# Luckick/EAGCN

Hardware: AMD Instinct MI355X
Metric: molecules/sec fwd+bwd, 2-layer 5-view EAGCN, Tox21 batch (higher is better)
Workload: dtype f32 (bf16x3 split, fp32 accumulate): every fp32 operand leaves its producer as three bf16 planes, six v_mfma_f32_32x32x16_bf16 piece products per 16 k rebuild the fp32 product (csrc/gemm_bx3.hip); aggregation, BatchNorm, head, first layer fp32

## Files before the change

eagcn_amd/_lib.py:

```python
import ctypes as C
import os

_HERE = os.path.dirname(os.path.abspath(__file__))
LIB_PATH = os.path.join(_HERE, 'lib', 'libeagcn_hip.so')

MAX_VIEWS = 8
MAX_SEGS = 8
META_WORDS = 16
META_NLOG = 8
META_T, META_NMAX, META_NTILES, META_BAD_ADJ, META_BAD_REL, META_NEDGE, META_OVERFLOW, META_EDGE_OVERFLOW = range(8)
META_NBLK = 9
STRUCT_CONCATE, STRUCT_WEIGHTED = 0, 1

_fp = C.c_void_p


class Batch(C.Structure):
    _fields_ = [('B', C.c_int32), ('N', C.c_int32), ('K', C.c_int32), ('ldc', C.c_int32),
                ('T', C.c_int32), ('n_max', C.c_int32), ('n_tiles', C.c_int32),
                ('channels', C.c_int32 * MAX_VIEWS),
                ('code', _fp), ('deg_bn', _fp), ('nat', _fp), ('row0', _fp), ('tile0', _fp),
                ('meta', _fp), ('row_mol', _fp), ('row_loc', _fp), ('row_m', _fp), ('row_deg', _fp),
                ('tile_mol', _fp), ('row_info', _fp), ('tile_info', _fp),
                ('rel_vec', _fp * MAX_VIEWS), ('rel_c', C.c_int32 * MAX_VIEWS),
# ... 41 lines not shown
def bond_ptrs_len(T, B):
    return 4 * T + 4 * B + 8 * (B + 1) + 8


def set_bond_lists(c, small_ptr, ptrs, edges, E):
    c.E = int(E)
    c.ecnt, c.edge0 = small_ptr, small_ptr + 4 * c.B
    pb, T = ptrs.data_ptr(), c.T
    c.row_ptr, c.col_ptr, c.mol_info = pb, pb + 8 * T, pb + 16 * T
    blk = pb + 16 * T + 16 * c.B
    c.blk = blk + (-blk) % 16 if ptrs.numel() >= bond_ptrs_len(T, c.B) else None
    eb = edges.data_ptr()
    c.nbr, c.tnbr = eb, eb + 4 * E
    code = eb + 8 * E
    code += (-code) % 8
    c.ecode, c.tcode = code, code + 8 * E


def index_error(meta, row_cap=None, edge_cap=None, compact=False):
    if meta[META_BAD_ADJ] and compact:
        return '%d bonds are out of range or listed twice' % meta[META_BAD_ADJ]
    if meta[META_BAD_ADJ]:
        return ('adjs holds %d entries outside {0,1}: the hot path requires a 0/1 adjacency (reference neural_fp.py:85,109-110)'
                % meta[META_BAD_ADJ])
    if meta[META_BAD_REL]:
        return ('%d bonded (i,j,view) positions are not one-hot over the relation channels (reference neural_fp.py:111-120); '
                'build the model with relations=\'general\' for relation tensors with arbitrary channel values (layers.py:82)'
                % meta[META_BAD_REL])
    if row_cap is not None and meta[META_OVERFLOW]:
        return ('%d packed rows, more than row_cap=%d (the batch is indexed as an empty batch; no memory is overwritten)'
                % (meta[META_OVERFLOW], row_cap))
    if edge_cap is not None and meta[META_EDGE_OVERFLOW]:
        return ('%d directed bonds, more than edge_cap=%d (the batch is indexed as an empty batch; no memory is overwritten)'
                % (meta[META_EDGE_OVERFLOW], edge_cap))
    return None


def dropout_seeds(seed, n_layers=4):
    seed = int(seed)
    return [(seed + 7919 * (l + 1)) & (2 ** 63 - 1) for l in range(n_layers)], (seed + 0x51ED27) & (2 ** 63 - 1)


STRUCTURES = {'Concate': 0, 'Weighted_sum': 1}


def structure_code(name):
    return STRUCTURES.get(name, -1)


class GatParams(C.Structure):
    _fields_ = [('fin', C.c_int32), ('ld_in', C.c_int32), ('F', C.c_int32), ('training', C.c_int32),
                ('alpha', C.c_float), ('att_dropout', C.c_float), ('dropout', C.c_float), ('reserved_', C.c_float),
                ('seed', C.c_uint64), ('W', _fp), ('a', _fp), ('seed_dev', C.c_void_p)]


POOL_MAX = 8


class PoolAtt(C.Structure):
    _fields_ = [('K', C.c_int32), ('mode', C.c_int32), ('att_c', C.c_int32 * MAX_VIEWS), ('att_w', _fp * MAX_VIEWS),
                ('ave_a', _fp), ('self_r', _fp), ('datt_w', _fp * MAX_VIEWS), ('dave_a', _fp), ('dself_r', _fp)]


class Layout(C.Structure):
    _fields_ = [('nseg', C.c_int32), ('width', C.c_int32 * MAX_SEGS), ('pad', C.c_int32 * MAX_SEGS)]


class LayerParams(C.Structure):
    _fields_ = [('K', C.c_int32), ('structure', C.c_int32), ('training', C.c_int32),
                ('width', C.c_int32 * MAX_VIEWS), ('inp', Layout),
                ('dropout', C.c_float), ('bn_eps', C.c_float), ('bn_momentum', C.c_float),
                ('seed', C.c_uint64), ('seed_dev', _fp),
                ('att_w', _fp * MAX_VIEWS), ('self_r', _fp * MAX_VIEWS), ('W', _fp * MAX_VIEWS),
                ('bias', _fp * MAX_VIEWS), ('gamma', _fp * MAX_VIEWS), ('beta', _fp * MAX_VIEWS),
                ('run_mean', _fp * MAX_VIEWS), ('run_var', _fp * MAX_VIEWS), ('ave_w', _fp)]


class LayerBufs(C.Structure):
    _fields_ = [('x', _fp), ('P', _fp), ('Y', _fp), ('rscale', _fp), ('bn', _fp), ('xout', _fp),
                ('pad_row', _fp), ('scratch', _fp), ('scratch_bytes', C.c_size_t),
                ('aux_stream', _fp), ('packed', _fp), ('packed_bytes', C.c_size_t),
                ('stats_hook', _fp), ('stats_user', _fp), ('x_planes', _fp), ('xout_planes', _fp)]


class LayerGrads(C.Structure):
    _fields_ = [('dW', _fp * MAX_VIEWS), ('dbias', _fp * MAX_VIEWS), ('dgamma', _fp * MAX_VIEWS),
                ('dbeta', _fp * MAX_VIEWS), ('datt_w', _fp * MAX_VIEWS), ('dself_r', _fp * MAX_VIEWS),
                ('dave_w', _fp)]


class HeadParams(C.Structure):
    _fields_ = [('f_in', C.c_int32), ('n_den1', C.c_int32), ('n_den2', C.c_int32), ('nclass', C.c_int32),
                ('dropout', C.c_float), ('bn_eps', C.c_float), ('bn_momentum', C.c_float),
                ('den1_w', _fp), ('den2_w', _fp), ('den3_w', _fp),
                ('gbn_w', _fp), ('gbn_b', _fp), ('gbn_rm', _fp), ('gbn_rv', _fp),
                ('bn1_w', _fp), ('bn1_b', _fp), ('bn1_rm', _fp), ('bn1_rv', _fp),
                ('bn2_w', _fp), ('bn2_b', _fp), ('bn2_rm', _fp), ('bn2_rv', _fp)]


class HeadGrads(C.Structure):
    _fields_ = [(n, _fp) for n in ('d_den1_w', 'd_den2_w', 'd_den3_w', 'd_gbn_w', 'd_gbn_b', 'd_bn1_w', 'd_bn1_b',
                                   'd_bn2_w', 'd_bn2_b')]


class Model(C.Structure):
    _fields_ = [('n_layers', C.c_int32), ('molfp_mode', C.c_int32), ('training', C.c_int32),
                ('head_seed', C.c_uint64), ('head_seed_dev', _fp), ('input_packed', C.c_int32), ('aux_stream', _fp),
                ('layer', LayerParams * 4), ('head', HeadParams), ('stats_hook', _fp), ('stats_user', _fp),
                ('stats_world', C.c_int32), ('fuse_readout', C.c_int32), ('fwd_signal', _fp), ('wait_flag', _fp), ('start_signal', _fp)]


class StepLoss(C.Structure):
    _fields_ = [('kind', C.c_int32), ('labels', _fp), ('class_weight', _fp), ('loss', _fp), ('scale', _fp), ('dout', _fp)]


ALLREDUCE_FN = C.CFUNCTYPE(C.c_int, C.c_void_p, C.c_int, C.c_void_p, C.c_void_p)


SIGNATURES = {
    'eagcn_abi_version': (C.c_int, []),
    'eagcn_struct_size': (C.c_size_t, [C.c_int]),
    'eagcn_last_error': (C.c_char_p, []),
    'eagcn_pad16': (C.c_int, [C.c_int]),
    'eagcn_layer_out_ld': (C.c_int, [C.POINTER(LayerParams)]),
    'eagcn_layer_fp': (C.c_int, [C.POINTER(LayerParams)]),
    'eagcn_layer_packed_bytes': (C.c_size_t, [C.POINTER(Batch), C.POINTER(LayerParams)]),
    'eagcn_layer_fwd_scratch_bytes': (C.c_size_t, [C.POINTER(Batch), C.POINTER(LayerParams)]),
    'eagcn_layer_bwd_scratch_bytes': (C.c_size_t, [C.POINTER(Batch), C.POINTER(LayerParams)]),
    'eagcn_layer_route': (C.c_int, [C.POINTER(Batch), C.POINTER(LayerParams), C.POINTER(LayerBufs), C.c_int, C.c_int, C.c_int, C.c_int,
                                    C.POINTER(C.c_int32 * 16)]),
    'eagcn_index_build': (C.c_int, [_fp, C.POINTER(_fp), C.POINTER(Batch), _fp, _fp]),
    'eagcn_index_from_bonds': (C.c_int, [_fp, _fp, _fp, _fp, C.c_int64, C.POINTER(Batch), _fp, _fp]),
    'eagcn_index_rows': (C.c_int, [C.POINTER(Batch), _fp]),
    'eagcn_set_gemm_mode': (C.c_int, [C.c_int]),
    'eagcn_stream_wait_counter': (C.c_int, [_fp, C.c_uint32, _fp]),
    'eagcn_stream_signal_flag': (C.c_int, [_fp, _fp]),
    'eagcn_stream_wait_flag': (C.c_int, [_fp, C.c_double, _fp]),
    'eagcn_stream_wait_timeouts': (C.c_int, []),
    'eagcn_stream_wait_reset': (None, []),
    'eagcn_adam_step': (C.c_int, [_fp, _fp, _fp, _fp, C.c_int64, _fp, _fp, _fp, _fp]),
    'eagcn_grad_norm_workspace_bytes': (C.c_size_t, []),
    'eagcn_grad_norm': (C.c_int, [_fp, _fp, C.c_int64, _fp, C.c_int, _fp]),
    'eagcn_adam_step_clipped': (C.c_int, [_fp, _fp, _fp, _fp, C.c_int64, _fp, _fp, _fp, _fp, _fp, _fp, _fp]),
    'eagcn_agg_wants_bond_lists': (C.c_int, [C.c_int, C.c_int]),
    'eagcn_agg_wants_bond_lists_for': (C.c_int, [C.c_int, C.c_int, C.c_int]),
    'eagcn_bx3_used_splits': (C.c_int, [C.c_int, C.c_int, C.c_int, C.c_int]),
    'eagcn_set_bx3_wide': (C.c_int, [C.c_int]),
    'eagcn_set_top_bn_sums': (C.c_int, [C.c_int]),
    'eagcn_set_hidden_bn_sums': (C.c_int, [C.c_int]),
    'eagcn_hidden_bn_sums_taken': (C.c_long, [C.c_int]),
    'eagcn_set_first_layer_fused': (C.c_int, [C.c_int]),
    'eagcn_first_layer_fused_taken': (C.c_long, [C.c_int]),
    'eagcn_first_layer_fused_last': (None, [C.POINTER(C.c_int32)]),
    'eagcn_bx3_pair_used_splits': (C.c_int, [C.c_int] * 7),
    'eagcn_bx3_plane_elems': (C.c_size_t, [C.c_int, C.c_int]),
    'eagcn_bx3_split': (C.c_int, [_fp, C.c_int, C.c_int, _fp, C.c_size_t, C.c_int, C.c_int, _fp]),
    'eagcn_gemm_bx3': (C.c_int, [C.c_int, C.c_int, C.c_int, C.c_int, _fp, C.c_size_t, C.c_int, C.c_int, _fp, C.c_size_t, C.c_int, C.c_int,
                                 _fp, C.c_int, C.c_int, C.c_size_t, C.c_int, _fp]),
    'eagcn_gemm_bx3_pair': (C.c_int, [C.c_int, C.c_int, C.c_int, _fp, C.c_size_t, C.c_int, C.c_int, _fp, C.c_size_t, C.c_int, C.c_int, _fp, C.c_int,
                                      C.c_int, C.c_int, C.c_int, _fp, C.c_size_t, C.c_int, C.c_int, _fp, C.c_size_t, C.c_int, C.c_int, _fp, C.c_int,
                                      C.c_int, C.c_size_t, C.c_int, _fp]),
    'eagcn_pack_rows': (C.c_int, [C.POINTER(Batch), _fp, C.c_int, C.POINTER(Layout), _fp, _fp]),
    'eagcn_unpack_rows': (C.c_int, [C.POINTER(Batch), _fp, C.POINTER(Layout), _fp, _fp, C.c_int, _fp]),
    'eagcn_pad_rows': (C.c_int, [_fp, _fp, C.c_int, C.c_int, C.c_int, _fp, _fp]),
    'eagcn_gat_scratch_bytes': (C.c_size_t, [C.POINTER(Batch), C.c_int]),
    'eagcn_gat_forward': (C.c_int, [C.POINTER(Batch), C.POINTER(GatParams), _fp, _fp, _fp, _fp, _fp]),
    'eagcn_gat_backward': (C.c_int, [C.POINTER(Batch), C.POINTER(GatParams), _fp, _fp, _fp, _fp, _fp, _fp, _fp, _fp, _fp,
                                     C.c_size_t, _fp]),
    'eagcn_pool_scratch_bytes': (C.c_size_t, []),
    'eagcn_pool_attention_forward': (C.c_int, [C.POINTER(Batch), C.POINTER(PoolAtt), _fp, C.c_int, _fp, _fp, _fp]),
    'eagcn_pool_attention_backward': (C.c_int, [C.POINTER(Batch), C.POINTER(PoolAtt), _fp, C.c_int, _fp, _fp, _fp, C.c_size_t,
                                                _fp]),
    'eagcn_pool_mix_forward': (C.c_int, [C.POINTER(Batch), C.POINTER(Layout), _fp, C.c_int, _fp, _fp, _fp, _fp, C.c_int, _fp]),
    'eagcn_pool_mix_backward': (C.c_int, [C.POINTER(Batch), C.POINTER(Layout), _fp, C.c_int, _fp, _fp, _fp, _fp, C.c_int, _fp,
                                          _fp, _fp, _fp]),
    'eagcn_pool_reduce_forward': (C.c_int, [C.POINTER(Batch), _fp, C.c_int, C.c_int, C.c_int, _fp, _fp, _fp, _fp]),
    'eagcn_pool_reduce_backward': (C.c_int, [C.POINTER(Batch), _fp, C.c_int, C.c_int, C.c_int, _fp, _fp, _fp, _fp, _fp]),
    'eagcn_layer_forward': (C.c_int, [C.POINTER(Batch), C.POINTER(LayerParams), C.POINTER(LayerBufs), _fp]),
    'eagcn_layer_backward': (C.c_int, [C.POINTER(Batch), C.POINTER(LayerParams), C.POINTER(LayerBufs),
                                       _fp, _fp, _fp, C.POINTER(LayerGrads), _fp]),
    'eagcn_attention_dense': (C.c_int, [C.POINTER(Batch), C.POINTER(LayerParams), _fp, _fp]),
    'eagcn_readout_forward': (C.c_int, [C.POINTER(Batch), _fp, C.POINTER(Layout), _fp, _fp, C.c_int, _fp,
                                        C.c_int, _fp]),
    'eagcn_readout_backward': (C.c_int, [C.POINTER(Batch), _fp, C.POINTER(Layout), _fp, C.c_int, C.c_int,
                                         _fp, _fp, _fp]),
    'eagcn_gemm_f32': (C.c_int, [C.c_int, C.c_int, C.c_int, C.c_int, C.c_int, _fp, C.c_int, _fp, C.c_int,
                                 _fp, C.c_int, _fp]),
    'eagcn_gemm_f32_dev': (C.c_int, [C.c_int, C.c_int, C.c_int, C.c_int, C.c_int, _fp, C.c_int, _fp, C.c_int,
                                     _fp, C.c_int, _fp, C.c_int, _fp]),
    'eagcn_gemm_sk_workspace_bytes': (C.c_size_t, []),
    'eagcn_gemm_f32_sk': (C.c_int, [C.c_int, C.c_int, C.c_int, C.c_int, C.c_int, _fp, C.c_int, _fp, C.c_int,
                                    _fp, C.c_int, _fp, C.c_size_t, _fp]),
    'eagcn_gemm_pair_sk': (C.c_int, [C.c_int, C.c_int, C.c_int, _fp, C.c_int, _fp, C.c_int, _fp, C.c_int,
                                     C.c_int, C.c_int, C.c_int, _fp, C.c_int, _fp, C.c_int, _fp, C.c_int,
                                     _fp, C.c_size_t, _fp]),
    'eagcn_gemm_pair_sk_slabs': (C.c_int, [C.c_int, C.c_int, C.c_int, _fp, C.c_int, _fp, C.c_int, _fp, C.c_int,
                                           C.c_int, C.c_int, C.c_int, _fp, C.c_int, _fp, C.c_int, _fp, C.c_int,
                                           C.c_size_t, _fp, C.c_size_t, _fp]),
    'eagcn_gemm_sk_plan': (C.c_int, [C.c_int] * 7 + [C.POINTER(C.c_int), C.POINTER(C.c_int)]),
    'eagcn_gemm_sk_timeouts': (C.c_int, []),
    'eagcn_gemm_sk_failed': (C.c_int, []),
    'eagcn_gemm_sk_reset_failed': (None, []),
    'eagcn_gemm_sk_inject_failure': (None, []),
    'eagcn_model_saved_bytes': (C.c_size_t, [C.POINTER(Batch), C.POINTER(Model)]),
    'eagcn_model_scratch_bytes': (C.c_size_t, [C.POINTER(Batch), C.POINTER(Model)]),
    'eagcn_model_atom_rep': (C.c_int, [C.POINTER(Batch), C.POINTER(Model), C.POINTER(C.c_size_t),
                                       C.POINTER(C.c_size_t), C.POINTER(C.c_int)]),
    'eagcn_model_atom_rep_materialize': (C.c_int, [C.POINTER(Batch), C.POINTER(Model), _fp, C.c_size_t, _fp]),
    'eagcn_model_pack_input': (C.c_int, [C.POINTER(Batch), C.POINTER(Model), _fp, _fp, C.c_size_t, _fp]),
    'eagcn_model_forward': (C.c_int, [C.POINTER(Batch), C.POINTER(Model), _fp, _fp, _fp, C.c_size_t, _fp,
                                      C.c_size_t, _fp, _fp, _fp]),
    'eagcn_model_backward': (C.c_int, [C.POINTER(Batch), C.POINTER(Model), _fp, _fp, C.c_size_t, _fp, C.c_size_t,
                                       _fp, _fp, C.POINTER(LayerGrads), C.POINTER(HeadGrads), _fp]),
    'eagcn_model_backward_range': (C.c_int, [C.POINTER(Batch), C.POINTER(Model), _fp, _fp, C.c_size_t, _fp, C.c_size_t,
                                             _fp, _fp, C.POINTER(LayerGrads), C.POINTER(HeadGrads), C.c_int, C.c_int, C.c_int, _fp]),
    'eagcn_model_route': (C.c_int, [C.POINTER(Batch), C.POINTER(Model), _fp, C.c_size_t, _fp, C.c_size_t, C.c_int, C.c_int, C.c_int, C.c_int,
                                    C.c_int, C.POINTER(C.c_int32 * 16 * 4)]),
    'eagcn_model_input_scratch_bytes': (C.c_size_t, [C.POINTER(Batch), C.POINTER(Model)]),
    'eagcn_model_backward_input': (C.c_int, [C.POINTER(Batch), C.POINTER(Model), _fp, _fp, C.c_size_t, _fp, C.c_size_t,
                                             _fp, _fp, C.POINTER(LayerGrads), C.POINTER(HeadGrads), _fp, _fp]),
    'eagcn_attr_alpha': (C.c_float, [C.c_int, C.c_int]),
    'eagcn_attr_weight': (C.c_float, [C.c_int]),
    'eagcn_attr_acc_elems': (C.c_size_t, [C.POINTER(Batch), C.POINTER(Model)]),
    'eagcn_attr_pack_input': (C.c_int, [C.POINTER(Batch), C.POINTER(Model), _fp, _fp, C.c_float, _fp, C.c_size_t, _fp]),
    'eagcn_attr_step': (C.c_int, [C.POINTER(Batch), C.POINTER(Model), _fp, _fp, C.c_size_t, _fp, C.c_size_t, _fp, _fp, C.c_float,
                                  C.c_int, _fp, _fp]),
    'eagcn_attr_finalize': (C.c_int, [C.POINTER(Batch), C.POINTER(Model), _fp, _fp, _fp, _fp, _fp, _fp]),
    'eagcn_layer_bond_grad': (C.c_int, [C.POINTER(Batch), C.POINTER(LayerParams), C.POINTER(LayerBufs), _fp, C.c_int, C.c_float, C.c_int,
                                        _fp, _fp]),
    'eagcn_bond_attr_finalize': (C.c_int, [C.POINTER(Batch), _fp, C.c_int, _fp, _fp, _fp, _fp, _fp, _fp]),
    'eagcn_model_forward_step': (C.c_int, [C.POINTER(Batch), C.POINTER(Model), _fp, _fp, _fp, C.c_size_t, _fp, C.c_size_t, _fp, _fp,
                                           C.POINTER(StepLoss), _fp, C.POINTER(HeadGrads), _fp]),
    'eagcn_head_saved_bytes': (C.c_size_t, [C.POINTER(HeadParams), C.c_int]),
    'eagcn_head_scratch_bytes': (C.c_size_t, [C.POINTER(HeadParams), C.c_int]),
    'eagcn_head_forward': (C.c_int, [C.POINTER(HeadParams), C.c_int, C.c_int, C.c_uint64, _fp, _fp, _fp, C.c_size_t, _fp, C.c_size_t,
                                     _fp, _fp, _fp]),
    'eagcn_head_backward': (C.c_int, [C.POINTER(HeadParams), C.c_int, C.c_int, C.c_uint64, _fp, _fp, _fp, C.c_size_t, _fp, C.c_size_t,
                                      _fp, _fp, C.POINTER(HeadGrads), _fp, _fp]),
    'eagcn_bce_loss': (C.c_int, [_fp, _fp, _fp, C.c_int, C.c_int, _fp, _fp, _fp]),
    'eagcn_mse_loss': (C.c_int, [_fp, _fp, C.c_int, _fp, _fp, _fp]),
    'eagcn_eval_append': (C.c_int, [_fp, _fp, C.c_int, C.c_int, C.c_int, _fp, _fp, _fp, C.c_int64, _fp]),
    'eagcn_eval_metrics_workspace_bytes': (C.c_size_t, [C.c_int64, C.c_int]),
    'eagcn_eval_class_metrics': (C.c_int, [_fp, _fp, _fp, C.c_int64, C.c_int, _fp, C.c_size_t, _fp, _fp]),
    'eagcn_eval_reg_metrics': (C.c_int, [_fp, _fp, _fp, C.c_int64, C.c_int, _fp, C.c_size_t, _fp, _fp]),
    'eagcn_rep_gather': (C.c_int, [C.POINTER(Batch), _fp, C.POINTER(Layout), _fp, _fp, C.c_int, C.c_int, _fp, _fp, _fp, _fp, _fp, _fp,
                                   C.c_int64, _fp]),
    'eagcn_rep_gather_dense': (C.c_int, [_fp, C.c_int, C.c_int, C.c_int, _fp, C.c_int, C.c_int, C.c_int, _fp, _fp, _fp, _fp, _fp, _fp,
                                         C.c_int64, _fp]),
    'eagcn_kmeans_workspace_bytes': (C.c_size_t, [C.c_int64, C.c_int, C.c_int]),
    'eagcn_kmeans_begin': (C.c_int, [_fp, C.c_int64, C.c_int, C.c_int, C.c_int, _fp, C.c_double, _fp, C.c_size_t, _fp]),
    'eagcn_kmeans_iterate': (C.c_int, [_fp, C.c_int64, C.c_int, C.c_int, C.c_int, _fp, C.c_size_t, _fp]),
    'eagcn_kmeans_finish': (C.c_int, [_fp, C.c_int64, C.c_int, C.c_int, C.c_int, _fp, C.c_size_t, _fp]),
    'eagcn_kmeans_assign': (C.c_int, [_fp, C.c_int64, C.c_int, C.c_int, _fp, C.c_int, _fp, _fp, _fp, C.c_size_t, _fp]),
    'eagcn_sqdist': (C.c_int, [_fp, C.c_int64, C.c_int, C.c_int, _fp, _fp]),
    'eagcn_tsne_workspace_bytes': (C.c_size_t, [C.c_int64]),
    'eagcn_tsne_affinities': (C.c_int, [_fp, C.c_int64, C.c_double, _fp, C.c_int, _fp, _fp, _fp, C.c_size_t, _fp]),
    'eagcn_tsne_gradient': (C.c_int, [_fp, C.c_int, _fp, C.c_int64, C.c_float, C.c_int, _fp, _fp, _fp, C.c_size_t, _fp]),
    'eagcn_tsne_begin': (C.c_int, [_fp, C.c_int, C.c_int64, _fp, C.c_float, C.c_float, C.c_int, C.c_int, C.c_double, _fp, C.c_size_t,
                                   _fp]),
    'eagcn_tsne_iterate': (C.c_int, [_fp, C.c_int, C.c_int64, _fp, C.c_size_t, _fp]),
    'eagcn_tsne_finish': (C.c_int, [_fp, C.c_int, C.c_int64, _fp, C.c_size_t, _fp]),
    'eagcn_pca_workspace_bytes': (C.c_size_t, [C.c_int64, C.c_int]),
    'eagcn_pca_cov': (C.c_int, [_fp, C.c_int64, C.c_int, C.c_int, _fp, _fp, _fp, C.c_size_t, _fp]),
    'eagcn_pca_project': (C.c_int, [_fp, C.c_int64, C.c_int, C.c_int, _fp, _fp, C.c_int, _fp, _fp]),
    'eagcn_knn_workspace_bytes': (C.c_size_t, [C.c_int64, C.c_int64, C.c_int, C.c_int, C.c_int]),
    'eagcn_knn': (C.c_int, [_fp, C.c_int64, C.c_int, C.c_int, _fp, C.c_int64, C.c_int, C.c_int, C.c_int, C.c_int, _fp, _fp, _fp, C.c_size_t,
                            _fp]),
    'eagcn_knn_rank': (C.c_int, [_fp, C.c_int64, C.c_int, C.c_int, _fp, C.c_int, C.c_int, _fp, _fp, C.c_size_t, _fp]),
    'eagcn_prof_enable': (None, [C.c_int]),
    'eagcn_prof_reset': (None, []),
    'eagcn_prof_ntags': (C.c_int, []),
    'eagcn_prof_tag_name': (C.c_char_p, [C.c_int]),
    'eagcn_prof_read': (C.c_int, [C.c_int, C.POINTER(C.c_double), C.POINTER(C.c_double), C.POINTER(C.c_int64)]),
}

_lib = None


class EagcnHipError(RuntimeError):
    pass


ABI_VERSION = 8


def load():
    global _lib
    if _lib is not None:
        return _lib
    if not os.path.exists(LIB_PATH):
        raise EagcnHipError(
            'libeagcn_hip.so is not built (%s). Run `python -c "import __graft_entry__ as g; g.build()"` '
            'or `python -m eagcn_amd.build`; eagcn_amd has no CPU fallback.' % LIB_PATH)
    lib = C.CDLL(LIB_PATH)
    lib.eagcn_abi_version.restype = C.c_int
    if lib.eagcn_abi_version() != ABI_VERSION:
        raise EagcnHipError('libeagcn_hip.so speaks ABI version %d, this binding version %d: rebuild it '
                            '(`python -c "import __graft_entry__ as g; g.build()"`)' % (lib.eagcn_abi_version(), ABI_VERSION))
    for name, (res, args) in SIGNATURES.items():
        fn = getattr(lib, name)
        fn.restype = res
        fn.argtypes = args
    for which, cls in ((0, Batch), (1, Layout), (2, LayerParams), (3, LayerBufs), (4, LayerGrads), (5, HeadParams), (6, HeadGrads),
                       (7, Model), (10, StepLoss)):
        if lib.eagcn_struct_size(which) != C.sizeof(cls):
            raise EagcnHipError('ABI mismatch: %s is %d bytes here, %d in libeagcn_hip.so'
# ... 27 lines not shown
```

eagcn_amd/build.py:

```python
import os
import shutil
import subprocess
import sys
from concurrent.futures import ThreadPoolExecutor

HERE = os.path.dirname(os.path.abspath(__file__))
CSRC = os.path.join(HERE, 'csrc')
LIBDIR = os.path.join(HERE, 'lib')
LIB = os.path.join(LIBDIR, 'libeagcn_hip.so')
HIP_SOURCES = ['index.hip', 'gemm.hip', 'gemm3.hip', 'gemm_bx3.hip', 'gemm_bx3w.hip', 'agg.hip', 'lagg.hip', 'lagg_in.hip', 'lagg_top.hip', 'lagg_dw.hip', 'gat.hip', 'pool.hip', 'layer.hip', 'readout.hip', 'head.hip', 'head2.hip', 'loss.hip', 'clip.hip', 'attr.hip', 'battr.hip', 'metrics.hip', 'reps.hip', 'embed.hip', 'knn.hip']
CPP_SOURCES = ['api.cpp']
HEADERS = ['common.h', 'kernels.h', 'lagg_kernel.h', 'gemm_x6.h', 'bx3.h', 'bx3_epi.h', os.path.join('..', '..', 'include', 'eagcn_hip.h')]
ARCH = 'gfx950'


def _hipcc():
    for cand in (shutil.which('hipcc'), '/opt/rocm/bin/hipcc'):
        if cand and os.path.exists(cand):
            return cand
    raise RuntimeError('hipcc not found: the EAGCN HIP library cannot be built')


def _newest(paths):
    return max(os.path.getmtime(p) for p in paths)


def needs_build():
    srcs = [os.path.join(CSRC, s) for s in HIP_SOURCES + CPP_SOURCES + HEADERS if os.path.exists(os.path.join(CSRC, s))]
    return (not os.path.exists(LIB)) or os.path.getmtime(LIB) < _newest(srcs)


def build_library(force=False, verbose=False):
    if not force and not needs_build():
        return LIB
    hipcc = _hipcc()
    os.makedirs(LIBDIR, exist_ok=True)
    objdir = os.path.join(LIBDIR, 'obj')
    os.makedirs(objdir, exist_ok=True)
    flags = ['--offload-arch=' + ARCH, '-O3', '-std=c++17', '-fPIC', '-Wall', '-Wno-unused-function', '-munsafe-fp-atomics']

    hdr_time = _newest([os.path.join(CSRC, h) for h in HEADERS if os.path.exists(os.path.join(CSRC, h))])

    def compile_one(src):
        obj = os.path.join(objdir, os.path.splitext(src)[0] + '.o')
        if not force and os.path.exists(obj) and os.path.getmtime(obj) > max(hdr_time, os.path.getmtime(os.path.join(CSRC, src))):
            return obj
        cmd = [hipcc] + flags + ['-c', os.path.join(CSRC, src), '-o', obj]
        if src.endswith('.cpp'):
            cmd = [hipcc, '-O2', '-std=c++17', '-fPIC', '-c', os.path.join(CSRC, src), '-o', obj]
        r = subprocess.run(cmd, capture_output=True, text=True)
        if r.returncode != 0:
            raise RuntimeError('hipcc failed on %s:\n%s\n%s' % (src, r.stdout, r.stderr))
        if verbose and r.stderr.strip():
            print(r.stderr, file=sys.stderr)
        return obj

    sources = [s for s in HIP_SOURCES + CPP_SOURCES if os.path.exists(os.path.join(CSRC, s))]
    with ThreadPoolExecutor(max_workers=min(8, len(sources))) as ex:
        objs = list(ex.map(compile_one, sources))
    tmp = LIB + '.tmp'
    r = subprocess.run([hipcc, '--offload-arch=' + ARCH, '-shared', '-fPIC', '-o', tmp] + objs,
                       capture_output=True, text=True)
    if r.returncode != 0:
        raise RuntimeError('link failed:\n%s\n%s' % (r.stdout, r.stderr))
    os.replace(tmp, LIB)
    return LIB


if __name__ == '__main__':
    print(build_library(force='--force' in sys.argv, verbose=True))
```

eagcn_amd/csrc/head.hip:

```cpp
#include <stdlib.h>

#include <algorithm>

#include "common.h"
#include "kernels.h"

namespace eagcn {

__global__ void wait_counter_kernel(const uint32_t* __restrict__ word, uint32_t value, int* __restrict__ err,
                                    unsigned long long budget_ticks) {
    if (threadIdx.x == 0) {
        const unsigned long long t0 = wall_clock64();
        while ((int32_t)(__hip_atomic_load(word, __ATOMIC_ACQUIRE, __HIP_MEMORY_SCOPE_AGENT) - value) < 0) {
            __builtin_amdgcn_s_sleep(64);
            if (wall_clock64() - t0 > budget_ticks) {
                if (err) __hip_atomic_store(err, 1, __ATOMIC_RELAXED, __HIP_MEMORY_SCOPE_SYSTEM);
                break;
            }
        }
    }
}



// ... 129 lines not shown
    const eagcn_head_params* h = &m->head;
    const size_t B = (size_t)b->B, T = (size_t)b->T;
    s.n_hst = 2 * (h->f_in + h->n_den1 + h->n_den2) + 6;
    s.hst = c.take<double>((size_t)(HEAD_COPIES + 1) * s.n_hst + HEAD_WS);
    s.hsb = s.hst + (size_t)HEAD_COPIES * s.n_hst;
    s.hws = s.hsb + s.n_hst;
    s.da2 = c.take<float>(B * h->n_den2);
    s.da1 = c.take<float>(B * h->n_den1);
    s.dgn = c.take<float>(B * h->f_in);
    s.dg = c.take<float>(B * h->f_in);
    s.hdw_ks = head_dw_chunks(b->B);
    s.hdw = c.take<float>(s.hdw_ks > 1 ? (size_t)s.hdw_ks * ((size_t)h->f_in * h->n_den1 + (size_t)h->n_den1 * h->n_den2 +
                                                             (size_t)h->n_den2 * h->nclass) : 1);
    int ldmax = 0;
    size_t lbytes = 0;
    for (int l = 0; l < m->n_layers; ++l) {
        ldmax = std::max(ldmax, eagcn_layer_out_ld(&m->layer[l]));
        lbytes = std::max(lbytes, eagcn_layer_fwd_scratch_bytes(b, &m->layer[l]));
        lbytes = std::max(lbytes, eagcn_layer_bwd_scratch_bytes(b, &m->layer[l]));
    }
    s.dxa = c.take<float>(T * ldmax);
    s.dxb = c.take<float>(T * ldmax);
    s.dpad = c.take<float>((size_t)EAGCN_MAX_VIEWS * ldmax);
    s.layer_bytes = lbytes;
    s.layer = c.take<char>(lbytes);
    s.top_dge = c.take<float>(B * h->f_in);
    s.top_slab = c.take<double>((size_t)top_bn_slabs(b->B) * eagcn_layer_fp(&m->layer[m->n_layers - 1]) * 2);
    int fpmax = 0;
    for (int l = 0; l + 1 < m->n_layers; ++l) fpmax = std::max(fpmax, eagcn_layer_fp(&m->layer[l]));
    s.hid_slab = c.take<double>(fpmax ? (size_t)hidden_bn_slabs(b->T) * fpmax * 2 : 1);
    if (out) *out = s;
    return c.off;
}

static int check_model(const eagcn_batch* b, const eagcn_model* m, const char* who) {
    EAGCN_CHECK_ARG(b && m, "%s: null argument", who);
    if (int rc = check_reserved_null(m->aux_stream, who, "eagcn_model.aux_stream")) return rc;
    EAGCN_CHECK_ARG(m->n_layers >= 1 && m->n_layers <= 4, "%s: n_layers=%d", who, m->n_layers);
    const eagcn_head_params* h = &m->head;
    EAGCN_CHECK_ARG(h->f_in >= 1 && h->n_den1 >= 1 && h->n_den2 >= 1 && h->nclass >= 1, "%s: bad head sizes", who);
    EAGCN_CHECK_ARG(h->den1_w && h->den2_w && h->den3_w && h->gbn_w && h->gbn_b && h->gbn_rm && h->gbn_rv &&
                        h->bn1_w && h->bn1_b && h->bn1_rm && h->bn1_rv && h->bn2_w && h->bn2_b && h->bn2_rm &&
                        h->bn2_rv, "%s: null head parameter", who);
    const eagcn_layer_params* last = &m->layer[m->n_layers - 1];
    const int f_last = last->structure == EAGCN_STRUCT_CONCATE ? [&] { int s = 0; for (int k = 0; k < last->K; ++k) s += last->width[k]; return s; }()
                                                                 : last->width[0];
    EAGCN_CHECK_ARG(f_last == h->f_in, "%s: head expects %d features, last layer yields %d", who, h->f_in, f_last);
    EAGCN_CHECK_ARG(!m->training || b->B > 1, "%s: BatchNorm in training mode needs more than one molecule", who);
    return EAGCN_OK;
}

static eagcn_layout out_layout(const eagcn_layer_params* p) {
    eagcn_layout l;
    memset(&l, 0, sizeof(l));
    if (p->structure == EAGCN_STRUCT_CONCATE) {
        l.nseg = p->K;
        for (int k = 0; k < p->K; ++k) { l.width[k] = p->width[k]; l.pad[k] = pad16(p->width[k]); }
    } else {
        l.nseg = 1;
        l.width[0] = p->width[0];
        l.pad[0] = pad16(p->width[0]);
    }
    return l;
}

static bool fused_readout(const eagcn_model* m) {
    static const bool env = !env_flag("EAGCN_NO_FUSED_READOUT", false);
    return env && m->fuse_readout && m->layer[m->n_layers - 1].structure == EAGCN_STRUCT_CONCATE;
}

struct ModelAsk { int layer_hi = -1, layer_lo = 0; bool has_dx0 = false, input_only = false; };
struct LayerPlan {
    eagcn_layer_bufs w;
    LayerRoute fwd, bwd;
    bool planes_only = false;
    bool skip_apply = false;
    BxBnEpi below = {};
};
struct ModelPlan { LayerPlan L[4]; bool top_formed = false; };
static ModelPlan plan_model(const eagcn_batch* b, const eagcn_model* m, const ModelSaved& sv, const ModelScratch& sc, const ModelAsk& ask) {
    ModelPlan P{};
    const int top = m->n_layers - 1;
    PlanAsk full;
    full.has_dx = true;
    for (int l = 0; l <= top; ++l) {
        const LayerSaved& L = sv.L[l];
        LayerPlan& Q = P.L[l];
        eagcn_layer_bufs& w = Q.w;
        w.P = L.P; w.Y = L.Y; w.rscale = L.rscale; w.bn = L.bn; w.xout = L.xout; w.pad_row = L.pad_row;
        w.scratch = sc.layer; w.scratch_bytes = sc.layer_bytes; w.packed = L.packed; w.packed_bytes = L.packed_bytes;
        w.stats_hook = m->stats_hook; w.stats_user = m->stats_user;
        w.x_planes = l > 0 ? sv.L[l - 1].xout_planes : nullptr; w.xout_planes = L.xout_planes;
        const bool try_planes = w.x_planes && planes_only_enabled();
        w.x = l == 0 ? sv.x0 : try_planes ? nullptr : sv.L[l - 1].xout;
        Q.fwd = plan_layer(b, &m->layer[l], &w, PlanAsk{});
        if (try_planes) {
            P.L[l - 1].planes_only = Q.fwd.fwd_prod == FWD_PLANES && plan_layer(b, &m->layer[l], &w, full).bwd_prod == BWD_PLANES_PAIR;
            if (!P.L[l - 1].planes_only) { w.x = sv.L[l - 1].xout; Q.fwd = plan_layer(b, &m->layer[l], &w, PlanAsk{}); }
        }
    }
    P.L[top].skip_apply = fused_readout(m);
    const float* dge = top_bn_gather_enabled() ? sc.top_dge : nullptr;
    auto call_ask = [&](int l, const ModelAsk& k, bool top_sums) {
        PlanAsk a;
        a.has_dx = l > 0 || k.has_dx0; a.mol_grad = l == top; a.input_only = k.input_only; a.has_drain_out = l > k.layer_lo && !k.input_only;
        a.top_sums = l == top && top_sums && !k.input_only; a.top_gather = a.top_sums && top_gather_ok(&m->layer[top], dge, m->head.f_in);
        return a;
    };
    if (top_bn_sums_enabled() && P.L[top].skip_apply && m->training && m->layer[top].training && !m->stats_hook && (unsigned)m->molfp_mode <= 1u) {
        const LayerRoute r = plan_layer(b, &m->layer[top], &P.L[top].w, call_ask(top, ModelAsk{top}, true));
        P.top_formed = r.bn2 == BN2_STAGED_FROM_READOUT && r.bwd_agg == AGG_LAGG && r.edge == EDGE_WITH_LAGG;
    }
    for (int l = ask.layer_hi; l >= ask.layer_lo; --l) {
        LayerPlan& Q = P.L[l];
        PlanAsk a = call_ask(l, ask, P.top_formed);
        a.dh_given = l < ask.layer_hi && P.L[l + 1].bwd.carries_below;
        if (l > ask.layer_lo && !ask.input_only && m->training && !m->stats_hook && sv.L[l].ld_in == sv.L[l - 1].fp) {
            PlanAsk low = call_ask(l - 1, ask, false);
            low.dh_given = true;
            a.below = plan_layer(b, &m->layer[l - 1], &P.L[l - 1].w, low).dh_given;
        }
        Q.bwd = plan_layer(b, &m->layer[l], &Q.w, a);
        if (Q.bwd.carries_below) {
            const eagcn_layer_params* lo = &m->layer[l - 1];
            const DropArgs dr = drop_args(lo->dropout, lo->training != 0, lo->seed, lo->seed_dev);
            const LayerSaved& S = sv.L[l - 1];
            Q.below = BxBnEpi{S.Y, S.fp, S.bn, S.fp, b->row_m, dr.on, dr.thr, dr.inv_keep, dr.seed, dr.seed_dev, sc.hid_slab};
        }
    }
    return P;
}

}

using namespace eagcn;

#define RC(call) do { int rc_ = (call); if (rc_) return rc_; } while (0)

extern "C" size_t eagcn_model_saved_bytes(const eagcn_batch* b, const eagcn_model* m) {
    return carve_saved(nullptr, b, m, nullptr);
}
extern "C" size_t eagcn_model_scratch_bytes(const eagcn_batch* b, const eagcn_model* m) {
    return carve_scratch(nullptr, b, m, nullptr);
}
extern "C" int eagcn_model_atom_rep(const eagcn_batch* b, const eagcn_model* m, size_t* xout_offset,
                                    size_t* pad_row_offset, int* ld) {
    EAGCN_CHECK_ARG(b && m && xout_offset && pad_row_offset && ld, "eagcn_model_atom_rep: null argument");
    RC(check_reserved_null(m->aux_stream, "eagcn_model_atom_rep", "eagcn_model.aux_stream"));
    ModelSaved s;
    carve_saved(nullptr, b, m, &s);
    *xout_offset = s.xout_last_off;
    *pad_row_offset = s.pad_last_off;
    *ld = eagcn_layer_out_ld(&m->layer[m->n_layers - 1]);
    return EAGCN_OK;
}

extern "C" int eagcn_model_atom_rep_materialize(const eagcn_batch* b, const eagcn_model* m, void* saved, size_t saved_bytes,
                                                 void* stream) {
    EAGCN_CHECK_ARG(b && m && saved, "eagcn_model_atom_rep_materialize: null argument");
    RC(check_reserved_null(m->aux_stream, "eagcn_model_atom_rep_materialize", "eagcn_model.aux_stream"));
    if (!fused_readout(m)) return EAGCN_OK;
    ModelSaved sv;
    EAGCN_CHECK_ARG(carve_saved(saved, b, m, &sv) <= saved_bytes, "eagcn_model_atom_rep_materialize: saved block too small");
    const int l = m->n_layers - 1;
    LayerSaved& L = sv.L[l];
    eagcn_layer_bufs w;
    memset(&w, 0, sizeof(w));
    w.Y = L.Y; w.bn = L.bn; w.xout = L.xout; w.pad_row = L.pad_row; w.packed = L.packed; w.packed_bytes = L.packed_bytes;
    return layer_apply_impl(b, &m->layer[l], &w, stream);
}

extern "C" int eagcn_model_pack_input(const eagcn_batch* b, const eagcn_model* m, const float* afm, void* saved,
                                      size_t saved_bytes, void* stream) {
    EAGCN_CHECK_ARG(b && m && afm && saved, "eagcn_model_pack_input: null argument");
    RC(check_reserved_null(m->aux_stream, "eagcn_model_pack_input", "eagcn_model.aux_stream"));
    ModelSaved sv;
    EAGCN_CHECK_ARG(carve_saved(saved, b, m, &sv) <= saved_bytes, "eagcn_model_pack_input: saved block too small");
    return eagcn_pack_rows(b, afm, layout_width(&m->layer[0].in), &m->layer[0].in, sv.x0, stream);
}

struct HeadPlan {
    HeadFwd f1, f2, f3;
    HeadBwd b3, b2, b1;
    HeadGbn bg;
    double *st_g, *st_1, *st_2, *sb_g, *sb_1, *sb_2;
    bool sync;
    const int64_t* size;
};
static HeadPlan head_plan(const eagcn_batch* b, const eagcn_model* m, const ModelSaved& sv, const ModelScratch& sc, float* out,
                          float* graph_rep, const float* dout, const float* dgraph_rep, const eagcn_head_grads* hg,
                          const int64_t* size = nullptr, bool top_formed = false) {
    HeadPlan P;
    P.size = size;
    const eagcn_head_params* h = &m->head;
    const int B = b->B, F = h->f_in, n1 = h->n_den1, n2 = h->n_den2, nc = h->nclass;
    P.st_g = sc.hst; P.st_1 = sc.hst + 2 * F + 2; P.st_2 = sc.hst + 2 * (F + n1) + 4;
    P.sb_g = sc.hsb; P.sb_1 = sc.hsb + 2 * F + 2; P.sb_2 = sc.hsb + 2 * (F + n1) + 4;
    P.sync = m->stats_hook && m->training;
    const int copies = P.sync ? 1 : HEAD_COPIES;
    const HeadDrop nodrop{0, 0u, 1.0f, 0, nullptr}, drop1 = drop_args(h->dropout, m->training != 0, m->head_seed, m->head_seed_dev);
    P.f1 = HeadFwd{B, F, n1, sv.g, P.st_g, h->gbn_w, h->gbn_b, h->gbn_rm, h->gbn_rv, sv.bn_g, h->den1_w, sv.h1, nullptr, P.st_1,
                   m->training, 0, h->bn_eps, h->bn_momentum, nodrop};
    P.f2 = HeadFwd{B, n1, n2, sv.h1, P.st_1, h->bn1_w, h->bn1_b, h->bn1_rm, h->bn1_rv, sv.bn_1, h->den2_w, sv.h2, graph_rep, P.st_2,
                   m->training, 1, h->bn_eps, h->bn_momentum, drop1};
    P.f3 = HeadFwd{B, n2, nc, sv.h2, P.st_2, h->bn2_w, h->bn2_b, h->bn2_rm, h->bn2_rv, sv.bn_2, h->den3_w, out, nullptr, nullptr,
                   m->training, 1, h->bn_eps, h->bn_momentum, nodrop};
    if (P.sync) { P.f1.cnt_in = P.st_g + 2 * F; P.f2.cnt_in = P.st_1 + 2 * n1; P.f3.cnt_in = P.st_2 + 2 * n2; }
    P.f3.nw = 8;
    P.f1.signal = m->fwd_signal;
    P.f1.st_copies = P.f2.st_copies = P.f3.st_copies = copies;
    P.f1.st_stride = P.f2.st_stride = P.f3.st_stride = sc.n_hst;
    if (!hg) return P;
    const double *cn_g = sc.hst + 2 * F, *cn_1 = sc.hst + 2 * F + 2 + 2 * n1, *cn_2 = sc.hst + 2 * (F + n1) + 4 + 2 * n2;
    const float gscale = P.sync && m->stats_world > 1 ? 1.0f / (float)m->stats_world : 1.0f;
    P.b3 = HeadBwd{B, n2, nc, sv.h2, sv.bn_2, 1, nodrop, h->den3_w, dout, nullptr, nullptr, nullptr, nullptr, nullptr, nullptr,
                   sc.da2, P.sb_2, hg->d_den3_w, m->training};
    P.b2 = HeadBwd{B, n1, n2, sv.h1, sv.bn_1, 1, drop1, h->den2_w, sc.da2, sv.h2, sv.bn_2, P.sb_2, dgraph_rep, hg->d_bn2_w, hg->d_bn2_b,
                   sc.da1, P.sb_1, hg->d_den2_w, m->training};
    P.b1 = HeadBwd{B, F, n1, sv.g, sv.bn_g, 0, nodrop, h->den1_w, sc.da1, sv.h1, sv.bn_1, P.sb_1, nullptr, hg->d_bn1_w, hg->d_bn1_b,
                   sc.dgn, P.sb_g, hg->d_den1_w, m->training};
    if (P.sync) { P.b2.cnt_y = cn_2; P.b2.gscale = gscale; P.b1.cnt_y = cn_1; P.b1.gscale = gscale; }
    P.b3.nw = 8;
    const int ks = sc.hdw_ks;
    float* part3 = sc.hdw;
    float* part2 = part3 + (size_t)ks * n2 * nc;
    float* part1 = part2 + (size_t)ks * n1 * n2;
    if (ks > 1) {
        P.b3.ks = ks; P.b3.dW_part = part3;
        P.b2.ks = ks; P.b2.dW_part = part2;
        P.b1.ks = ks; P.b1.dW_part = part1;
    }
    P.bg = HeadGbn{B, F, sc.dgn, sv.g, sv.bn_g, P.sb_g, sc.dg, hg->d_gbn_w, hg->d_gbn_b, m->training};
    if (P.sync) { P.bg.cnt = cn_g; P.bg.gscale = gscale; }
    if (top_formed) {
        const eagcn_layer_params* last = &m->layer[m->n_layers - 1];
        const eagcn_layout lay = out_layout(last);
        P.bg.top = HeadTopSums{sv.top_a1, sv.top_a2, sc.top_slab, top_bn_slabs(B), eagcn_layer_fp(last), make_colmap(&lay), P.size, m->molfp_mode,
                               top_bn_gather_enabled() ? sc.top_dge : nullptr};
    }
    if (ks > 1) {
        P.bg.sum[0] = HeadDwSum{hg->d_den3_w, part3, n2 * nc, ks};
        P.bg.sum[1] = HeadDwSum{hg->d_den2_w, part2, n1 * n2, ks};
        P.bg.sum[2] = HeadDwSum{hg->d_den1_w, part1, F * n1, ks};
        P.bg.nsum = 3;
    }
    return P;
}

static int model_forward_trunk(const eagcn_batch* b, const eagcn_model* m, const float* afm, const int64_t* size, void* saved,
                               size_t saved_bytes, void* scratch, size_t scratch_bytes, ModelSaved& sv, ModelScratch& sc,
                               ModelPlan& P, void* stream, const char* who) {
    hipStream_t s = (hipStream_t)stream;
    RC(check_model(b, m, who));
    EAGCN_CHECK_GEMM3(who);
    EAGCN_CHECK_ARG((afm || m->input_packed) && saved && scratch, "%s: null buffer", who);
    EAGCN_CHECK_ARG(m->molfp_mode == 0 || size, "%s: 'ave' read-out needs size", who);
    EAGCN_CHECK_ARG(carve_saved(saved, b, m, &sv) <= saved_bytes, "%s: saved block too small", who);
    EAGCN_CHECK_ARG(carve_scratch(scratch, b, m, &sc) <= scratch_bytes, "%s: scratch too small", who);
    const eagcn_head_params* h = &m->head;
    HandOff ho{m->start_signal, m->wait_flag, wait_err_word(), 200000000ull};
    if (!m->input_packed && (m->wait_flag || m->start_signal)) {
        handoff_kernel<<<1, 64, 0, s>>>(ho);
        EAGCN_LAUNCH_CHECK();
        ho.start = nullptr; ho.flag = nullptr;
    }
    ZeroJob zj;
    RC(gemm3_zero_job(sc.layer, sc.layer_bytes, sc.hst, (HEAD_COPIES + 1) * sc.n_hst + HEAD_WS, &zj));
    if (!m->input_packed)
        RC(eagcn_pack_rows(b, afm, layout_width(&m->layer[0].in), &m->layer[0].in, sv.x0, stream));
    {
        const eagcn_layer_params* ps[4];
        void* pk[4];
        size_t pkb[4];
        for (int l = 0; l < m->n_layers; ++l) { ps[l] = &m->layer[l]; pk[l] = sv.L[l].packed; pkb[l] = sv.L[l].packed_bytes; }
        RC(pack_params_all(b, ps, pk, pkb, m->n_layers, stream, &zj, &ho));
    }
    P = plan_model(b, m, sv, sc, ModelAsk{});
    for (int l = 0; l < m->n_layers; ++l)
        RC(layer_forward_impl(b, &m->layer[l], &P.L[l].w, stream, P.L[l].fwd, true, P.L[l].skip_apply, P.L[l].planes_only));
    const eagcn_layer_params* last = &m->layer[m->n_layers - 1];
    const LayerSaved& LL = sv.L[m->n_layers - 1];
    const eagcn_layout lay = out_layout(last);
    const int B = b->B, F = h->f_in, n1 = h->n_den1, n2 = h->n_den2;
    double *st_g = sc.hst, *st_1 = sc.hst + 2 * F + 2, *st_2 = sc.hst + 2 * (F + n1) + 4;
    const int copies = (m->stats_hook && m->training) ? 1 : HEAD_COPIES;
    if (fused_readout(m)) {
        ReadoutBn rb;
        rb.Y = LL.Y; rb.ldy = LL.fp; rb.bn = LL.bn; rb.fp = LL.fp;
        const DropArgs ld = drop_args(last->dropout, last->training != 0, last->seed, last->seed_dev);
        rb.do_drop = ld.on; rb.thr = ld.thr; rb.inv_keep = ld.inv_keep; rb.seed = ld.seed; rb.seed_dev = ld.seed_dev;
        rb.size = size; rb.mode = m->molfp_mode; rb.g = sv.g; rb.F = F; rb.st = st_g;
        rb.cnt0 = st_g + 2 * F; rb.cnt1 = st_1 + 2 * n1; rb.cnt2 = st_2 + 2 * n2;
        rb.st_copies = copies; rb.st_stride = sc.n_hst;
        if (P.top_formed) { rb.A1 = sv.top_a1; rb.A2 = sv.top_a2; }
        RC(readout_bn_forward(b, &lay, rb, stream));
    } else if (pad_sampled(m))
        RC(readout_forward_sampled(b, LL.xout, &lay, last, LL.bn + (size_t)LL.fp , size,
                                   m->molfp_mode, sv.g, F, sv.pad_cnt, sv.padc, sv.pad_tab, stream));
    else
        RC(eagcn_readout_forward(b, LL.xout, &lay, last->structure == EAGCN_STRUCT_WEIGHTED ? LL.pad_row : nullptr,
                                 size, m->molfp_mode, sv.g, F, stream));
    if (!fused_readout(m)) RC(head_colstats(sv.g, B, F, st_g, s, st_g + 2 * F, st_1 + 2 * n1, st_2 + 2 * n2));
    return EAGCN_OK;
}

static int stats_hook_call(const eagcn_model* m, bool sync, double* buf, int n, void* stream) {
    if (!sync) return EAGCN_OK;
    if (m->stats_hook(buf, n, stream, m->stats_user)) {
        set_error("eagcn_model: the sync-BatchNorm all-reduce hook failed");
        return EAGCN_ERR_HIP;
    }
    return EAGCN_OK;
}

static int head_forward_launches(const eagcn_model* m, const HeadPlan& P, void* stream) {
    hipStream_t s = (hipStream_t)stream;
    const eagcn_head_params* h = &m->head;
    RC(stats_hook_call(m, P.sync, P.st_g, 2 * h->f_in + 1, stream));
    RC(head_fwd(P.f1, s));
    RC(stats_hook_call(m, P.sync, P.st_1, 2 * h->n_den1 + 1, stream));
    RC(head_fwd(P.f2, s));
    RC(stats_hook_call(m, P.sync, P.st_2, 2 * h->n_den2 + 1, stream));
    RC(head_fwd(P.f3, s));
    return EAGCN_OK;
}
static int head_backward_launches(const eagcn_model* m, const HeadPlan& P, void* stream) {
    hipStream_t s = (hipStream_t)stream;
    const eagcn_head_params* h = &m->head;
    RC(head_bwd(P.b3, s));
    RC(stats_hook_call(m, P.sync, P.sb_2, 2 * h->n_den2, stream));
    RC(head_bwd(P.b2, s));
    RC(stats_hook_call(m, P.sync, P.sb_1, 2 * h->n_den1, stream));
    RC(head_bwd(P.b1, s));
    RC(stats_hook_call(m, P.sync, P.sb_g, 2 * h->f_in, stream));
    RC(head_gbn_bwd(P.bg, s));
    return EAGCN_OK;
}
static int readout_pad_backward(const eagcn_batch* b, const eagcn_model* m, const int64_t* size, const ModelSaved& sv,
                                const ModelScratch& sc, void* stream) {
    const eagcn_layer_params* last = &m->layer[m->n_layers - 1];
    const eagcn_layout lay = out_layout(last);
    const int F = m->head.f_in;
    if (pad_sampled(m)) return readout_backward_pad_views(b, sc.dg, &lay, size, m->molfp_mode, F, last->K, sv.pad_cnt, last->dropout, sc.dpad, stream);
    if (last->structure == EAGCN_STRUCT_WEIGHTED) return readout_backward_pad(b, sc.dg, &lay, size, m->molfp_mode, F, sc.dpad, stream);
    return EAGCN_OK;
}

extern "C" int eagcn_model_forward(const eagcn_batch* b, const eagcn_model* m, const float* afm,
                                   const int64_t* size, void* saved, size_t saved_bytes, void* scratch,
                                   size_t scratch_bytes, float* out, float* graph_rep, void* stream) {
    EAGCN_CHECK_ARG(out && graph_rep, "eagcn_model_forward: null buffer");
    ModelSaved sv;
    ModelScratch sc;
    ModelPlan mp;
    RC(model_forward_trunk(b, m, afm, size, saved, saved_bytes, scratch, scratch_bytes, sv, sc, mp, stream, "eagcn_model_forward"));
    const HeadPlan P = head_plan(b, m, sv, sc, out, graph_rep, nullptr, nullptr, nullptr);
    return head_forward_launches(m, P, stream);
}

namespace eagcn {
static int check_head(const eagcn_head_params* h, int B, int training, const char* who) {
    EAGCN_CHECK_ARG(h, "%s: null argument", who);
    EAGCN_CHECK_ARG(B >= 1 && h->f_in >= 1 && h->n_den1 >= 1 && h->n_den2 >= 1 && h->nclass >= 1, "%s: bad head sizes", who);
    EAGCN_CHECK_ARG(h->den1_w && h->den2_w && h->den3_w && h->gbn_w && h->gbn_b && h->gbn_rm && h->gbn_rv && h->bn1_w && h->bn1_b &&
                        h->bn1_rm && h->bn1_rv && h->bn2_w && h->bn2_b && h->bn2_rm && h->bn2_rv, "%s: null head parameter", who);
    EAGCN_CHECK_ARG(!training || B > 1, "%s: BatchNorm in training mode needs more than one molecule", who);
    return EAGCN_OK;
}
static size_t carve_head_saved(void* base, const eagcn_head_params* h, int B, ModelSaved* out) {
    Carver2 c(base);
    ModelSaved s;
    memset(&s, 0, sizeof(s));
    s.h1 = c.take<float>((size_t)B * h->n_den1);
    s.h2 = c.take<float>((size_t)B * h->n_den2);
    s.bn_g = c.take<float>((size_t)4 * h->f_in);
    s.bn_1 = c.take<float>((size_t)4 * h->n_den1);
    s.bn_2 = c.take<float>((size_t)4 * h->n_den2);
    if (out) *out = s;
    return c.off;
}
static size_t carve_head_scratch(void* base, const eagcn_head_params* h, int B, ModelScratch* out) {
    Carver2 c(base);
    ModelScratch s;
    memset(&s, 0, sizeof(s));
    s.n_hst = 2 * (h->f_in + h->n_den1 + h->n_den2) + 6;
    s.hst = c.take<double>((size_t)(HEAD_COPIES + 1) * s.n_hst + HEAD_WS);
    s.hsb = s.hst + (size_t)HEAD_COPIES * s.n_hst;
    s.hws = s.hsb + s.n_hst;
    s.da2 = c.take<float>((size_t)B * h->n_den2);
    s.da1 = c.take<float>((size_t)B * h->n_den1);
    s.dgn = c.take<float>((size_t)B * h->f_in);
    s.hdw_ks = head_dw_chunks(B);
    s.hdw = c.take<float>(s.hdw_ks > 1 ? (size_t)s.hdw_ks * ((size_t)h->f_in * h->n_den1 + (size_t)h->n_den1 * h->n_den2 +
                                                             (size_t)h->n_den2 * h->nclass) : 1);
    if (out) *out = s;
    return c.off;
}
__global__ __launch_bounds__(256) void head_zero_kernel(double* __restrict__ p, int n) {
    for (int i = blockIdx.x * blockDim.x + threadIdx.x; i < n; i += gridDim.x * blockDim.x) p[i] = 0.0;
}
static int head_zero(double* p, size_t n, hipStream_t s) {
    head_zero_kernel<<<(unsigned)std::max<size_t>(1, std::min<size_t>((n + 255) / 256, 64)), 256, 0, s>>>(p, (int)n);
    EAGCN_LAUNCH_CHECK();
    return EAGCN_OK;
}
static void head_alone_model(const eagcn_head_params* h, int B, int training, uint64_t seed, const uint64_t* seed_dev,
                             eagcn_batch* b, eagcn_model* m) {
    memset(b, 0, sizeof(*b));
    memset(m, 0, sizeof(*m));
    b->B = B;
    m->head = *h; m->training = training ? 1 : 0; m->head_seed = seed; m->head_seed_dev = seed_dev;
}
}

extern "C" size_t eagcn_head_saved_bytes(const eagcn_head_params* h, int B) { return h ? carve_head_saved(nullptr, h, B, nullptr) : 0; }
extern "C" size_t eagcn_head_scratch_bytes(const eagcn_head_params* h, int B) { return h ? carve_head_scratch(nullptr, h, B, nullptr) : 0; }

extern "C" int eagcn_head_forward(const eagcn_head_params* h, int B, int training, uint64_t seed, const uint64_t* seed_dev,
                                  const float* g, void* saved, size_t saved_bytes, void* scratch, size_t scratch_bytes, float* out,
                                  float* graph_rep, void* stream) {
    hipStream_t s = (hipStream_t)stream;
    RC(check_head(h, B, training, "eagcn_head_forward"));
    EAGCN_CHECK_GEMM3("eagcn_head_forward");
    EAGCN_CHECK_ARG(g && saved && scratch && out && graph_rep, "eagcn_head_forward: null buffer");
    ModelSaved sv;
    ModelScratch sc;
    EAGCN_CHECK_ARG(carve_head_saved(saved, h, B, &sv) <= saved_bytes, "eagcn_head_forward: saved block too small");
    EAGCN_CHECK_ARG(carve_head_scratch(scratch, h, B, &sc) <= scratch_bytes, "eagcn_head_forward: scratch too small");
    eagcn_batch b;
    eagcn_model m;
    head_alone_model(h, B, training, seed, seed_dev, &b, &m);
    sv.g = const_cast<float*>(g);
    const int F = h->f_in, n1 = h->n_den1, n2 = h->n_den2;
    RC(head_zero(sc.hst, (size_t)(HEAD_COPIES + 1) * sc.n_hst + HEAD_WS, s));
    double *st_g = sc.hst, *st_1 = sc.hst + 2 * F + 2, *st_2 = sc.hst + 2 * (F + n1) + 4;
    RC(head_colstats(g, B, F, st_g, s, st_g + 2 * F, st_1 + 2 * n1, st_2 + 2 * n2));
    const HeadPlan P = head_plan(&b, &m, sv, sc, out, graph_rep, nullptr, nullptr, nullptr);
    return head_forward_launches(&m, P, stream);
}

extern "C" int eagcn_head_backward(const eagcn_head_params* h, int B, int training, uint64_t seed, const uint64_t* seed_dev,
                                   const float* g, void* saved, size_t saved_bytes, void* scratch, size_t scratch_bytes,
                                   const float* dout, const float* dgraph_rep, const eagcn_head_grads* hg, float* dg, void* stream) {
    hipStream_t s = (hipStream_t)stream;
    RC(check_head(h, B, training, "eagcn_head_backward"));
    EAGCN_CHECK_GEMM3("eagcn_head_backward");
    EAGCN_CHECK_ARG(g && saved && scratch && dout && hg && dg, "eagcn_head_backward: null buffer");
// ... 279 lines not shown
```

eagcn_amd/csrc/kernels.h:

```cpp
#pragma once
#include "bx3.h"
#include "common.h"

namespace eagcn {

struct AggArgs {
    eagcn_batch bt;
    ViewCols vc;
    const float* src; int lds;
    float* dst; int ldd;
    const float* sig;
    const float* rsig;
    float* rscale;
    double* stats;
    int nchunk;
    int cpw = 1;
    int xcd = 0;
    bool w_rowm = false;
    bool w_gather = false;
    BxOut planes = {nullptr, 0, 0, 0};
    const float* bn_tab = nullptr; const float* bn_cc = nullptr; int bn_fp = 0;
    const float* w_aw = nullptr;
    int w_drop = 0; uint32_t w_thr = 0; float w_inv_keep = 1.0f; uint64_t w_seed = 0; const uint64_t* w_seed_dev = nullptr;
    const float* fx = nullptr; int fx_ld = 0; float* dw = nullptr; size_t dw_slab = 0; int dw_ny = 0;
// ... 114 lines not shown
                               "co-resident with its owner): that launch's results are NaN-poisoned; call "           \
                               "eagcn_gemm_sk_reset_failed() after fixing the cause (EAGCN_GEMM3_WGS, concurrent work)", who); \
            return EAGCN_ERR_HIP;                                                                                      \
        }                                                                                                              \
    } while (0)
int gemm_mode();
inline int gemm_planes() { const int m = gemm_mode(); return m == 3 ? 3 : m == 4 ? 1 : 0; }
struct ZeroJob { unsigned* u; int nu; double* d; int nd; };
struct HandOff { uint32_t* start; uint32_t* flag; int* err; unsigned long long budget; };
__device__ __forceinline__ void handoff_body(const HandOff& h) {
    if (h.start) __hip_atomic_fetch_add(h.start, 1u, __ATOMIC_RELEASE, __HIP_MEMORY_SCOPE_AGENT);
    if (h.flag) {
        const unsigned long long t0 = wall_clock64();
        while (__hip_atomic_load(h.flag, __ATOMIC_ACQUIRE, __HIP_MEMORY_SCOPE_AGENT) == 0u) {
            __builtin_amdgcn_s_sleep(8);
            if (wall_clock64() - t0 > h.budget) {
                if (h.err) __hip_atomic_store(h.err, 1, __ATOMIC_RELAXED, __HIP_MEMORY_SCOPE_SYSTEM);
                break;
            }
        }
        __hip_atomic_store(h.flag, 0u, __ATOMIC_RELAXED, __HIP_MEMORY_SCOPE_AGENT);
    }
}
int gemm3_zero_job(void* workspace, size_t bytes, double* zero, int nzero, ZeroJob* out);
int zero_fill(void* p, size_t bytes, hipStream_t s);
bool gemm3_ok(const GemmDesc& g);
int launch_gemm3(const GemmDesc& g, const DwScatter* sc, void* workspace, size_t bytes, hipStream_t s);
int launch_gemm3_pair(const GemmDesc& dx, const GemmDesc& dw, const DwScatter* sc, void* workspace, size_t bytes, hipStream_t s,
                      size_t xk_slab = 0);

constexpr int HEAD_COPIES = 8;
using HeadDrop = DropArgs;
struct HeadFwd {
    int B, K, N;
    const float* x; const double* st_in; const float *gamma, *beta; float *run_mean, *run_var; float* bn;
    const float* W; float* y; float* y2; double* st_out;
    int training, relu; float eps, momentum; HeadDrop drop;
    const double* cnt_in = nullptr;
    int st_copies = 1, st_stride = 0;
    const float* lab = nullptr; int nlab = 0; unsigned* lab_cnt = nullptr;
    int nw = 0;
    uint32_t* signal = nullptr;
};
struct HeadBwd {
    int B, K, N;
    const float* x; const float* bnp; int relu_p; HeadDrop drop; const float* W;
    const float* dy; const float* y; const float* bny; const double* sb_y; const float* extra;
    float *dgamma_y, *dbeta_y; float* dyp; double* sb_p; float* dW; int training;
    const double* cnt_y = nullptr;
    float gscale = 1.0f;
    int ks = 1; float* dW_part = nullptr;
    int nw = 0;
};
inline int head_dw_chunks(int B) { return B > 256 ? (B + 255) / 256 < 16 ? (B + 255) / 256 : 16 : 1; }
struct HeadDwSum { float* dst; const float* part; int n, ks; };
struct HeadTopSums { const float *A1, *A2; double* slab; int nslab, fp; ColMapD map; const int64_t* size; int mode; float* dge; };
struct HeadGbn { int B, F; const float *dgn, *g, *bn; const double* sb; float *dg, *dgamma, *dbeta; int training;
                 const double* cnt = nullptr; float gscale = 1.0f;
                 HeadDwSum sum[3] = {}; int nsum = 0;
                 HeadTopSums top = {}; };
inline int top_bn_slabs(int B) { return B > 256 ? 64 : 16; }
struct HeadLoss { int kind;
                  const float* labels; const float* weight; float* loss; const float* scale; float* dout; };
struct HeadMid { HeadFwd f3; HeadBwd b3; HeadLoss L;
                 double* ws; };
constexpr int HEAD_WS = 4;
struct HeadLossFin { float* loss; const double* ws; const float* scale; int kind, n; };
bool head_mid_ok(int n_den2, int nclass);
int head_mid(const HeadMid& a, hipStream_t s);
int head_bwd_pair(const HeadBwd& a, const HeadBwd& e, const HeadLossFin& lf, hipStream_t s);
int head_colstats(const float* g, int B, int F, double* st, hipStream_t s, double* cnt0 = nullptr, double* cnt1 = nullptr,
                  double* cnt2 = nullptr);
int head_fwd(const HeadFwd& a, hipStream_t s);
int head_bwd(const HeadBwd& a, hipStream_t s);
int head_gbn_bwd(const HeadGbn& a, hipStream_t s);

struct EdgeDrain {
    double* eacc; int K;
    float* datt_w[EAGCN_MAX_VIEWS]; float* dself_r[EAGCN_MAX_VIEWS]; int channels[EAGCN_MAX_VIEWS];
    const float* rsig;
};
struct LayerBwdOpts {
    const ReadoutGrad* rg = nullptr;
    bool dpad_views = false;
    const ZeroJob* zero_after = nullptr;
    const EdgeDrain* drain_in = nullptr;
    EdgeDrain* drain_out = nullptr;
    bool input_only = false;
    const double* top_sums = nullptr; int top_nslab = 0;
    const float* top_dge = nullptr;
    const BxBnEpi* below = nullptr;
    const double* dh_sums = nullptr; int dh_nslab = 0;
};
inline int hidden_bn_slabs(int T) { return (T > 0 ? T + BX_EPI_ROWS - 1 : BX_EPI_ROWS) / BX_EPI_ROWS; }
bool top_bn_sums_enabled();
bool top_bn_gather_enabled();
bool planes_only_enabled();
bool top_gather_ok(const eagcn_layer_params* p, const float* dge, int F);

enum FwdProd { FWD_NONE = 0, FWD_PLANES, FWD_BALANCED, FWD_TILED, FWD_REFUSED };
enum AggPath { AGG_DENSE = 0, AGG_LAGG };
enum Bn2 {
    BN2_NONE = 0,
    BN2_ELEMENTWISE,
    BN2_REDUCE_APPLY,
    BN2_STAGED_FROM_DH,
    BN2_STAGED_FROM_UPSTREAM,
    BN2_STAGED_ROWMASK,
    BN2_STAGED_FROM_READOUT
};
enum EdgePath { EDGE_NONE = 0, EDGE_WITH_LAGG, EDGE_COLAUNCH };
enum BwdProd {
    BWD_NONE = 0, BWD_PLANES_PAIR, BWD_PLANES_DW, BWD_PLANES_DX,
    BWD_G3_XK, BWD_G3_SCATTER,
    BWD_TILED_PAIR, BWD_TILED_SEPARATE, BWD_TILED_DX,
    BWD_REFUSED
};
struct PlanAsk {
    bool has_dx = false;
    bool mol_grad = false;
    bool input_only = false;
    bool has_drain_out = false;
    bool top_sums = false;
    bool top_gather = false;
    bool dh_given = false;
    bool below = false;
};
struct LayerRoute {
    FwdProd fwd_prod = FWD_NONE; bool fwd_split_x = false;
    AggPath fwd_agg = AGG_DENSE, bwd_agg = AGG_DENSE;
    Bn2 bn2 = BN2_NONE;
    bool rows_first = false, rows_late = false;
    bool store_dh = false;
    EdgePath edge = EDGE_NONE; bool edge_atomic = false;
    BwdProd bwd_prod = BWD_NONE; bool bwd_split_x = false;
    bool bx_wide = false;
    bool carries_below = false;
    bool defer_drain = false;
    bool dh_given = false;
    bool dw_fused = false; int dw_ny = 0; bool dw_in_dp = false;
    bool bn2_staged() const { return bn2 >= BN2_STAGED_FROM_DH; }
    bool bwd_planes() const { return bwd_prod >= BWD_PLANES_PAIR && bwd_prod <= BWD_PLANES_DX; }
};
LayerRoute plan_layer(const eagcn_batch* b, const eagcn_layer_params* p, const eagcn_layer_bufs* w, const PlanAsk& ask);
int layer_backward_impl(const eagcn_batch* b, const eagcn_layer_params* p, const eagcn_layer_bufs* w, const float* dxout,
                        const float* dpad_row, float* dx, const eagcn_layer_grads* g, void* stream, const LayerRoute& r,
                        const LayerBwdOpts& o = LayerBwdOpts{});
int model_backward_input_packed(const eagcn_batch* b, const eagcn_model* m, const int64_t* size, void* saved, size_t saved_bytes,
                                void* scratch, size_t scratch_bytes, const float* dout, const float* dgraph_rep,
                                const eagcn_layer_grads* lg, const eagcn_head_grads* hg, float** dx0, void* stream, const char* who);
int launch_attr_dense(const eagcn_batch* b, const eagcn_layout* in, const float* acc, const float* x, const float* base, float* attr,
                      float* score, hipStream_t s);
int model_input_slot(const eagcn_batch* b, const eagcn_model* m, void* saved, size_t saved_bytes, float** x0, const char* who);
int layer_forward_impl(const eagcn_batch* b, const eagcn_layer_params* p, const eagcn_layer_bufs* w, void* stream, const LayerRoute& r,
                       bool prepacked, bool skip_apply = false, bool planes_only = false);
inline int check_reserved_null(const void* value, const char* who, const char* field) {
    EAGCN_CHECK_ARG(!value, "%s: %s is reserved and must be null", who, field);
    return EAGCN_OK;
}
int layer_apply_impl(const eagcn_batch* b, const eagcn_layer_params* p, const eagcn_layer_bufs* w, void* stream);
int pack_params_all(const eagcn_batch* b, const eagcn_layer_params* const* ps, void* const* packed,
                    const size_t* packed_bytes, int n, void* stream, const ZeroJob* zj = nullptr, const HandOff* ho = nullptr);
struct ReadoutBn {
    const float* Y; int ldy;
    const float* bn; int fp;
    int do_drop; uint32_t thr; float inv_keep; uint64_t seed; const uint64_t* seed_dev;
    const int64_t* size; int mode;
    float* g; int F;
    double* st;
    int st_copies = 1, st_stride = 0;
    bool pair = false;
    double *cnt0, *cnt1, *cnt2;
    float* A1 = nullptr; float* A2 = nullptr;
};
int readout_bn_forward(const eagcn_batch* b, const eagcn_layout* lay, const ReadoutBn& a, void* stream);
int readout_forward_sampled(const eagcn_batch* b, const float* x, const eagcn_layout* lay, const eagcn_layer_params* p,
                            const float* bn_sh, const int64_t* size, int mode, float* g, int F, uint16_t* cnt, float* padc,
                            uint32_t* tab, void* stream);
int readout_backward_pad_views(const eagcn_batch* b, const float* dg, const eagcn_layout* lay, const int64_t* size, int mode,
                               int F, int K, const uint16_t* cnt, float dropout, float* dpad, void* stream);
int readout_backward_pad(const eagcn_batch* b, const float* dg, const eagcn_layout* lay, const int64_t* size,
                         int mode, int F, float* dpad_row, void* stream);

}
```

eagcn_amd/csrc/layer.hip:

```cpp
#include <algorithm>

#include <stdlib.h>

#include "common.h"
#include "kernels.h"

namespace eagcn {

struct ParamPtrs {
    const float* att_w[EAGCN_MAX_VIEWS];
    const float* self_r[EAGCN_MAX_VIEWS];
    const float* W[EAGCN_MAX_VIEWS];
    const float* bias[EAGCN_MAX_VIEWS];
    const float* gamma[EAGCN_MAX_VIEWS];
    const float* beta[EAGCN_MAX_VIEWS];
    float* run_mean[EAGCN_MAX_VIEWS];
    float* run_var[EAGCN_MAX_VIEWS];
    const float* ave_w;
    int channels[EAGCN_MAX_VIEWS];
    const float* rel_vec[EAGCN_MAX_VIEWS];
    int rel_c[EAGCN_MAX_VIEWS];
};
__device__ __forceinline__ float att_logit(const ParamPtrs& pp, int k, int c) {
    if (!pp.rel_vec[k]) return pp.att_w[k][c - 1];
    const float* v = pp.rel_vec[k] + (size_t)(c - 1) * pp.rel_c[k];
    float s = 0.0f;
    for (int ch = 0; ch < pp.rel_c[k]; ++ch) s = fmaf(pp.att_w[k][ch], v[ch], s);
    return s;
}
struct GradPtrs {
    float* dW[EAGCN_MAX_VIEWS];
    float* dbias[EAGCN_MAX_VIEWS];
    float* dgamma[EAGCN_MAX_VIEWS];
    float* dbeta[EAGCN_MAX_VIEWS];
    float* datt_w[EAGCN_MAX_VIEWS];
    float* dself_r[EAGCN_MAX_VIEWS];
    float* dave_w;
};

enum { CP_GAMMA = 0, CP_BETA, CP_BIAS, CP_RMEAN, CP_RVAR, CP_AVEW, CP_ROWS = 8 };

__device__ __forceinline__ int col_view(const ViewCols& vc, int cp) {
    int k = 0;
#pragma unroll
    for (int v = 1; v < EAGCN_MAX_VIEWS; ++v) k += (v < vc.K && cp >= vc.off[v]) ? 1 : 0;
    return k;
}
__device__ __forceinline__ int packed_to_exact(const ColMapD& m, int cp) {
    int eo = 0, po = 0;
    for (int s = 0; s < m.nseg; ++s) {
        if (cp < po + m.p[s]) return (cp - po < m.w[s]) ? eo + (cp - po) : -1;
        eo += m.w[s];
        po += m.p[s];
    }
    return -1;
}

__device__ __forceinline__ void pack_params_body(const ParamPtrs& pp, const ViewCols& vc, const ColMapD& in, int ld_in,
                                                 int fp, float* __restrict__ Wcat, float* __restrict__ WcatT,
                                                 float* __restrict__ colp, float* __restrict__ sig, float* __restrict__ rsig,
                                                 const BxOut wp = BxOut{nullptr, 0, 0, 0}, const BxOut wtp = BxOut{nullptr, 0, 0, 0}) {
    __shared__ float tile[32][33];
    const int tx = threadIdx.x & 31, ty = threadIdx.x >> 5;
    const int ntx = (fp + 31) >> 5, nty = (ld_in + 31) >> 5;
    for (int t = blockIdx.x; t < ntx * nty; t += gridDim.x) {
        const int ip0 = (t / ntx) << 5, cp0 = (t % ntx) << 5;
        {
            const int cp = cp0 + tx;
            const int k = cp < fp ? col_view(vc, cp) : 0;
            const int f = cp - vc.off[k];
#pragma unroll
            for (int j = 0; j < 4; ++j) {
                const int ip = ip0 + ty + 8 * j;
                float v = 0.0f;
                if (ip < ld_in && cp < fp) {
                    const int fi = packed_to_exact(in, ip);
                    if (fi >= 0 && f < vc.width[k]) v = pp.W[k][(size_t)fi * vc.width[k] + f];
                    Wcat[(size_t)ip * fp + cp] = v;
                }
                tile[ty + 8 * j][tx] = v;
            }
        }
        __syncthreads();
#pragma unroll
        for (int j = 0; j < 4; ++j) {
            const int cp = cp0 + ty + 8 * j, ip = ip0 + tx;
            if (cp < fp && ip < ld_in) WcatT[(size_t)cp * ld_in + ip] = tile[tx][ty + 8 * j];
        }
        if (wp.p) {
            const int r = threadIdx.x >> 3, c4 = (threadIdx.x & 7) << 2;
            if (ip0 + r < ld_in && cp0 + c4 < fp)
                bx_store4(wp, ip0 + r, cp0 + c4, make_float4(tile[r][c4], tile[r][c4 + 1], tile[r][c4 + 2], tile[r][c4 + 3]));
            if (cp0 + r < fp && ip0 + c4 < ld_in)
                bx_store4(wtp, cp0 + r, ip0 + c4, make_float4(tile[c4][r], tile[c4 + 1][r], tile[c4 + 2][r], tile[c4 + 3][r]));
        }
        __syncthreads();
    }
    for (int cp = blockIdx.x * blockDim.x + threadIdx.x; cp < fp; cp += gridDim.x * blockDim.x) {
        const int k = col_view(vc, cp), f = cp - vc.off[k];
        const bool ok = f < vc.width[k];
        colp[CP_GAMMA * fp + cp] = ok ? pp.gamma[k][f] : 0.0f;
        colp[CP_BETA * fp + cp] = ok ? pp.beta[k][f] : 0.0f;
        colp[CP_BIAS * fp + cp] = ok ? pp.bias[k][f] : 0.0f;
        colp[CP_RMEAN * fp + cp] = ok ? pp.run_mean[k][f] : 0.0f;
        colp[CP_RVAR * fp + cp] = ok ? pp.run_var[k][f] : 1.0f;
        colp[CP_AVEW * fp + cp] = pp.ave_w ? pp.ave_w[k] : 1.0f;
    }
    for (int e = blockIdx.x * blockDim.x + threadIdx.x; e < vc.K * 256; e += gridDim.x * blockDim.x) {
        const int k = e >> 8, c = e & 255;
        sig[e] = (c >= 1 && c <= pp.channels[k]) ? sigmoidf_(att_logit(pp, k, c)) : 0.0f;
    }
    if (blockIdx.x == 0 && threadIdx.x < vc.K) rsig[threadIdx.x] = sigmoidf_(pp.self_r[threadIdx.x][0]);
}
__global__ __launch_bounds__(256) void pack_params_kernel(ParamPtrs pp, ViewCols vc, ColMapD in, int ld_in, int fp,
                                                           float* __restrict__ Wcat, float* __restrict__ WcatT,
                                                           float* __restrict__ colp, float* __restrict__ sig,
                                                           float* __restrict__ rsig, BxOut wp, BxOut wtp) {
    pack_params_body(pp, vc, in, ld_in, fp, Wcat, WcatT, colp, sig, rsig, wp, wtp);
}
struct PackJob {
    ParamPtrs pp; ViewCols vc; ColMapD in; int ld_in, fp;
    float *Wcat, *WcatT, *colp, *sig, *rsig;
    BxOut wp, wtp;
};
struct PackJobs { PackJob j0, j1, j2, j3; };
__global__ __launch_bounds__(256) void pack_params_multi_kernel(PackJobs jobs, ZeroJob zj, HandOff ho) {
    if (blockIdx.y == 0) {
        for (int i = blockIdx.x * blockDim.x + threadIdx.x; i < max(zj.nu, zj.nd); i += gridDim.x * blockDim.x) {
            if (i < zj.nu) zj.u[i] = 0u;
            if (i < zj.nd) zj.d[i] = 0.0;
        }
    }
    if (blockIdx.y == 0) pack_params_body(jobs.j0.pp, jobs.j0.vc, jobs.j0.in, jobs.j0.ld_in, jobs.j0.fp, jobs.j0.Wcat, jobs.j0.WcatT, jobs.j0.colp, jobs.j0.sig, jobs.j0.rsig, jobs.j0.wp, jobs.j0.wtp);
    else if (blockIdx.y == 1) pack_params_body(jobs.j1.pp, jobs.j1.vc, jobs.j1.in, jobs.j1.ld_in, jobs.j1.fp, jobs.j1.Wcat, jobs.j1.WcatT, jobs.j1.colp, jobs.j1.sig, jobs.j1.rsig, jobs.j1.wp, jobs.j1.wtp);
    else if (blockIdx.y == 2) pack_params_body(jobs.j2.pp, jobs.j2.vc, jobs.j2.in, jobs.j2.ld_in, jobs.j2.fp, jobs.j2.Wcat, jobs.j2.WcatT, jobs.j2.colp, jobs.j2.sig, jobs.j2.rsig, jobs.j2.wp, jobs.j2.wtp);
    else pack_params_body(jobs.j3.pp, jobs.j3.vc, jobs.j3.in, jobs.j3.ld_in, jobs.j3.fp, jobs.j3.Wcat, jobs.j3.WcatT, jobs.j3.colp, jobs.j3.sig, jobs.j3.rsig, jobs.j3.wp, jobs.j3.wtp);
    if (blockIdx.x == 0 && blockIdx.y == 0 && threadIdx.x == 0) handoff_body(ho);
}

template <int L>
__device__ __forceinline__ void slab_sum(const double* __restrict__ slab, int nslab, int fp, int cp, int sl,
                                           double& s1, double& s2) {
    s1 = 0.0;
    s2 = 0.0;
    for (int s0 = sl; s0 < nslab; s0 += L * 8) {
        double2 v[8];
#pragma unroll
        for (int u = 0; u < 8; ++u) {
            const int s = s0 + L * u;
            v[u] = s < nslab ? *reinterpret_cast<const double2*>(slab + ((size_t)s * fp + cp) * 2) : make_double2(0.0, 0.0);
        }
#pragma unroll
        for (int u = 0; u < 8; ++u) { s1 += v[u].x; s2 += v[u].y; }
    }
#pragma unroll
    for (int o = L / 2; o > 0; o >>= 1) {
        s1 += __shfl_xor(s1, o);
        s2 += __shfl_xor(s2, o);
    }
}

constexpr int BWD_ROWS = 7;
template <int L>
__global__ __launch_bounds__(256) void bn_stats_sum_kernel(const double* __restrict__ slab, int nslab, int fp, double M,
                                                            double* __restrict__ out, const int32_t* __restrict__ meta,
                                                            int mode, int tiles_per_wg, int nvirt, int batch_B) {
    if (meta[EAGCN_META_NLOG] > 0) M = (double)batch_B * (double)meta[EAGCN_META_NLOG];
    if (mode == 1 && tiles_per_wg > 0) nslab = min(nslab, (meta[EAGCN_META_NTILES] + tiles_per_wg - 1) / tiles_per_wg);
    if (mode == 1 && tiles_per_wg < 0) nslab = min(nslab, meta[EAGCN_META_NBLK]);
    if (mode == 2) nslab = max(1, min(nslab, (meta[EAGCN_META_T] + nvirt + BWD_ROWS - 1) / BWD_ROWS));
    const int cpr = blockIdx.x * (256 / L) + threadIdx.x / L, sl = threadIdx.x % L;
    const int cp = min(cpr, fp - 1);
    double s1, s2;
    slab_sum<L>(slab, nslab, fp, cp, sl, s1, s2);
    if (cpr < fp && sl == 0) { out[2 * cp] = s1; out[2 * cp + 1] = s2; }
    if (blockIdx.x == 0 && threadIdx.x == 0) out[2 * fp] = M;
}

template <int L>
__global__ __launch_bounds__(256) void bn_finalize_kernel(const double* __restrict__ slab, int nslab, int fp,
                                                           double M, int training, float eps, float momentum,
                                                           const float* __restrict__ colp, ParamPtrs pp,
                                                           ViewCols vc, float* __restrict__ bn,
                                                           const int32_t* __restrict__ meta, int tiles_per_wg, int batch_B,
                                                           const double* __restrict__ M_dev) {
    if (meta[EAGCN_META_NLOG] > 0) M = (double)batch_B * (double)meta[EAGCN_META_NLOG];
    if (M_dev) M = *M_dev;
    if (tiles_per_wg > 0) nslab = min(nslab, (meta[EAGCN_META_NTILES] + tiles_per_wg - 1) / tiles_per_wg);
    if (tiles_per_wg < 0) nslab = min(nslab, meta[EAGCN_META_NBLK]);
    const int cpr = blockIdx.x * (256 / L) + threadIdx.x / L, sl = threadIdx.x % L;
    const int cp = min(cpr, fp - 1);
    double s1 = 0.0, s2 = 0.0;
    if (training) slab_sum<L>(slab, nslab, fp, cp, sl, s1, s2);
    if (cpr >= fp || sl != 0) return;
    const int k = col_view(vc, cp), f = cp - vc.off[k];
    const float gamma = colp[CP_GAMMA * fp + cp], beta = colp[CP_BETA * fp + cp];
    const float bias = colp[CP_BIAS * fp + cp];
    float mu, inv;
    if (training) {
        const double mean = s1 / M;
        double var = s2 / M - mean * mean;
        var = var > 0.0 ? var : 0.0;
        mu = (float)mean;
        inv = (float)(1.0 / sqrt(var + (double)eps));
        if (f < vc.width[k]) {
            const double unbiased = var * (M / (M - 1.0));
            pp.run_mean[k][f] = (float)((1.0 - momentum) * (double)colp[CP_RMEAN * fp + cp] + momentum * (mean + (double)bias));
            pp.run_var[k][f] = (float)((1.0 - momentum) * (double)colp[CP_RVAR * fp + cp] + momentum * unbiased);
        }
    } else {
        mu = colp[CP_RMEAN * fp + cp] - bias;
        inv = 1.0f / sqrtf(colp[CP_RVAR * fp + cp] + eps);
    }
    const float sc = gamma * inv;
    bn[BN_SC * fp + cp] = sc;
    bn[BN_SH * fp + cp] = beta - mu * sc;
    bn[BN_MU * fp + cp] = mu;
    bn[BN_INV * fp + cp] = inv;
}

struct ApplyArgs {
    eagcn_batch bt;
    ViewCols vc;
    int structure, fp;
    const float* Y; int ldy;
    const float* bn;
    const float* colp;
    float* out; int ldo;
    float* pad_row;
    int do_drop; uint32_t thr; float inv_keep; uint64_t seed; const uint64_t* seed_dev;
    BxOut planes;
    int tile_map;
};

__global__ __launch_bounds__(256) void bn_apply_kernel(ApplyArgs a) {
    const int fp = a.fp;
    const uint64_t seed = a.seed_dev ? *a.seed_dev : a.seed;
    if (blockIdx.x == 0) {
        for (int c = threadIdx.x; c < a.ldo; c += blockDim.x) {
            float v = 0.0f;
            if (a.structure == EAGCN_STRUCT_WEIGHTED)
                for (int k = 0; k < a.vc.K; ++k) {
                    const int cp = a.vc.off[k] + c;
                    v += a.colp[CP_AVEW * fp + cp] * fmaxf(a.bn[BN_SH * fp + cp], 0.0f);
                }
            a.pad_row[c] = v;
        }
    }
    const int T = dev_rows(a.bt);
    if (a.structure == EAGCN_STRUCT_CONCATE) {
        const uint32_t g4 = a.tile_map ? ((uint32_t)(fp + 31) >> 5) : fp / 4;
        const uint32_t total = a.tile_map ? (((uint32_t)T + 7) >> 3) * g4 * 64u : (uint32_t)T * g4;
        for (uint32_t e = blockIdx.x * blockDim.x + threadIdx.x; e < total; e += gridDim.x * blockDim.x) {
            int r, c;
            if (a.tile_map) {
                const uint32_t it = e >> 6, rg = it / g4;
                r = (int)(rg * 8u + ((e >> 3) & 7u)); c = (int)((it - rg * g4) * 32u + (e & 7u) * 4u);
                if (r >= T || c >= fp) continue;
            } else {
                r = (int)(e / g4); c = (int)(e - (uint32_t)r * g4) * 4;
            }
            const float4 y = *reinterpret_cast<const float4*>(a.Y + (size_t)r * a.ldy + c);
            const float4 sc = *reinterpret_cast<const float4*>(a.bn + BN_SC * fp + c);
            const float4 sh = *reinterpret_cast<const float4*>(a.bn + BN_SH * fp + c);
            const float m = a.bt.row_m[r];
            float4 o;
            o.x = fmaxf(y.x * sc.x + sh.x, 0.0f) * m;
            o.y = fmaxf(y.y * sc.y + sh.y, 0.0f) * m;
            o.z = fmaxf(y.z * sc.z + sh.z, 0.0f) * m;
            o.w = fmaxf(y.w * sc.w + sh.w, 0.0f) * m;
            if (a.do_drop) {
                float ds[4];
                drop_scale4(seed, (uint64_t)r * fp + c, a.thr, a.inv_keep, ds);
                o.x *= ds[0]; o.y *= ds[1]; o.z *= ds[2]; o.w *= ds[3];
            }
            if (a.out) *reinterpret_cast<float4*>(a.out + (size_t)r * a.ldo + c) = o;
            if (a.planes.p) bx_store4(a.planes, r, c, o);
        }
    } else {
        const uint32_t g4 = a.tile_map ? ((uint32_t)(a.ldo + 31) >> 5) : a.ldo / 4;
        const uint32_t total = a.tile_map ? (((uint32_t)T + 7) >> 3) * g4 * 64u : (uint32_t)T * g4;
        for (uint32_t e = blockIdx.x * blockDim.x + threadIdx.x; e < total; e += gridDim.x * blockDim.x) {
            int r, f;
            if (a.tile_map) {
                const uint32_t it = e >> 6, rg = it / g4;
                r = (int)(rg * 8u + ((e >> 3) & 7u)); f = (int)((it - rg * g4) * 32u + (e & 7u) * 4u);
                if (r >= T || f >= a.ldo) continue;
            } else {
                r = (int)(e / g4); f = (int)(e - (uint32_t)r * g4) * 4;
            }
            float4 y[EAGCN_MAX_VIEWS];
#pragma unroll
            for (int k = 0; k < EAGCN_MAX_VIEWS; ++k)
                if (k < a.vc.K) y[k] = *reinterpret_cast<const float4*>(a.Y + (size_t)r * a.ldy + a.vc.off[k] + f);
            float4 acc = {0.0f, 0.0f, 0.0f, 0.0f};
#pragma unroll
            for (int k = 0; k < EAGCN_MAX_VIEWS; ++k)
                if (k < a.vc.K) {
                    const int cp = a.vc.off[k] + f;
                    const float4 sc = *reinterpret_cast<const float4*>(a.bn + BN_SC * fp + cp);
                    const float4 sh = *reinterpret_cast<const float4*>(a.bn + BN_SH * fp + cp);
                    const float4 w = *reinterpret_cast<const float4*>(a.colp + CP_AVEW * fp + cp);
                    float4 p;
                    p.x = fmaxf(y[k].x * sc.x + sh.x, 0.0f);
                    p.y = fmaxf(y[k].y * sc.y + sh.y, 0.0f);
                    p.z = fmaxf(y[k].z * sc.z + sh.z, 0.0f);
                    p.w = fmaxf(y[k].w * sc.w + sh.w, 0.0f);
                    if (a.do_drop) {
                        float ds[4];
                        drop_scale4(seed, (uint64_t)r * fp + cp, a.thr, a.inv_keep, ds);
                        p.x *= ds[0]; p.y *= ds[1]; p.z *= ds[2]; p.w *= ds[3];
                    }
                    acc.x += w.x * p.x; acc.y += w.y * p.y; acc.z += w.z * p.z; acc.w += w.w * p.w;
                }
            if (a.out) *reinterpret_cast<float4*>(a.out + (size_t)r * a.ldo + f) = acc;
            if (a.planes.p) bx_store4(a.planes, r, f, acc);
        }
    }
}

struct BwdArgs {
    const int32_t* meta; int Tcap;
    const int32_t* row_mol;
    const float* row_m;
    ViewCols vc;
    int structure, fp, nvirt;
    const float* dxout; int ldo;
    ReadoutGrad rg;
    const float* dpad;
    int dpad_views;
    const float* Y; int ldy;
    const float* bn;
    const float* colp;
    float* dH;
    double* slab;
    double* slab_da;
    int do_drop; uint32_t thr; float inv_keep; uint64_t seed; const uint64_t* seed_dev;
    double* zero; int nzero;
    EdgeDrain drain;
    const float* cc;
    int store_dh;
};

template <bool WEIGHTED, bool DG, bool DROP, bool APPLY>
__global__ __launch_bounds__(256) void bn_bwd_reduce_kernel(BwdArgs a) {
    __shared__ double da_s[EAGCN_MAX_VIEWS];
    const uint64_t seed = DROP ? (a.seed_dev ? *a.seed_dev : a.seed) : 0ull;
    const int fp = a.fp, T = min(a.meta[EAGCN_META_T], a.Tcap);
    const int rows = T + (APPLY ? 0 : a.nvirt);
    const int nwg = max(1, min((int)gridDim.x, (rows + BWD_ROWS - 1) / BWD_ROWS));
    if (!APPLY && a.drain.eacc && blockIdx.x == 0 && blockIdx.y == 0) {
        const int K = a.drain.K;
        for (int e = threadIdx.x; e < K * EDGE_SLAB; e += blockDim.x) {
            const int k = e / EDGE_SLAB, c = e - k * EDGE_SLAB;
            if (c > 256) continue;
            double v[EDGE_COPIES];
#pragma unroll
            for (int z = 0; z < EDGE_COPIES; ++z) v[z] = a.drain.eacc[((size_t)z * K + k) * EDGE_SLAB + c];
            double t = 0.0;
#pragma unroll
            for (int z = 0; z < EDGE_COPIES; ++z) { t += v[z]; a.drain.eacc[((size_t)z * K + k) * EDGE_SLAB + c] = 0.0; }
            float* dw = nullptr;
            float* dr = nullptr;
            int ch = 0;
#pragma unroll
            for (int q = 0; q < EAGCN_MAX_VIEWS; ++q)
                if (q == k) { dw = a.drain.datt_w[q]; dr = a.drain.dself_r[q]; ch = a.drain.channels[q]; }
            if (c == 256) {
                const double r = (double)a.drain.rsig[k];
                dr[0] = (float)(t * r * (1.0 - r));
            } else if (c >= 1 && c <= ch) {
                dw[c - 1] = (float)t;
            }
        }
    }
    if ((int)blockIdx.x >= nwg || (APPLY && T == 0)) return;
    if constexpr (!APPLY) {
        if (threadIdx.x < EAGCN_MAX_VIEWS) da_s[threadIdx.x] = 0.0;
        __syncthreads();
    }
    constexpr bool weighted = WEIGHTED;
    double da[EAGCN_MAX_VIEWS];
#pragma unroll
    for (int k = 0; k < EAGCN_MAX_VIEWS; ++k) da[k] = 0.0;
    const int c_lo = blockIdx.y * (int)blockDim.x * 4;
    for (int cp = c_lo + threadIdx.x * 4; cp < min(fp, c_lo + (int)blockDim.x * 4); cp += blockDim.x * 4) {
        const int k = col_view(a.vc, cp), f = cp - a.vc.off[k];
        const float4 sc = *reinterpret_cast<const float4*>(a.bn + BN_SC * fp + cp);
        const float4 sh = *reinterpret_cast<const float4*>(a.bn + BN_SH * fp + cp);
        const float4 mu = *reinterpret_cast<const float4*>(a.bn + BN_MU * fp + cp);
// ... 433 lines not shown
    ParamPtrs pp;
    memset(&pp, 0, sizeof(pp));
    for (int k = 0; k < p->K; ++k) {
        pp.att_w[k] = p->att_w[k]; pp.self_r[k] = p->self_r[k]; pp.W[k] = p->W[k]; pp.bias[k] = p->bias[k];
        pp.gamma[k] = p->gamma[k]; pp.beta[k] = p->beta[k]; pp.run_mean[k] = p->run_mean[k];
        pp.run_var[k] = p->run_var[k]; pp.channels[k] = b->channels[k];
        pp.rel_vec[k] = b->rel_vec[k]; pp.rel_c[k] = b->rel_c[k];
    }
    pp.ave_w = p->structure == EAGCN_STRUCT_WEIGHTED ? p->ave_w : nullptr;
    return pp;
}

static inline int ew_grid(size_t n) { return (int)std::max<size_t>(1, std::min<size_t>((n + 255) / 256, 2048)); }

static void launch_pack_params(const ParamPtrs& pp, const LayerDims& d, const ColMapD& in, const Packed& pk, hipStream_t s) {
    ProfScope ps(PROF_PACK, s);
    pack_params_kernel<<<ew_grid(d.wslab), 256, 0, s>>>(pp, d.vc, in, d.ld_in, d.fp, pk.Wcat, pk.WcatT, pk.colp, pk.sig, pk.rsig,
                                                        BxOut{d.np ? pk.Wp : nullptr, d.wpslab, d.np, d.ld_in},
                                                        BxOut{d.np ? pk.WTp : nullptr, d.wtpslab, d.np, d.fp});
}
static double layer_gemm_work(const eagcn_batch* b, const eagcn_layer_params* p, const LayerDims& d) {
    double fsum = 0.0;
    for (int k = 0; k < p->K; ++k) fsum += p->width[k];
    return 2.0 * (double)b->T * (double)d.fin * fsum;
}

struct LayerOperands {
    const float* x; const uint16_t* xp;
    float* P; Packed pk;
    float* dP; uint16_t* dPp; float* dx; float* dWcat;
};
static LayerOperands layer_operands(const eagcn_layer_bufs* w, const LayerScratch& sc, float* dx) {
    return LayerOperands{w->x, w->x_planes ? w->x_planes : sc.xp, w->P, sc.pk, sc.dP, sc.dPp, dx, sc.dWcat};
}
struct PlaneProducts { BxProb bp, bx, bw; };
static PlaneProducts layer_plane_products(const eagcn_batch* b, const LayerDims& d, const LayerOperands& o) {
    const size_t xstride = bx_plane_elems(b->T, d.ld_in), pstride = bx_plane_elems(b->T, d.fp);
    const int* T_dev = b->meta + EAGCN_META_T;
    PlaneProducts q;
    memset(&q, 0, sizeof(q));
    q.bp.A = BxPlanes{o.xp, xstride, d.ld_in, b->T}; q.bp.B = BxPlanes{o.pk.WTp, d.wtpslab, d.ld_in, d.fp}; q.bp.C = o.P; q.bp.ldc = d.fp;
    q.bp.M = b->T; q.bp.N = d.fp; q.bp.K = d.ld_in; q.bp.M_dev = T_dev; q.bp.tn = 0; q.bp.splits = 1;
    q.bx.A = BxPlanes{o.dPp, pstride, d.fp, b->T}; q.bx.B = BxPlanes{o.pk.Wp, d.wpslab, d.fp, d.ld_in}; q.bx.C = o.dx; q.bx.ldc = d.ld_in;
    q.bx.M = b->T; q.bx.N = d.ld_in; q.bx.K = d.fp; q.bx.M_dev = T_dev; q.bx.tn = 0; q.bx.splits = 1;
    q.bw.A = BxPlanes{o.xp, xstride, d.ld_in, b->T}; q.bw.B = BxPlanes{o.dPp, pstride, d.fp, b->T};
    q.bw.C = o.dWcat; q.bw.ldc = d.fp; q.bw.M = d.ld_in; q.bw.N = d.fp; q.bw.K = b->T; q.bw.K_dev = T_dev; q.bw.tn = 1;
    q.bw.splits = d.bx_splits; q.bw.slab = d.wslab;
    return q;
}
struct Fp32Products { GemmDesc gp, gt, gx, gw; };
static Fp32Products layer_fp32_products(const eagcn_batch* b, const LayerDims& d, const LayerOperands& o, double work) {
    const int* T_dev = b->meta + EAGCN_META_T;
    Fp32Products q{GemmDesc{0, 1, b->T, d.fp, d.ld_in, o.x, d.ld_in, o.pk.WcatT, d.ld_in, o.P, d.fp, 1, 0, work},
                   GemmDesc{0, 0, b->T, d.fp, d.ld_in, o.x, d.ld_in, o.pk.Wcat, d.fp, o.P, d.fp, 1, 0, work},
                   GemmDesc{0, 1, b->T, d.ld_in, d.fp, o.dP, d.fp, o.pk.Wcat, d.fp, o.dx, d.ld_in, 1, 0, work},
                   GemmDesc{1, 0, d.ld_in, d.fp, b->T, o.x, d.ld_in, o.dP, d.fp, o.dWcat, d.fp, d.nsplit, d.wslab, work}};
    q.gp.M_dev = T_dev; q.gt.M_dev = T_dev; q.gx.M_dev = T_dev; q.gw.K_dev = T_dev;
    return q;
}

static bool sw_gemm3() { static const bool on = !env_flag("EAGCN_NO_GEMM3", false); return on; }
bool planes_only_enabled() { static const bool on = env_flag("EAGCN_PLANES_ONLY", true); return on; }
static bool bn_bwd_two_pass(bool weighted) {
    static const int force = getenv("EAGCN_BWD_STORE_DH") ? (env_flag("EAGCN_BWD_STORE_DH", false) ? 1 : 0) : -1;
    return force < 0 ? weighted : force == 0;
}
static bool gemm3_layer(int ld_in) {
    return sw_gemm3() && ld_in >= 128 && gemm_mode() != 2;
}
static int g_first_layer_fused = env_flag("EAGCN_FIRST_LAYER_FUSED", true) ? 1 : 0;
static long g_first_layer_fused_taken = 0;
static int32_t g_first_layer_fused_last[3] = {0, 0, 0};
static bool first_layer_fused_enabled() { return g_first_layer_fused != 0; }
static int g_hidden_bn_sums = env_flag("EAGCN_HIDDEN_BN_SUMS", true) ? 1 : 0;
static long g_hidden_bn_taken = 0;

static LayerRoute plan_layer(const eagcn_batch* b, const eagcn_layer_params* p, const eagcn_layer_bufs* w, const LayerDims& d,
                             const PlanAsk& ask) {
    LayerRoute r;
    const bool wt = p->structure == EAGCN_STRUCT_WEIGHTED;
    bool general = false;
    for (int k = 0; k < p->K; ++k) general = general || b->rel_vec[k] != nullptr;
    r.edge_atomic = !general;
    r.store_dh = !bn_bwd_two_pass(wt);
    if (b->T <= 0) return r;
    r.fwd_agg = fwd_agg_lagg(b, d.vc) ? AGG_LAGG : AGG_DENSE;
    float* const some_dx = reinterpret_cast<float*>(static_cast<uintptr_t>(4096));
    LayerScratch sc;
    carve_layer(w->scratch, b, d, true, &sc);
    if (w->packed) carve_packed(w->packed, d, &sc.pk);
    const LayerOperands o = layer_operands(w, sc, ask.has_dx ? some_dx : nullptr);
    const PlaneProducts bq = layer_plane_products(b, d, o);
    const Fp32Products gq = layer_fp32_products(b, d, o, 0.0);

    r.fwd_split_x = d.np && !w->x_planes;
    if (d.np && bx3_ok(bq.bp)) r.fwd_prod = FWD_PLANES;
    else if (!w->x) r.fwd_prod = FWD_REFUSED;
    else r.fwd_prod = (gemm3_layer(d.ld_in) && gemm3_ok(gq.gp)) ? FWD_BALANCED : FWD_TILED;

    const bool fuse_w = bn_bwd_two_pass(wt) && wt && lagg_wfuse();
    const bool absorbs = !bn_bwd_two_pass(wt) || (wt && lagg_wfuse());
    const bool lagg = ask.input_only ? lagg_use(b, 1, true) : (r.edge_atomic && lagg_use(b, 1, absorbs));
    r.bwd_agg = lagg ? AGG_LAGG : AGG_DENSE;
    if (ask.input_only && !p->training) {
        r.bn2 = !lagg ? BN2_REDUCE_APPLY : wt ? BN2_STAGED_FROM_UPSTREAM : BN2_STAGED_ROWMASK;
        r.rows_first = lagg && ask.mol_grad;
    } else if (lagg && fuse_w) {
        r.bn2 = BN2_STAGED_FROM_UPSTREAM;
        r.rows_first = ask.mol_grad;
    } else if (bn_bwd_two_pass(wt)) r.bn2 = BN2_REDUCE_APPLY;
    else r.bn2 = lagg ? BN2_STAGED_FROM_DH : BN2_ELEMENTWISE;
    if (ask.top_sums && r.bn2 == BN2_STAGED_FROM_DH && ask.mol_grad && !wt) {
        r.bn2 = BN2_STAGED_FROM_READOUT;
        r.rows_late = !ask.top_gather;
        r.store_dh = false;
    }

    r.dh_given = ask.dh_given && g_hidden_bn_sums && r.bn2 == BN2_STAGED_FROM_DH && r.store_dh && !wt && p->training && !ask.mol_grad &&
                 !ask.input_only && hidden_bn_slabs(b->T) <= d.gxb;
    const bool planes = d.np && bx3_ok(bq.bw) && (!ask.has_dx || bx3_ok(bq.bx));
    r.bwd_split_x = planes && !w->x_planes && !ask.input_only;
    if (ask.input_only) r.bwd_prod = planes ? BWD_PLANES_DX : BWD_TILED_DX;
    else if (!planes && !w->x) r.bwd_prod = BWD_REFUSED;
    if (r.bwd_prod != BWD_NONE) return r;
    r.edge = (lagg && r.edge_atomic) ? EDGE_WITH_LAGG : EDGE_COLAUNCH;
    if (planes) {
        r.bwd_prod = ask.has_dx ? BWD_PLANES_PAIR : BWD_PLANES_DW;
        r.bx_wide = (ask.has_dx ? bx3_pick_wide(bq.bx, &bq.bw, b->t_hint) : bx3_pick_wide(bq.bw, nullptr, b->t_hint)) != 0;
        r.carries_below = ask.below && ask.has_dx && !r.bx_wide;
    } else if (ask.has_dx && gemm3_layer(d.ld_in) && gemm3_ok(gq.gw) && gemm3_ok(gq.gx))
        r.bwd_prod = gemm3_xk_enabled() ? BWD_G3_XK : BWD_G3_SCATTER;
    else r.bwd_prod = ask.has_dx ? BWD_TILED_PAIR : BWD_TILED_SEPARATE;
    r.defer_drain = ask.has_drain_out && r.edge_atomic && r.bwd_prod == BWD_G3_SCATTER;
    const bool plain_staging = r.bn2 != BN2_STAGED_FROM_UPSTREAM && r.bn2 != BN2_STAGED_ROWMASK && r.bn2 != BN2_STAGED_FROM_READOUT;
    if (first_layer_fused_enabled() && r.bwd_prod == BWD_TILED_SEPARATE && r.edge == EDGE_WITH_LAGG && r.bwd_agg == AGG_LAGG &&
        plain_staging && d.ld_in <= 32 && gemm_mode() != 1 && gemm_mode() != 2 && w->x) {
        const long cap_w = std::max(std::max(d.nsplit, G3_XSEG), d.np ? d.bx_splits : 1);
        const long cap_p = (long)(((size_t)std::max(b->T, 1) * d.fp) / d.wslab);
        r.dw_fused = true;
        r.dw_ny = (int)std::max<long>(1, std::min<long>(lagg_bwd_grid_y(b, d.vc), std::max(cap_w, cap_p)));
        r.dw_in_dp = r.dw_ny > cap_w;
    }
    return r;
}
LayerRoute plan_layer(const eagcn_batch* b, const eagcn_layer_params* p, const eagcn_layer_bufs* w, const PlanAsk& ask) {
    return plan_layer(b, p, w, layer_dims(b, p), ask);
}
bool top_gather_ok(const eagcn_layer_params* p, const float* dge, int F) {
    bool ok = dge && (reinterpret_cast<uintptr_t>(dge) & 15) == 0 && (F & 3) == 0;
    for (int k = 0; k < p->K; ++k) ok = ok && (p->width[k] & 3) == 0;
    return ok;
}

static int apply_launch(const eagcn_batch* b, const eagcn_layer_params* p, const eagcn_layer_bufs* w, const LayerDims& d,
                        const float* colp, hipStream_t s, bool planes_only = false) {
    ProfScope psbn(PROF_BN, s);
    ApplyArgs aa;
    aa.bt = *b; aa.vc = d.vc; aa.structure = p->structure; aa.fp = d.fp; aa.Y = w->Y; aa.ldy = d.fp;
    aa.bn = w->bn; aa.colp = colp; aa.out = w->xout; aa.ldo = d.ldo; aa.pad_row = w->pad_row;
    const DropArgs dr = drop_args(p->dropout, p->training != 0, p->seed, p->seed_dev);
    aa.do_drop = dr.on; aa.thr = dr.thr; aa.inv_keep = dr.inv_keep; aa.seed = dr.seed; aa.seed_dev = dr.seed_dev;
    aa.planes = BxOut{gemm_planes() ? w->xout_planes : nullptr, bx_plane_elems(b->T, d.ldo), gemm_planes(), b->T};
    if (planes_only && aa.planes.p) aa.out = nullptr;
    aa.tile_map = aa.planes.p ? 1 : 0;
    const size_t nthr = aa.tile_map ? (size_t)cdiv(std::max(b->T, 1), 8) * cdiv(d.ldo, 32) * 64 : (size_t)std::max(b->T, 1) * d.ldo / 4;
    bn_apply_kernel<<<ew_grid(nthr), 256, 0, s>>>(aa);
    EAGCN_LAUNCH_CHECK();
    return EAGCN_OK;
}

}

using namespace eagcn;

extern "C" int eagcn_pad16(int w) { return pad16(w); }
extern "C" int eagcn_layer_fp(const eagcn_layer_params* p) { return view_cols(p).off[p->K]; }
extern "C" int eagcn_layer_out_ld(const eagcn_layer_params* p) {
    return p->structure == EAGCN_STRUCT_CONCATE ? eagcn_layer_fp(p) : pad16(p->width[0]);
}
extern "C" size_t eagcn_layer_packed_bytes(const eagcn_batch* b, const eagcn_layer_params* p) {
    return carve_packed(nullptr, layer_dims(b, p), nullptr);
}
extern "C" size_t eagcn_layer_fwd_scratch_bytes(const eagcn_batch* b, const eagcn_layer_params* p) {
    return carve_layer(nullptr, b, layer_dims(b, p), false, nullptr);
}
extern "C" size_t eagcn_layer_bwd_scratch_bytes(const eagcn_batch* b, const eagcn_layer_params* p) {
    return carve_layer(nullptr, b, layer_dims(b, p), true, nullptr);
}

static bool layer_reads_planes_only(const eagcn_batch* b, const eagcn_layer_params* p) {
    void* const some = reinterpret_cast<void*>(static_cast<uintptr_t>(4096));
    eagcn_layer_bufs w{};
    w.x_planes = static_cast<const uint16_t*>(some); w.P = static_cast<float*>(some); w.scratch = some;
    PlanAsk ask;
    ask.has_dx = true;
    const LayerRoute r = plan_layer(b, p, &w, ask);
    return planes_only_enabled() && r.fwd_prod == FWD_PLANES && r.bwd_prod == BWD_PLANES_PAIR;
}

extern "C" int eagcn_layer_route(const eagcn_batch* b, const eagcn_layer_params* p, const eagcn_layer_bufs* w, int has_dx,
                                 int mol_grad, int input_only, int has_drain_out, int32_t out[16]) {
    int rc = check_layer(b, p, "eagcn_layer_route");
    if (rc) return rc;
    EAGCN_CHECK_ARG(w && out, "eagcn_layer_route: null argument");
    rc = check_reserved_null(w->aux_stream, "eagcn_layer_route", "eagcn_layer_bufs.aux_stream");
    if (rc) return rc;
    PlanAsk ask;
    ask.has_dx = has_dx != 0; ask.mol_grad = mol_grad != 0; ask.input_only = input_only != 0; ask.has_drain_out = has_drain_out != 0;
    const LayerRoute r = plan_layer(b, p, w, ask);
    const int32_t v[16] = {(int32_t)r.fwd_prod, r.fwd_split_x, (int32_t)r.fwd_agg, (int32_t)r.bwd_agg, (int32_t)r.bn2, r.rows_first, r.rows_late, r.store_dh, (int32_t)r.edge,
                           r.edge_atomic, (int32_t)r.bwd_prod, r.bwd_split_x, r.defer_drain,
                           layer_reads_planes_only(b, p), 0, 0};
    memcpy(out, v, sizeof(v));
    return EAGCN_OK;
}

static int clear_handoff_flags(const eagcn_layer_bufs* w, void* stream) {
    if (!(w && w->scratch && w->scratch_bytes >= gemm3_workspace_bytes())) return EAGCN_OK;
    return gemm3_clear_flags(w->scratch, w->scratch_bytes, (hipStream_t)stream);
}
static int plan_checked(const eagcn_batch* b, const eagcn_layer_params* p, const eagcn_layer_bufs* w, const PlanAsk& ask, const char* who,
                        LayerRoute* r) {
    const int rc = check_layer(b, p, who);
    if (rc) return rc;
    EAGCN_CHECK_ARG(w, "%s: null buffer", who);
    *r = plan_layer(b, p, w, ask);
    return EAGCN_OK;
}
extern "C" int eagcn_layer_forward(const eagcn_batch* b, const eagcn_layer_params* p, const eagcn_layer_bufs* w,
                                   void* stream) {
    EAGCN_CHECK_GEMM3("eagcn_layer_forward");
    LayerRoute r;
    int rc = check_reserved_null(w ? w->aux_stream : nullptr, "eagcn_layer_forward", "eagcn_layer_bufs.aux_stream");
    if (!rc) rc = plan_checked(b, p, w, PlanAsk{}, "eagcn_layer_forward", &r);
    if (!rc) rc = clear_handoff_flags(w, stream);
    return rc ? rc : layer_forward_impl(b, p, w, stream, r, false);
}

int eagcn::pack_params_all(const eagcn_batch* b, const eagcn_layer_params* const* ps, void* const* packed,
                           const size_t* packed_bytes, int n, void* stream, const ZeroJob* zj, const HandOff* ho) {
    hipStream_t s = (hipStream_t)stream;
    EAGCN_CHECK_ARG(n >= 1 && n <= 4, "pack_params_all: 1..4 layers");
    PackJob jobs[4];
    size_t wmax = 0;
    for (int l = 0; l < 4; ++l) {
        const int ll = l < n ? l : n - 1;
        int rc = check_layer(b, ps[ll], "eagcn_model_forward");
        if (rc) return rc;
        const LayerDims d = layer_dims(b, ps[ll]);
        Packed pk;
        const size_t pneed = carve_packed(packed[ll], d, &pk);
        if (pneed > packed_bytes[ll]) {
            set_error("pack_params_all: packed buffer of layer %d too small (%zu < %zu)", ll, packed_bytes[ll], pneed);
            return EAGCN_ERR_SCRATCH;
        }
        jobs[l].pp = param_ptrs(b, ps[ll]); jobs[l].vc = d.vc; jobs[l].in = make_colmap(&ps[ll]->in);
        jobs[l].ld_in = d.ld_in; jobs[l].fp = d.fp;
        jobs[l].Wcat = pk.Wcat; jobs[l].WcatT = pk.WcatT; jobs[l].colp = pk.colp; jobs[l].sig = pk.sig; jobs[l].rsig = pk.rsig;
        jobs[l].wp = BxOut{d.np ? pk.Wp : nullptr, d.wpslab, d.np, d.ld_in};
        jobs[l].wtp = BxOut{d.np ? pk.WTp : nullptr, d.wtpslab, d.np, d.fp};
        if (l < n) wmax = std::max(wmax, d.wslab);
    }
    PackJobs pj{jobs[0], jobs[1], jobs[2], jobs[3]};
    ProfScope ps_(PROF_PACK, s);
    const ZeroJob none{nullptr, 0, nullptr, 0};
    const HandOff noho{nullptr, nullptr, nullptr, 0};
    pack_params_multi_kernel<<<dim3(ew_grid(wmax), n), 256, 0, s>>>(pj, zj ? *zj : none, ho ? *ho : noho);
    EAGCN_LAUNCH_CHECK();
    return EAGCN_OK;
}

#define EAGCN_BY_SLABS(n, kernel, ...) do { if ((n) > 64) kernel<64><<<cdiv(d.fp, 4), 256, 0, s>>>(__VA_ARGS__); \
                                            else kernel<16><<<cdiv(d.fp, 16), 256, 0, s>>>(__VA_ARGS__); } while (0)

int eagcn::layer_forward_impl(const eagcn_batch* b, const eagcn_layer_params* p, const eagcn_layer_bufs* w,
                              void* stream, const LayerRoute& r, bool prepacked, bool skip_apply, bool planes_only) {
    hipStream_t s = (hipStream_t)stream;
    int rc = check_layer(b, p, "eagcn_layer_forward");
    if (rc) return rc;
    EAGCN_CHECK_ARG(w && w->bn && w->xout && w->pad_row && w->scratch, "eagcn_layer_forward: null buffer");
    EAGCN_CHECK_ARG(b->T == 0 || ((w->x || w->x_planes) && w->P && w->Y && w->rscale), "eagcn_layer_forward: null activation buffer");
    EAGCN_CHECK_ARG(!planes_only || (w->xout_planes && gemm_planes()), "eagcn_layer_forward: planes-only output without plane images");
    const LayerDims d = layer_dims(b, p);
    LayerScratch sc;
    rc = carve_checked(b, w, d, false, &sc, "eagcn_layer_forward");
    if (rc) return rc;
    const ParamPtrs pp = param_ptrs(b, p);
    EAGCN_CHECK_ARG(!prepacked || w->packed, "eagcn_layer_forward: prepacked parameters need the packed block");
    if (!prepacked) launch_pack_params(pp, d, make_colmap(&p->in), sc.pk, s);
    EAGCN_LAUNCH_CHECK();
    int nslab = 0, tiles_per_wg = agg_ksplit(b) ? 1 : 4;
    if (b->T > 0) {
        const double gemm_work = layer_gemm_work(b, p, d);
        const LayerOperands o = layer_operands(w, sc, nullptr);
        const Fp32Products gq = layer_fp32_products(b, d, o, gemm_work);
        if (r.fwd_prod == FWD_REFUSED) {
            set_error("eagcn_layer_forward: the input exists as plane images only and the plane product does not apply");
            return EAGCN_ERR_ARG;
        }
        if (r.fwd_split_x) {
            rc = launch_bx3_split(w->x, b->T, b->meta + EAGCN_META_T, d.ld_in, sc.xp, bx_plane_elems(b->T, d.ld_in), b->T, d.np, s);
            if (rc) return rc;
        }
        switch (r.fwd_prod) {
        case FWD_PLANES: {
            const BxProb bp = layer_plane_products(b, d, o).bp;
            rc = launch_bx3(bp, nullptr, d.np, s, gemm_work, PROF_GEMM, bx3_pick_wide(bp, nullptr, b->t_hint));
            break;
        }
        case FWD_BALANCED: rc = launch_gemm3(gq.gp, nullptr, sc.gws, gemm3_workspace_bytes(), s); break;
        default: rc = launch_gemm(gq.gt, s); break;
        }
        if (rc) return rc;
        AggArgs a;
        a.bt = *b; a.vc = d.vc; a.src = w->P; a.lds = d.fp; a.dst = w->Y; a.ldd = d.fp;
        a.sig = sc.pk.sig; a.rsig = sc.pk.rsig; a.rscale = w->rscale; a.stats = sc.stats; a.nchunk = 1;
        if (r.fwd_agg == AGG_LAGG) {
            rc = launch_lagg_fwd(a, s);
            nslab = lagg_slabs(b);
            tiles_per_wg = -1;
        } else {
            rc = launch_agg(a, false, s);
            nslab = d.gx;
        }
        if (rc) return rc;
    }
    const double M = (double)b->B * (double)b->N;
    {
        ProfScope psbn(PROF_BN, s);
        const bool sync = w->stats_hook && p->training;
        if (sync) {
            EAGCN_BY_SLABS(nslab, bn_stats_sum_kernel, sc.stats, nslab, d.fp, M, sc.gsum, b->meta, 1, tiles_per_wg, 0, b->B);
            EAGCN_LAUNCH_CHECK();
            if (w->stats_hook(sc.gsum, 2 * d.fp + 1, stream, w->stats_user)) {
                set_error("eagcn_layer_forward: the sync-BatchNorm all-reduce hook failed");
                return EAGCN_ERR_HIP;
            }
            nslab = 1;
        }
        EAGCN_BY_SLABS(nslab, bn_finalize_kernel, sync ? sc.gsum : sc.stats, nslab, d.fp, M, p->training, p->bn_eps, p->bn_momentum, sc.pk.colp,
                       pp, d.vc, w->bn, b->meta, sync ? 0 : tiles_per_wg, b->B, sync ? sc.gsum + 2 * d.fp : nullptr);
        EAGCN_LAUNCH_CHECK();
    }
    if (skip_apply) return EAGCN_OK;
    return apply_launch(b, p, w, d, sc.pk.colp, s, planes_only);
}

static int g_top_bn_sums = !env_flag("EAGCN_TOP_BN_SUMS", true) ? 0 : env_int("EAGCN_TOP_BN_SUMS", 1) == 2 ? 2 : 1;
bool eagcn::top_bn_sums_enabled() { return g_top_bn_sums != 0; }
bool eagcn::top_bn_gather_enabled() { return g_top_bn_sums == 1; }
extern "C" int eagcn_set_top_bn_sums(int on) {
    const int old = g_top_bn_sums;
    g_top_bn_sums = on == 2 ? 2 : on ? 1 : 0;
    return old;
}
extern "C" long eagcn_hidden_bn_sums_taken(int reset) {
    const long n = g_hidden_bn_taken;
    if (reset) g_hidden_bn_taken = 0;
    return n;
}
extern "C" int eagcn_set_hidden_bn_sums(int on) {
    const int old = g_hidden_bn_sums;
    g_hidden_bn_sums = on ? 1 : 0;
    return old;
}
extern "C" long eagcn_first_layer_fused_taken(int reset) {
    const long n = g_first_layer_fused_taken;
    if (reset) g_first_layer_fused_taken = 0;
    return n;
}
extern "C" void eagcn_first_layer_fused_last(int32_t out[3]) { memcpy(out, g_first_layer_fused_last, sizeof(g_first_layer_fused_last)); }
extern "C" int eagcn_set_first_layer_fused(int on) {
    const int old = g_first_layer_fused;
    g_first_layer_fused = on ? 1 : 0;
    return old;
}
int eagcn::layer_apply_impl(const eagcn_batch* b, const eagcn_layer_params* p, const eagcn_layer_bufs* w, void* stream) {
    EAGCN_CHECK_ARG(b && p && w && w->bn && w->xout && w->pad_row && w->packed, "layer_apply: null buffer");
    const LayerDims d = layer_dims(b, p);
    Packed pk;
    EAGCN_CHECK_ARG(carve_packed(w->packed, d, &pk) <= w->packed_bytes, "layer_apply: packed buffer too small");
    return apply_launch(b, p, w, d, pk.colp, (hipStream_t)stream);
}

static void launch_bn_bwd_pass(bool apply, bool wt, bool dg, bool dr, dim3 grid, const BwdArgs& ba, hipStream_t s) {
#define EAGCN_BWD(W, G, D) do { if (apply) bn_bwd_reduce_kernel<W, G, D, true><<<grid, 256, 0, s>>>(ba); \
                                else bn_bwd_reduce_kernel<W, G, D, false><<<grid, 256, 0, s>>>(ba); } while (0)
    if (wt) { if (dg) { if (dr) EAGCN_BWD(true, true, true); else EAGCN_BWD(true, true, false); }
              else    { if (dr) EAGCN_BWD(true, false, true); else EAGCN_BWD(true, false, false); } }
    else    { if (dg) { if (dr) EAGCN_BWD(false, true, true); else EAGCN_BWD(false, true, false); }
              else    { if (dr) EAGCN_BWD(false, false, true); else EAGCN_BWD(false, false, false); } }
#undef EAGCN_BWD
}

extern "C" int eagcn_layer_backward(const eagcn_batch* b, const eagcn_layer_params* p, const eagcn_layer_bufs* w,
                                    const float* dxout, const float* dpad_row, float* dx,
                                    const eagcn_layer_grads* g, void* stream) {
    EAGCN_CHECK_GEMM3("eagcn_layer_backward");
    LayerRoute r;
    int rc = check_reserved_null(w ? w->aux_stream : nullptr, "eagcn_layer_backward", "eagcn_layer_bufs.aux_stream");
    PlanAsk ask;
    ask.has_dx = dx != nullptr;
    if (!rc) rc = plan_checked(b, p, w, ask, "eagcn_layer_backward", &r);
    if (!rc) rc = clear_handoff_flags(w, stream);
    return rc ? rc : layer_backward_impl(b, p, w, dxout, dpad_row, dx, g, stream, r);
}

namespace {
struct LayerBwd {
    const eagcn_batch* b; const eagcn_layer_params* p; const eagcn_layer_bufs* w;
    const float* dxout; const float* dpad_row; LayerBwdOpts o;
    LayerDims d; LayerScratch sc; LayerRoute r; ParamPtrs pp; GradPtrs gp; ColMapD in;
    hipStream_t s;
    bool wt, dg; DropArgs drop; double gemm_work;
    int nsplit = 0, xk_G = 0;
    bool bx_slabs = false;
    int bx_per = 0;
};
}

static GradPtrs grad_ptrs(const eagcn_layer_params* p, const eagcn_layer_grads* g, const LayerDims& d, float* discard) {
    GradPtrs gp;
    memset(&gp, 0, sizeof(gp));
    for (int k = 0; k < p->K; ++k) {
        if (discard) {
            gp.dgamma[k] = discard + d.vc.off[k];
            gp.dbeta[k] = discard + d.fp + d.vc.off[k];
            gp.dbias[k] = discard + 2 * d.fp + d.vc.off[k];
        } else {
            gp.dW[k] = g->dW[k]; gp.dbias[k] = g->dbias[k]; gp.dgamma[k] = g->dgamma[k]; gp.dbeta[k] = g->dbeta[k];
            gp.datt_w[k] = g->datt_w[k]; gp.dself_r[k] = g->dself_r[k];
        }
    }
    gp.dave_w = p->structure != EAGCN_STRUCT_WEIGHTED ? nullptr : discard ? discard + 3 * d.fp : g->dave_w;
    return gp;
}

static int bwd_batchnorm(LayerBwd& c) {
    const eagcn_batch* b = c.b; const eagcn_layer_params* p = c.p; const eagcn_layer_bufs* w = c.w;
    const LayerDims& d = c.d; const LayerScratch& sc = c.sc; const LayerRoute& r = c.r; hipStream_t s = c.s;
    BwdArgs ba;
    ba.meta = b->meta; ba.Tcap = b->T; ba.row_mol = b->row_mol; ba.row_m = b->row_m;
    ba.vc = d.vc; ba.structure = p->structure; ba.fp = d.fp;
    ba.nvirt = (c.dpad_row && c.wt) ? 1 : 0;
    ba.dxout = c.dxout; ba.ldo = d.ldo; ba.dpad = c.dpad_row; ba.dpad_views = c.o.dpad_views ? 1 : 0;
    if (c.o.rg) ba.rg = *c.o.rg; else memset(&ba.rg, 0, sizeof(ba.rg)); ba.Y = w->Y; ba.ldy = d.fp; ba.bn = w->bn;
    ba.colp = sc.pk.colp; ba.dH = sc.dY; ba.slab = sc.slab; ba.slab_da = sc.slab_da;
    ba.do_drop = c.drop.on; ba.thr = c.drop.thr; ba.inv_keep = c.drop.inv_keep; ba.seed = c.drop.seed; ba.seed_dev = c.drop.seed_dev;
    const ZeroJob* za = c.o.zero_after;
    ba.zero = za ? za->d : nullptr;
    ba.nzero = za ? za->nd : 0;
    if (c.o.drain_in && c.o.drain_in->eacc) ba.drain = *c.o.drain_in; else memset(&ba.drain, 0, sizeof(ba.drain));
    ba.cc = sc.cc; ba.store_dh = r.store_dh ? 1 : 0;
    const int ny = cdiv(d.fp, 1024);
    const dim3 grid2(std::max(1, std::min(b->T, d.gxb)), ny);
    const bool dr = ba.do_drop != 0;
    int rc;
    if (c.o.input_only && !p->training) {
        if (r.rows_first) { rc = launch_readout_bwd_rows(b, ba.rg, d.ldo, sc.dY, s); if (rc) return rc; }
        if (r.bn2 == BN2_REDUCE_APPLY) {
            rc = zero_fill(sc.cc, (size_t)2 * d.fp * sizeof(float), s);
            if (rc) return rc;
            launch_bn_bwd_pass(true, c.wt, c.dg, false, grid2, ba, s);
            EAGCN_LAUNCH_CHECK();
        }
        return (za && za->nd) ? zero_fill(za->d, (size_t)za->nd * sizeof(double), s) : EAGCN_OK;
    }
    ProfScope ps(PROF_BN, s);
    const double M = (double)b->B * (double)b->N;
    if (r.bn2 == BN2_STAGED_FROM_READOUT) {
        const int ns = c.o.top_nslab;
        EAGCN_BY_SLABS(ns, bn_bwd_finalize_kernel, c.o.top_sums, sc.slab_da, ns, d.fp, M, p->training, w->bn, d.vc, c.gp, sc.cc, b->meta, 0,
                       b->B, ny, ns, nullptr, ba.zero, ba.nzero, 1);
        EAGCN_LAUNCH_CHECK();
        return r.rows_late ? launch_readout_bwd_rows(b, ba.rg, d.ldo, sc.dY, s) : EAGCN_OK;
    }
    if (r.dh_given) {
        ++g_hidden_bn_taken;
        const int ns = c.o.dh_nslab;
        EAGCN_BY_SLABS(ns, bn_bwd_finalize_kernel, c.o.dh_sums, sc.slab_da, ns, d.fp, M, p->training, w->bn, d.vc, c.gp, sc.cc, b->meta, 0,
                       b->B, ny, ns, nullptr, ba.zero, ba.nzero, 2);
        EAGCN_LAUNCH_CHECK();
        return EAGCN_OK;
    }
    const int gxb = std::max(1, std::min(b->T + ba.nvirt, d.gxb));
    bool dg = c.dg;
    if (r.rows_first) {
        rc = launch_readout_bwd_rows(b, ba.rg, d.ldo, sc.dY, s);
        if (rc) return rc;
        ba.dxout = sc.dY;
        dg = false;
    }
    launch_bn_bwd_pass(false, c.wt, dg, dr, dim3(gxb, ny), ba, s);
    EAGCN_LAUNCH_CHECK();
    const double* gsum = nullptr;
    if (w->stats_hook && p->training) {
        EAGCN_BY_SLABS(gxb, bn_stats_sum_kernel, sc.slab, gxb, d.fp, M, sc.gsum, b->meta, 2, 0, ba.nvirt, b->B);
        EAGCN_LAUNCH_CHECK();
// ... 214 lines not shown
```

eagcn_amd/csrc/readout.hip:

```cpp
#include <algorithm>

#include "common.h"
#include "kernels.h"

namespace eagcn {

__device__ __forceinline__ int exact_to_packed(const ColMapD& m, int ce) {
    int eo = 0, po = 0;
    for (int s = 0; s < m.nseg; ++s) {
        if (ce < eo + m.w[s]) return po + (ce - eo);
        eo += m.w[s];
        po += m.p[s];
    }
    return -1;
}

struct PadSample {
    int K, ld, fp;
    int off[EAGCN_MAX_VIEWS];
    const float* bn_sh;
    const float* ave_w;
    uint64_t seed; const uint64_t* seed_dev;
    uint32_t thr16; float inv_keep;
    uint16_t* cnt;
    float* padc;
    const uint32_t* tab;
    int tab_ld;
};
__global__ __launch_bounds__(1024) void pad_binomial_table_kernel(eagcn_batch bt, uint32_t thr16, uint32_t* __restrict__ tab, int tab_ld) {
    __shared__ double x_s[2][1024];
    const int m = blockIdx.x, k = threadIdx.x;
    if (m > dev_n(bt) || m >= tab_ld) return;
    const double q = __dsub_rn(1.0, __ddiv_rn((double)thr16, 65536.0));
    const double r = __ddiv_rn(q, __dsub_rn(1.0, q));
    int mode = (int)floor(__dmul_rn((double)(m + 1), q));
    mode = mode < 0 ? 0 : (mode > m ? m : mode);
    const bool in = k <= m;
    auto scan = [&](double v, bool down, bool mul) -> double {
        int cur = 0;
        x_s[0][k] = v;
        __syncthreads();
        for (int d = 1; d <= m; d <<= 1) {
            const int o = down ? k + d : k - d;
            double y = x_s[cur][k];
            if (in && o >= 0 && o <= m) y = mul ? __dmul_rn(y, x_s[cur][o]) : __dadd_rn(y, x_s[cur][o]);
            x_s[cur ^ 1][k] = y;
            __syncthreads();
            cur ^= 1;
        }
        const double res = x_s[cur][k];
        __syncthreads();
        return res;
    };
    double up = 1.0, dn = 1.0;
    if (in && k > mode) up = __ddiv_rn(__dmul_rn((double)(m - k + 1), r), (double)k);
    if (in && k < mode) dn = __ddiv_rn((double)(k + 1), __dmul_rn((double)(m - k), r));
    const double pu = scan(up, false, true), pd = scan(dn, true, true);
    const double w = k >= mode ? pu : pd;
    const double c = scan(in ? w : 0.0, false, false);
    __shared__ double S_s;
    if (k == m) S_s = c;
    __syncthreads();
    if (in) {
        const double y = __dmul_rn(__ddiv_rn(c, S_s), 4294967296.0);
        tab[(size_t)m * tab_ld + k] = y >= 4294967295.0 ? 0xFFFFFFFFu : (uint32_t)y;
    }
}
__global__ __launch_bounds__(256) void readout_pad_sample_kernel(eagcn_batch bt, PadSample a) {
    __shared__ uint32_t t_s[1025];
    const int b = blockIdx.y;
    const int c = blockIdx.x * blockDim.x + threadIdx.x;
    const uint64_t seed = a.seed_dev ? *a.seed_dev : a.seed;
    const int m = max(dev_n(bt) - bt.nat[b], 0);
    for (int j = threadIdx.x; j < m; j += blockDim.x) t_s[j] = a.tab[(size_t)m * a.tab_ld + j];
    __syncthreads();
    if (c >= a.ld) return;
    float acc = 0.0f;
    for (int k = 0; k < a.K; ++k) {
        const int cp = a.off[k] + c;
        const uint32_t u = (uint32_t)(rng_u64(seed, (PAD_STREAM_BASE + (uint64_t)b) * (uint64_t)a.fp + (uint64_t)cp) >> 32);
        int lo = 0, hi = m;
        while (lo < hi) {
            const int mid = (lo + hi) >> 1;
            if (t_s[mid] <= u) lo = mid + 1; else hi = mid;
        }
        a.cnt[((size_t)b * a.K + k) * a.ld + c] = (uint16_t)lo;
        acc += a.ave_w[k] * fmaxf(a.bn_sh[cp], 0.0f) * ((float)lo * a.inv_keep);
    }
    a.padc[(size_t)b * a.ld + c] = acc;
}
__global__ __launch_bounds__(1024) void readout_bwd_pad_views_kernel(eagcn_batch bt, const float* __restrict__ dg, ColMapD m,
                                                                      int ld, const int64_t* __restrict__ size, int mode, int F,
                                                                      int K, const uint16_t* __restrict__ cnt, float inv_keep,
                                                                      float* __restrict__ dpad) {
    __shared__ double part[16][64];
    const int lane = threadIdx.x & 63, wave = threadIdx.x >> 6;
    const int cp = blockIdx.x * 64 + lane, k = blockIdx.y;
    int eo = 0, po = 0, ce = -1;
    if (cp < ld)
        for (int s = 0; s < m.nseg; ++s) {
            if (cp < po + m.p[s]) { ce = (cp - po < m.w[s]) ? eo + (cp - po) : -1; break; }
            eo += m.w[s];
            po += m.p[s];
        }
    double acc = 0.0;
    if (ce >= 0) {
        const int per = (bt.B + 15) >> 4;
        const int b0 = wave * per, b1 = min(bt.B, b0 + per);
        for (int b = b0; b < b1; b += 8) {
            float v[8];
#pragma unroll
            for (int u = 0; u < 8; ++u) {
                const int bb = min(b + u, b1 - 1);
                const float inv = mode == 1 ? 1.0f / (float)size[bb] : 1.0f;
                const float t = (float)cnt[((size_t)bb * K + k) * ld + cp] * inv_keep * dg[(size_t)bb * F + ce] * inv;
                v[u] = b + u < b1 ? t : 0.0f;
            }
#pragma unroll
            for (int u = 0; u < 8; ++u) acc += (double)v[u];
        }
    }
    part[wave][lane] = acc;
    __syncthreads();
    if (wave == 0 && cp < ld) {
        double t = 0.0;
#pragma unroll
        for (int w = 0; w < 16; ++w) t += part[w][lane];
        dpad[(size_t)k * ld + cp] = (float)t;
    }
}

__global__ __launch_bounds__(256) void readout_fwd_kernel(eagcn_batch bt, const float* __restrict__ x, ColMapD m,
                                                           int ld, const float* __restrict__ pad_row,
                                                           const float* __restrict__ padc,
                                                           const int64_t* __restrict__ size, int mode,
                                                           float* __restrict__ g, int F) {
    __shared__ float part[4][64];
    const int b = blockIdx.x;
    const int lane = threadIdx.x & 63, wave = threadIdx.x >> 6;
    const int f = blockIdx.y * 64 + lane;
    const int n = bt.nat[b], r0 = bt.row0[b];
    const int cp = f < F ? exact_to_packed(m, f) : 0;
    float s = 0.0f;
    if (f < F)
        for (int i0 = wave; i0 < n; i0 += 16) {
            float v[4];
#pragma unroll
            for (int u = 0; u < 4; ++u) {
                const int i = i0 + 4 * u;
                v[u] = i < n ? x[(size_t)(r0 + i) * ld + cp] : 0.0f;
            }
            s += (v[0] + v[1]) + (v[2] + v[3]);
        }
    part[wave][lane] = s;
    __syncthreads();
    if (wave == 0 && f < F) {
        s = (part[0][lane] + part[1][lane]) + (part[2][lane] + part[3][lane]);
        if (padc) s += padc[(size_t)b * ld + cp];
        else if (pad_row) s += (float)(dev_n(bt) - n) * pad_row[cp];
        const float inv = mode == 1 ? 1.0f / (float)size[b] : 1.0f;
        g[(size_t)b * F + f] = s * inv;
    }
}

template <bool SUMS>
__global__ __launch_bounds__(256) void readout_bn_fwd_kernel(eagcn_batch bt, ColMapD m, ReadoutBn a) {
    __shared__ float part[4][4][64];
    __shared__ float part_a[SUMS ? 2 : 1][SUMS ? 4 : 1][SUMS ? 4 : 1][SUMS ? 64 : 1];
    const int lane = threadIdx.x & 63, wave = threadIdx.x >> 6;
    const int b0 = blockIdx.x * 4;
    const int f = blockIdx.y * 64 + lane;
    if (blockIdx.x == 0 && blockIdx.y == 0 && threadIdx.x == 0) {
        if (a.cnt0) *a.cnt0 = (double)bt.B;
        if (a.cnt1) *a.cnt1 = (double)bt.B;
        if (a.cnt2) *a.cnt2 = (double)bt.B;
    }
    const int nb = min(4, bt.B - b0);
    const bool okf = f < a.F;
    const int cp = okf ? exact_to_packed(m, f) : 0;
    float s[4] = {0.0f, 0.0f, 0.0f, 0.0f};
    float a1[SUMS ? 4 : 1] = {0.0f}, a2[SUMS ? 4 : 1] = {0.0f};
    if constexpr (SUMS) {
#pragma unroll
        for (int j = 1; j < 4; ++j) { a1[j] = 0.0f; a2[j] = 0.0f; }
    }
    const int rbeg = bt.row0[b0], rend = bt.row0[b0 + nb];
    int bnd[4];
#pragma unroll
    for (int j = 0; j < 4; ++j) bnd[j] = bt.row0[min(b0 + j + 1, b0 + nb)];
    if (okf) {
        const uint64_t seed = a.do_drop ? (a.seed_dev ? *a.seed_dev : a.seed) : 0ull;
        const float sc = a.bn[BN_SC * a.fp + cp], sh = a.bn[BN_SH * a.fp + cp];
        const float mu = SUMS ? a.bn[BN_MU * a.fp + cp] : 0.0f, iv = SUMS ? a.bn[BN_INV * a.fp + cp] : 0.0f;
        for (int r0 = rbeg + wave; r0 < rend; r0 += 32) {
            float y[8], mk[8];
#pragma unroll
            for (int u = 0; u < 8; ++u) {
                const int r = min(r0 + 4 * u, rend - 1);
                y[u] = a.Y[(size_t)r * a.ldy + cp];
                mk[u] = bt.row_m[r];
            }
            float ds[8];
            if (a.do_drop && a.pair) {
#pragma unroll
                for (int h = 0; h < 2; ++h) {
                    const int rs = r0 + 4 * (4 * h + (lane & 3));
                    const uint64_t zo = rng_u64(seed, ((uint64_t)rs * a.fp + cp) >> 2);
                    const int lo = (int)(uint32_t)zo, hi = (int)(uint32_t)(zo >> 32);
                    uint32_t w[4];
                    {
                        const uint32_t l0 = (uint32_t)__builtin_amdgcn_mov_dpp(lo, 0x00, 0xF, 0xF, true);
                        const uint32_t h0 = (uint32_t)__builtin_amdgcn_mov_dpp(hi, 0x00, 0xF, 0xF, true);
                        const uint32_t l1 = (uint32_t)__builtin_amdgcn_mov_dpp(lo, 0x55, 0xF, 0xF, true);
                        const uint32_t h1 = (uint32_t)__builtin_amdgcn_mov_dpp(hi, 0x55, 0xF, 0xF, true);
                        const uint32_t l2 = (uint32_t)__builtin_amdgcn_mov_dpp(lo, 0xAA, 0xF, 0xF, true);
                        const uint32_t h2 = (uint32_t)__builtin_amdgcn_mov_dpp(hi, 0xAA, 0xF, 0xF, true);
                        const uint32_t l3 = (uint32_t)__builtin_amdgcn_mov_dpp(lo, 0xFF, 0xF, 0xF, true);
                        const uint32_t h3 = (uint32_t)__builtin_amdgcn_mov_dpp(hi, 0xFF, 0xF, 0xF, true);
                        const bool up = (lane & 2) != 0;
                        w[0] = up ? h0 : l0; w[1] = up ? h1 : l1; w[2] = up ? h2 : l2; w[3] = up ? h3 : l3;
                    }
                    const int sh = 16 * (lane & 1);
#pragma unroll
                    for (int j = 0; j < 4; ++j) ds[4 * h + j] = ((w[j] >> sh) & 0xFFFFu) >= (a.thr >> 16) ? a.inv_keep : 0.0f;
                }
            } else {
#pragma unroll
                for (int u = 0; u < 8; ++u)
                    ds[u] = a.do_drop ? drop_scale_el(seed, (uint64_t)(r0 + 4 * u) * a.fp + cp, a.thr, a.inv_keep) : 1.0f;
            }
#pragma unroll
            for (int u = 0; u < 8; ++u) {
                const int r = r0 + 4 * u;
                if (r < rend) {
                    float v = fmaxf(y[u] * sc + sh, 0.0f) * mk[u];
                    if (a.do_drop) v *= ds[u];
                    const int mi = (r >= bnd[0] ? 1 : 0) + (r >= bnd[1] ? 1 : 0) + (r >= bnd[2] ? 1 : 0);
#pragma unroll
                    for (int j = 0; j < 4; ++j) s[j] += mi == j ? v : 0.0f;
                    if constexpr (SUMS) {
                        const float h = y[u] * sc + sh;
                        const float q = h > 0.0f ? mk[u] * (a.do_drop ? ds[u] : 1.0f) : 0.0f;
                        const float qx = q * ((y[u] - mu) * iv);
#pragma unroll
                        for (int j = 0; j < 4; ++j) { a1[j] += mi == j ? q : 0.0f; a2[j] += mi == j ? qx : 0.0f; }
                    }
                }
            }
        }
    }
#pragma unroll
    for (int j = 0; j < 4; ++j) part[wave][j][lane] = s[j];
    if constexpr (SUMS) {
#pragma unroll
        for (int j = 0; j < 4; ++j) { part_a[0][wave][j][lane] = a1[j]; part_a[1][wave][j][lane] = a2[j]; }
    }
    __syncthreads();
    if (wave == 0 && okf) {
        double s1 = 0.0, s2 = 0.0;
#pragma unroll
        for (int j = 0; j < 4; ++j)
            if (j < nb) {
                float v = (part[0][j][lane] + part[1][j][lane]) + (part[2][j][lane] + part[3][j][lane]);
                if (a.mode == 1) v *= 1.0f / (float)a.size[b0 + j];
                a.g[(size_t)(b0 + j) * a.F + f] = v;
                if constexpr (SUMS) {
                    a.A1[(size_t)(b0 + j) * a.F + f] = (part_a[0][0][j][lane] + part_a[0][1][j][lane]) + (part_a[0][2][j][lane] + part_a[0][3][j][lane]);
                    a.A2[(size_t)(b0 + j) * a.F + f] = (part_a[1][0][j][lane] + part_a[1][1][j][lane]) + (part_a[1][2][j][lane] + part_a[1][3][j][lane]);
                }
                s1 += (double)v;
                s2 += (double)v * (double)v;
            }
        double* st = a.st + (size_t)(blockIdx.x % a.st_copies) * a.st_stride;
        atomicAdd(&st[2 * f], s1);
        atomicAdd(&st[2 * f + 1], s2);
    }
}

int readout_bn_forward(const eagcn_batch* b, const eagcn_layout* lay, const ReadoutBn& a, void* stream) {
    hipStream_t s = (hipStream_t)stream;
    ProfScope ps(PROF_READOUT, s);
    ReadoutBn aa = a;
    aa.pair = (a.fp & 3) == 0 && (a.F & 3) == 0;
    for (int sg = 0; sg < lay->nseg; ++sg) aa.pair = aa.pair && (lay->width[sg] & 3) == 0 && (lay->pad[sg] & 3) == 0;
    EAGCN_CHECK_ARG((a.A1 == nullptr) == (a.A2 == nullptr), "readout_bn_forward: A1 and A2 come together");
    const dim3 grid(cdiv(b->B, 4), cdiv(a.F, 64));
    if (a.A1) readout_bn_fwd_kernel<true><<<grid, 256, 0, s>>>(*b, make_colmap(lay), aa);
    else readout_bn_fwd_kernel<false><<<grid, 256, 0, s>>>(*b, make_colmap(lay), aa);
    EAGCN_LAUNCH_CHECK();
    return EAGCN_OK;
}

__global__ __launch_bounds__(256) void readout_bwd_kernel(eagcn_batch bt, const float* __restrict__ dg, ColMapD m,
                                                           int ld, const int64_t* __restrict__ size, int mode,
                                                           int F, float* __restrict__ dx) {
    const size_t total = (size_t)dev_rows(bt) * ld;
    for (size_t e = (size_t)blockIdx.x * blockDim.x + threadIdx.x; e < total; e += (size_t)gridDim.x * blockDim.x) {
        const int r = (int)(e / ld), cp = (int)(e % ld);
        int eo = 0, po = 0, ce = -1;
        for (int s = 0; s < m.nseg; ++s) {
            if (cp < po + m.p[s]) { ce = (cp - po < m.w[s]) ? eo + (cp - po) : -1; break; }
            eo += m.w[s];
            po += m.p[s];
        }
        const int b = bt.row_mol[r];
        const float inv = mode == 1 ? 1.0f / (float)size[b] : 1.0f;
        dx[e] = ce >= 0 ? dg[(size_t)b * F + ce] * inv : 0.0f;
    }
}

__global__ __launch_bounds__(1024) void readout_bwd_pad_kernel(eagcn_batch bt, const float* __restrict__ dg, ColMapD m,
                                                                int ld, const int64_t* __restrict__ size, int mode,
                                                                int F, float* __restrict__ dpad) {
    __shared__ double part[16][64];
    const int lane = threadIdx.x & 63, wave = threadIdx.x >> 6;
    const int cp = blockIdx.x * 64 + lane;
    int eo = 0, po = 0, ce = -1;
    if (cp < ld)
        for (int s = 0; s < m.nseg; ++s) {
            if (cp < po + m.p[s]) { ce = (cp - po < m.w[s]) ? eo + (cp - po) : -1; break; }
            eo += m.w[s];
            po += m.p[s];
        }
    double acc = 0.0;
    if (ce >= 0) {
        const int per = (bt.B + 15) >> 4, n = dev_n(bt);
        const int b0 = wave * per, b1 = min(bt.B, b0 + per);
        for (int b = b0; b < b1; b += 8) {
            float v[8];
#pragma unroll
            for (int u = 0; u < 8; ++u) {
                const int bb = min(b + u, b1 - 1);
                const float inv = mode == 1 ? 1.0f / (float)size[bb] : 1.0f;
                const float t = (float)(n - bt.nat[bb]) * dg[(size_t)bb * F + ce] * inv;
                v[u] = b + u < b1 ? t : 0.0f;
            }
#pragma unroll
            for (int u = 0; u < 8; ++u) acc += (double)v[u];
        }
    }
    part[wave][lane] = acc;
    __syncthreads();
    if (wave == 0 && cp < ld) {
        double t = 0.0;
#pragma unroll
        for (int w = 0; w < 16; ++w) t += part[w][lane];
        dpad[cp] = (float)t;
    }
}

int readout_forward_sampled(const eagcn_batch* b, const float* x, const eagcn_layout* lay, const eagcn_layer_params* p,
                            const float* bn_sh, const int64_t* size, int mode, float* g, int F, uint16_t* cnt, float* padc,
                            uint32_t* tab, void* stream) {
    hipStream_t s = (hipStream_t)stream;
    const int ld = layout_ld(lay);
    EAGCN_CHECK_ARG(b->N <= 1023, "read-out of a Weighted_sum layer under dropout: N=%d exceeds the 1023 atom slots its kept-row table is built for", b->N);
    PadSample a;
    a.K = p->K; a.ld = ld; a.fp = p->K * ld;
    for (int k = 0; k < EAGCN_MAX_VIEWS; ++k) a.off[k] = k * ld;
    a.bn_sh = bn_sh; a.ave_w = p->ave_w; a.seed = p->seed; a.seed_dev = p->seed_dev;
    a.thr16 = (uint32_t)std::min(65535.0, (double)p->dropout * 65536.0);
    a.inv_keep = 1.0f / (1.0f - p->dropout);
    a.cnt = cnt; a.padc = padc;
    a.tab = tab; a.tab_ld = b->N + 1;
    ProfScope ps(PROF_READOUT, s);
    pad_binomial_table_kernel<<<b->N + 1, 1024, 0, s>>>(*b, a.thr16, tab, a.tab_ld);
    EAGCN_LAUNCH_CHECK();
    readout_pad_sample_kernel<<<dim3(cdiv(ld, 256), b->B), 256, 0, s>>>(*b, a);
    EAGCN_LAUNCH_CHECK();
    readout_fwd_kernel<<<dim3(b->B, cdiv(F, 64)), 256, 0, s>>>(*b, x, make_colmap(lay), ld, nullptr, padc, size, mode, g, F);
    EAGCN_LAUNCH_CHECK();
    return EAGCN_OK;
}
int readout_backward_pad_views(const eagcn_batch* b, const float* dg, const eagcn_layout* lay, const int64_t* size, int mode,
                               int F, int K, const uint16_t* cnt, float dropout, float* dpad, void* stream) {
    hipStream_t s = (hipStream_t)stream;
    ProfScope ps(PROF_READOUT, s);
    readout_bwd_pad_views_kernel<<<dim3(cdiv(layout_ld(lay), 64), K), 1024, 0, s>>>(*b, dg, make_colmap(lay), layout_ld(lay), size,
                                                                                mode, F, K, cnt, 1.0f / (1.0f - dropout), dpad);
    EAGCN_LAUNCH_CHECK();
    return EAGCN_OK;
}

int readout_backward_pad(const eagcn_batch* b, const float* dg, const eagcn_layout* lay, const int64_t* size,
                         int mode, int F, float* dpad_row, void* stream) {
    hipStream_t s = (hipStream_t)stream;
    ProfScope ps(PROF_READOUT, s);
    readout_bwd_pad_kernel<<<cdiv(layout_ld(lay), 64), 1024, 0, s>>>(*b, dg, make_colmap(lay), layout_ld(lay), size,
                                                                   mode, F, dpad_row);
    EAGCN_LAUNCH_CHECK();
    return EAGCN_OK;
}

}

using namespace eagcn;

extern "C" int eagcn_readout_forward(const eagcn_batch* b, const float* x, const eagcn_layout* lay,
                                     const float* pad_row, const int64_t* size, int mode, float* g, int F,
                                     void* stream) {
    hipStream_t s = (hipStream_t)stream;
    EAGCN_CHECK_ARG(b && lay && g, "eagcn_readout_forward: null argument");
    EAGCN_CHECK_ARG(b->T == 0 || x, "eagcn_readout_forward: null activations");
    EAGCN_CHECK_ARG(layout_width(lay) == F, "eagcn_readout_forward: layout width %d != F %d", layout_width(lay), F);
    EAGCN_CHECK_ARG(mode == 0 || (mode == 1 && size), "eagcn_readout_forward: mode 1 ('ave') needs size");
    ProfScope ps(PROF_READOUT, s);
    readout_fwd_kernel<<<dim3(b->B, cdiv(F, 64)), 256, 0, s>>>(*b, x, make_colmap(lay), layout_ld(lay), pad_row, nullptr, size, mode, g, F);
    EAGCN_LAUNCH_CHECK();
    return EAGCN_OK;
}

__global__ __launch_bounds__(256) void readout_bwd_rows_kernel(eagcn_batch bt, const float* __restrict__ dg, ColMapD m, int ld,
                                                                const int64_t* __restrict__ size, int mode, int F, float* __restrict__ dx) {
    const int cp = blockIdx.x * 256 + threadIdx.x;
    if (cp >= ld) return;
    int eo = 0, po = 0, ce = -1;
    for (int s = 0; s < m.nseg; ++s) {
        if (cp < po + m.p[s]) { ce = (cp - po < m.w[s]) ? eo + (cp - po) : -1; break; }
        eo += m.w[s];
        po += m.p[s];
    }
    const int T = dev_rows(bt);
    for (int r0 = blockIdx.y * 8; r0 < T; r0 += gridDim.y * 8) {
        float v[8];
#pragma unroll
        for (int u = 0; u < 8; ++u) {
            const int r = min(r0 + u, T - 1);
            const int b = bt.row_mol[r];
            const float inv = mode == 1 ? 1.0f / (float)size[b] : 1.0f;
            v[u] = ce >= 0 ? dg[(size_t)b * F + ce] * inv : 0.0f;
        }
#pragma unroll
        for (int u = 0; u < 8; ++u)
            if (r0 + u < T) dx[(size_t)(r0 + u) * ld + cp] = v[u];
    }
}
int eagcn::launch_readout_bwd_rows(const eagcn_batch* b, const ReadoutGrad& rg, int ld, float* dx, hipStream_t s) {
    const int gx = cdiv(ld, 256);
    const int gy = std::max(1, std::min(cdiv(std::max(b->T, 1), 8), std::max(1, 4096 / gx)));
    readout_bwd_rows_kernel<<<dim3(gx, gy), 256, 0, s>>>(*b, rg.dg, rg.map, ld, rg.size, rg.mode, rg.F, dx);
// ... 27 lines not shown
```

include/eagcn_hip.h:

```cpp
#ifndef EAGCN_HIP_H
#define EAGCN_HIP_H

#include <stddef.h>
#include <stdint.h>

#ifdef __cplusplus
extern "C" {
#endif

#define EAGCN_MAX_VIEWS 8
#define EAGCN_MAX_SEGS 8
#define EAGCN_MAX_CHANNELS 255
#define EAGCN_STRUCT_CONCATE 0
#define EAGCN_STRUCT_WEIGHTED 1

#define EAGCN_OK 0
#define EAGCN_ERR_ARG (-1)
#define EAGCN_ERR_HIP (-2)
#define EAGCN_ERR_SCRATCH (-3)

#define EAGCN_META_T 0
#define EAGCN_META_NMAX 1
#define EAGCN_META_NTILES 2
#define EAGCN_META_BAD_ADJ 3
// ... 214 lines not shown
    int32_t fuse_readout;
    uint32_t* fwd_signal;
    uint32_t* wait_flag;
    uint32_t* start_signal;
} eagcn_model;

int eagcn_stream_signal_flag(uint32_t* flag, void* stream);
int eagcn_stream_wait_flag(uint32_t* flag, double budget_seconds, void* stream);
int eagcn_stream_wait_timeouts(void);
void eagcn_stream_wait_reset(void);

int eagcn_stream_wait_counter(const uint32_t* counter, uint32_t value, void* stream);

size_t eagcn_model_saved_bytes(const eagcn_batch* b, const eagcn_model* m);
size_t eagcn_model_scratch_bytes(const eagcn_batch* b, const eagcn_model* m);
int eagcn_model_atom_rep(const eagcn_batch* b, const eagcn_model* m, size_t* xout_offset,
                         size_t* pad_row_offset, int* ld);
int eagcn_model_atom_rep_materialize(const eagcn_batch* b, const eagcn_model* m, void* saved, size_t saved_bytes, void* stream);
int eagcn_model_pack_input(const eagcn_batch* b, const eagcn_model* m, const float* afm, void* saved,
                           size_t saved_bytes, void* stream);
int eagcn_model_forward(const eagcn_batch* b, const eagcn_model* m, const float* afm, const int64_t* size,
                        void* saved, size_t saved_bytes, void* scratch, size_t scratch_bytes, float* out,
                        float* graph_rep, void* stream);
int eagcn_model_backward(const eagcn_batch* b, const eagcn_model* m, const int64_t* size, void* saved,
                         size_t saved_bytes, void* scratch, size_t scratch_bytes, const float* dout,
                         const float* dgraph_rep, const eagcn_layer_grads* lg, const eagcn_head_grads* hg,
                         void* stream);

int eagcn_model_backward_range(const eagcn_batch* b, const eagcn_model* m, const int64_t* size, void* saved,
                               size_t saved_bytes, void* scratch, size_t scratch_bytes, const float* dout,
                               const float* dgraph_rep, const eagcn_layer_grads* lg, const eagcn_head_grads* hg,
                               int with_head, int layer_hi, int layer_lo, void* stream);
int eagcn_model_route(const eagcn_batch* b, const eagcn_model* m, void* saved, size_t saved_bytes, void* scratch, size_t scratch_bytes,
                      int with_head, int layer_hi, int layer_lo, int has_dx0, int input_only, int32_t out[4][16]);

size_t eagcn_model_input_scratch_bytes(const eagcn_batch* b, const eagcn_model* m);
int eagcn_model_backward_input(const eagcn_batch* b, const eagcn_model* m, const int64_t* size, void* saved,
                               size_t saved_bytes, void* scratch, size_t scratch_bytes, const float* dout,
                               const float* dgraph_rep, const eagcn_layer_grads* lg, const eagcn_head_grads* hg,
                               float* dafm, void* stream);

float eagcn_attr_alpha(int step, int steps);
float eagcn_attr_weight(int steps);
size_t eagcn_attr_acc_elems(const eagcn_batch* b, const eagcn_model* m);
int eagcn_attr_pack_input(const eagcn_batch* b, const eagcn_model* m, const float* afm, const float* baseline, float alpha,
                          void* saved, size_t saved_bytes, void* stream);
int eagcn_attr_step(const eagcn_batch* b, const eagcn_model* m, const int64_t* size, void* saved, size_t saved_bytes,
                    void* scratch, size_t scratch_bytes, const float* dout, const float* dgraph_rep, float weight, int first,
                    float* acc, void* stream);
int eagcn_attr_finalize(const eagcn_batch* b, const eagcn_model* m, const float* afm, const float* baseline, const float* acc,
                        float* attr, float* score, void* stream);

int eagcn_layer_bond_grad(const eagcn_batch* b, const eagcn_layer_params* p, const eagcn_layer_bufs* w, const float* dxout, int mode,
                          float weight, int first, float* acc, void* stream);
int eagcn_bond_attr_finalize(const eagcn_batch* b, const float* acc, int K, int32_t* mol, int32_t* bi, int32_t* bj, float* score,
                             float* dense, void* stream);

typedef struct eagcn_step_loss {
    int32_t kind;
    const float* labels;
    const float* class_weight;
    float* loss;
    const float* scale;
    float* dout;
} eagcn_step_loss;
int eagcn_model_forward_step(const eagcn_batch* b, const eagcn_model* m, const float* afm, const int64_t* size,
                             void* saved, size_t saved_bytes, void* scratch, size_t scratch_bytes, float* out,
                             float* graph_rep, const eagcn_step_loss* loss, const float* dgraph_rep,
                             const eagcn_head_grads* hg, void* stream);

size_t eagcn_head_saved_bytes(const eagcn_head_params* h, int B);
size_t eagcn_head_scratch_bytes(const eagcn_head_params* h, int B);
int eagcn_head_forward(const eagcn_head_params* h, int B, int training, uint64_t seed, const uint64_t* seed_dev, const float* g,
                       void* saved, size_t saved_bytes, void* scratch, size_t scratch_bytes, float* out, float* graph_rep,
                       void* stream);
int eagcn_head_backward(const eagcn_head_params* h, int B, int training, uint64_t seed, const uint64_t* seed_dev, const float* g,
                        void* saved, size_t saved_bytes, void* scratch, size_t scratch_bytes, const float* dout,
                        const float* dgraph_rep, const eagcn_head_grads* hg, float* dg, void* stream);

int eagcn_bce_loss(const float* logits, const float* labels, const float* class_weight, int B, int T,
                   float* loss, float* dlogits, void* stream);
int eagcn_mse_loss(const float* pred, const float* target, int n, float* loss, float* dpred, void* stream);

int eagcn_adam_step(float* param, const float* grad, float* exp_avg, float* exp_avg_sq, int64_t n, const double* hyper_dev,
                    int64_t* step_dev, uint32_t* ticket_dev, void* stream);

size_t eagcn_grad_norm_workspace_bytes(void);
int eagcn_grad_norm(const float* grad, const uint8_t* live_lanes, int64_t n, void* workspace, int accumulate, void* stream);
int eagcn_adam_step_clipped(float* param, const float* grad, float* exp_avg, float* exp_avg_sq, int64_t n, const double* hyper_dev,
                            int64_t* step_dev, uint32_t* ticket_dev, void* norm_workspace, const double* clip_dev,
                            int64_t* stats_dev, void* stream);

int eagcn_eval_append(const float* logits, const float* labels, int B, int T, int classification, float* scores,
                      float* targets, uint8_t* valid, int64_t row_offset, void* stream);

size_t eagcn_eval_metrics_workspace_bytes(int64_t rows, int T);
int eagcn_eval_class_metrics(const float* scores, const float* targets, const uint8_t* valid, int64_t rows, int T, void* workspace,
                             size_t workspace_bytes, double* out, void* stream);
int eagcn_eval_reg_metrics(const float* scores, const float* targets, const uint8_t* valid, int64_t rows, int T, void* workspace,
                           size_t workspace_bytes, double* out, void* stream);

int eagcn_rep_gather(const eagcn_batch* b, const float* packed, const eagcn_layout* lay, const float* pad_row, const int32_t* subtype,
                     int lo, int hi, const int64_t* mol_index, int64_t* count, int32_t* scratch, float* X, int32_t* sub, int64_t* mol,
                     int64_t cap, void* stream);
int eagcn_rep_gather_dense(const float* dense, int B, int N, int F, const int32_t* subtype, int N_in, int lo, int hi,
                           const int64_t* mol_index, int64_t* count, int32_t* scratch, float* X, int32_t* sub, int64_t* mol, int64_t cap,
                           void* stream);

size_t eagcn_kmeans_workspace_bytes(int64_t n, int F, int k);
int eagcn_kmeans_begin(const float* X, int64_t n, int F, int ld, int k, const float* init, double tol, void* workspace,
                       size_t workspace_bytes, void* stream);
int eagcn_kmeans_iterate(const float* X, int64_t n, int F, int ld, int k, void* workspace, size_t workspace_bytes, void* stream);
int eagcn_kmeans_finish(const float* X, int64_t n, int F, int ld, int k, void* workspace, size_t workspace_bytes, void* stream);
int eagcn_kmeans_assign(const float* X, int64_t n, int F, int ld, const float* centers, int k, int32_t* labels, float* mind,
                        void* workspace, size_t workspace_bytes, void* stream);

#define EAGCN_TSNE_STOP_MAX_ITER 1
#define EAGCN_TSNE_STOP_NO_PROGRESS 2
#define EAGCN_TSNE_STOP_GRAD_NORM 3
int eagcn_sqdist(const float* X, int64_t n, int F, int ld, float* D, void* stream);
size_t eagcn_tsne_workspace_bytes(int64_t n);
int eagcn_tsne_affinities(const float* D, int64_t n, double perplexity, float* P, int ldp, double* betas, int32_t* steps, void* workspace,
                          size_t workspace_bytes, void* stream);
int eagcn_tsne_gradient(const float* P, int ldp, const float* Y, int64_t n, float alpha, int compute_kl, float* grad, double* out,
                        void* workspace, size_t workspace_bytes, void* stream);
int eagcn_tsne_begin(const float* P, int ldp, int64_t n, const float* Y0, float early_exaggeration, float learning_rate, int max_iter,
                     int n_iter_without_progress, double min_grad_norm, void* workspace, size_t workspace_bytes, void* stream);
int eagcn_tsne_iterate(const float* P, int ldp, int64_t n, void* workspace, size_t workspace_bytes, void* stream);
int eagcn_tsne_finish(const float* P, int ldp, int64_t n, void* workspace, size_t workspace_bytes, void* stream);
size_t eagcn_pca_workspace_bytes(int64_t n, int F);
int eagcn_pca_cov(const float* X, int64_t n, int F, int ld, double* mean, double* cov, void* workspace, size_t workspace_bytes, void* stream);
int eagcn_pca_project(const float* X, int64_t n, int F, int ld, const double* mean, const float* components, int k, float* out,
                      void* stream);

#define EAGCN_KNN_MAX_K 128
size_t eagcn_knn_workspace_bytes(int64_t n, int64_t m, int F, int k, int slabs);
int eagcn_knn(const float* X, int64_t n, int F, int ldx, const float* Q, int64_t m, int ldq, int k, int exclude_self, int slabs,
              int32_t* idx, float* dist, void* ws, size_t ws_bytes, void* stream);
int eagcn_knn_rank(const float* X, int64_t n, int F, int ld, const int32_t* cand, int k, int slabs, int32_t* rank, void* ws,
                   size_t ws_bytes, void* stream);

int eagcn_set_gemm_mode(int mode);

size_t eagcn_bx3_plane_elems(int rows_cap, int ld);
int eagcn_bx3_split(const float* x, int rows, int ld, uint16_t* planes, size_t plane_stride, int rows_cap, int np, void* stream);
int eagcn_bx3_used_splits(int splits, int M, int N, int K);
int eagcn_set_bx3_wide(int mode);
int eagcn_set_top_bn_sums(int on);
int eagcn_set_hidden_bn_sums(int on);
long eagcn_hidden_bn_sums_taken(int reset);
int eagcn_set_first_layer_fused(int on);
long eagcn_first_layer_fused_taken(int reset);
void eagcn_first_layer_fused_last(int32_t out[3]);
int eagcn_bx3_pair_used_splits(int splits, int M, int N, int K, int M0, int N0, int K0);
int eagcn_gemm_bx3(int tn, int M, int N, int K, const uint16_t* A, size_t a_pstride, int lda, int a_rows, const uint16_t* B,
                   size_t b_pstride, int ldb, int b_rows, float* C, int ldc, int splits, size_t slab, int np, void* stream);
int eagcn_gemm_bx3_pair(int M0, int N0, int K0, const uint16_t* A0, size_t a0_pstride, int lda0, int a0_rows, const uint16_t* B0,
                        size_t b0_pstride, int ldb0, int b0_rows, float* C0, int ldc0, int M1, int N1, int K1, const uint16_t* A1,
                        size_t a1_pstride, int lda1, int a1_rows, const uint16_t* B1, size_t b1_pstride, int ldb1, int b1_rows,
                        float* C1, int ldc1, int splits, size_t slab, int np, void* stream);

int eagcn_gemm_f32(int ta, int tb, int M, int N, int K, const float* A, int lda, const float* B,
                   int ldb, float* C, int ldc, void* stream);
int eagcn_gemm_f32_dev(int ta, int tb, int M, int N, int K, const float* A, int lda, const float* B,
                       int ldb, float* C, int ldc, const int32_t* extent_dev, int which, void* stream);

size_t eagcn_gemm_sk_workspace_bytes(void);
int eagcn_gemm_f32_sk(int ta, int tb, int M, int N, int K, const float* A, int lda, const float* B, int ldb, float* C,
                      int ldc, void* workspace, size_t workspace_bytes, void* stream);
int eagcn_gemm_pair_sk(int M0, int N0, int K0, const float* A0, int lda0, const float* B0, int ldb0, float* C0, int ldc0,
                       int M1, int N1, int K1, const float* A1, int lda1, const float* B1, int ldb1, float* C1, int ldc1,
                       void* workspace, size_t workspace_bytes, void* stream);
int eagcn_gemm_pair_sk_slabs(int M0, int N0, int K0, const float* A0, int lda0, const float* B0, int ldb0, float* C0, int ldc0,
                             int M1, int N1, int K1, const float* A1, int lda1, const float* B1, int ldb1, float* C1, int ldc1,
                             size_t slab, void* workspace, size_t workspace_bytes, void* stream);
int eagcn_gemm_sk_plan(int M0, int N0, int K0, int M1, int N1, int K1, int wgs, int* a, int* c);
int eagcn_gemm_sk_timeouts(void);
int eagcn_gemm_sk_failed(void);
void eagcn_gemm_sk_reset_failed(void);
void eagcn_gemm_sk_inject_failure(void);

void eagcn_prof_enable(int on);
void eagcn_prof_reset(void);
int eagcn_prof_ntags(void);
const char* eagcn_prof_tag_name(int tag);
int eagcn_prof_read(int tag, double* total_ms, double* work, int64_t* launches);

#ifdef __cplusplus
}
#endif
#endif
```

Baseline: 789,800.

## Fold BatchNorm finalize into the apply and readout kernels

Moves the BatchNorm statistics finalize (slab reduction into scale/shift and running stats) into the consumer kernels. The BN-apply kernel and the top-layer readout kernel now compute scale/shift from the slabs themselves, and extra grid rows co-launch the finalize body to write the BN table and running stats. This removes a separate small kernel launch and its serialization per layer. The cost is redundant slab reductions in every consumer block, larger kernel argument blocks, and gating conditions that decide when the fold applies.

```diff
diff --git a/eagcn_amd/_lib.py b/eagcn_amd/_lib.py
--- a/eagcn_amd/_lib.py
+++ b/eagcn_amd/_lib.py
@@ -217,6 +217,10 @@
     'eagcn_set_first_layer_fused': (C.c_int, [C.c_int]),
     'eagcn_first_layer_fused_taken': (C.c_long, [C.c_int]),
     'eagcn_first_layer_fused_last': (None, [C.POINTER(C.c_int32)]),
+    'eagcn_set_bn_fold': (C.c_int, [C.c_int]),
+    'eagcn_bn_fold_taken': (None, [C.c_int, C.POINTER(C.c_long)]),
+    'eagcn_set_bn_fold_caps': (None, [C.c_int, C.c_long]),
+    'eagcn_model_bn_table': (C.c_int, [C.POINTER(Batch), C.POINTER(Model), C.c_int, C.POINTER(C.c_size_t), C.POINTER(C.c_int)]),
     'eagcn_bx3_pair_used_splits': (C.c_int, [C.c_int] * 7),
     'eagcn_bx3_plane_elems': (C.c_size_t, [C.c_int, C.c_int]),
     'eagcn_bx3_split': (C.c_int, [_fp, C.c_int, C.c_int, _fp, C.c_size_t, C.c_int, C.c_int, _fp]),
diff --git a/eagcn_amd/build.py b/eagcn_amd/build.py
--- a/eagcn_amd/build.py
+++ b/eagcn_amd/build.py
@@ -10,7 +10,7 @@
 LIB = os.path.join(LIBDIR, 'libeagcn_hip.so')
 HIP_SOURCES = ['index.hip', 'gemm.hip', 'gemm3.hip', 'gemm_bx3.hip', 'gemm_bx3w.hip', 'agg.hip', 'lagg.hip', 'lagg_in.hip', 'lagg_top.hip', 'lagg_dw.hip', 'gat.hip', 'pool.hip', 'layer.hip', 'readout.hip', 'head.hip', 'head2.hip', 'loss.hip', 'clip.hip', 'attr.hip', 'battr.hip', 'metrics.hip', 'reps.hip', 'embed.hip', 'knn.hip']
 CPP_SOURCES = ['api.cpp']
-HEADERS = ['common.h', 'kernels.h', 'lagg_kernel.h', 'gemm_x6.h', 'bx3.h', 'bx3_epi.h', os.path.join('..', '..', 'include', 'eagcn_hip.h')]
+HEADERS = ['common.h', 'kernels.h', 'lagg_kernel.h', 'gemm_x6.h', 'bx3.h', 'bx3_epi.h', 'bn_fold.h', os.path.join('..', '..', 'include', 'eagcn_hip.h')]
 ARCH = 'gfx950'
 
 
diff --git a/eagcn_amd/csrc/bn_fold.h b/eagcn_amd/csrc/bn_fold.h
--- /dev/null
+++ b/eagcn_amd/csrc/bn_fold.h
@@ -0,0 +1,151 @@
+#pragma once
+#include "common.h"
+#include "kernels.h"
+
+namespace eagcn {
+
+enum { CP_GAMMA = 0, CP_BETA, CP_BIAS, CP_RMEAN, CP_RVAR, CP_AVEW, CP_ROWS = 8 };
+
+__device__ __forceinline__ int col_view(const ViewCols& vc, int cp) {
+    int k = 0;
+#pragma unroll
+    for (int v = 1; v < EAGCN_MAX_VIEWS; ++v) k += (v < vc.K && cp >= vc.off[v]) ? 1 : 0;
+    return k;
+}
+
+template <int L>
+__device__ __forceinline__ void slab_sum(const double* __restrict__ slab, int nslab, int fp, int cp, int sl,
+                                           double& s1, double& s2) {
+    s1 = 0.0;
+    s2 = 0.0;
+    for (int s0 = sl; s0 < nslab; s0 += L * 8) {
+        double2 v[8];
+#pragma unroll
+        for (int u = 0; u < 8; ++u) {
+            const int s = s0 + L * u;
+            v[u] = s < nslab ? *reinterpret_cast<const double2*>(slab + ((size_t)s * fp + cp) * 2) : make_double2(0.0, 0.0);
+        }
+#pragma unroll
+        for (int u = 0; u < 8; ++u) { s1 += v[u].x; s2 += v[u].y; }
+    }
+#pragma unroll
+    for (int o = L / 2; o > 0; o >>= 1) {
+        s1 += __shfl_xor(s1, o);
+        s2 += __shfl_xor(s2, o);
+    }
+}
+
+template <int J>
+__device__ __forceinline__ void slab_tree(double (&x1)[J], double (&x2)[J]) {
+#pragma unroll
+    for (int o = J / 2; o > 0; o >>= 1)
+#pragma unroll
+        for (int j = 0; j < o; ++j) { x1[j] += x1[j + o]; x2[j] += x2[j + o]; }
+}
+template <int L, int G, int NB>
+__device__ __forceinline__ void slab_tree_sum(const double* __restrict__ slab, int nslab, int fp, int cp, int g, double& s1, double& s2) {
+    constexpr int J = L / G, JB = J / NB;
+    static_assert(J * G == L && JB * NB == J && JB >= 1, "slots split evenly");
+    double b1[NB], b2[NB];
+#pragma unroll
+    for (int q = 0; q < NB; ++q) {
+        double x1[JB], x2[JB];
+#pragma unroll
+        for (int j = 0; j < JB; ++j) {
+            const int s = (j * NB + q) * G + g;
+            const double2 v = s < nslab ? *reinterpret_cast<const double2*>(slab + ((size_t)s * fp + cp) * 2) : make_double2(0.0, 0.0);
+            x1[j] = 0.0 + v.x; x2[j] = 0.0 + v.y;
+        }
+        for (int base = L; base < nslab; base += L) {
+#pragma unroll
+            for (int j = 0; j < JB; ++j) {
+                const int s = base + (j * NB + q) * G + g;
+                if (s < nslab) {
+                    const double2 v = *reinterpret_cast<const double2*>(slab + ((size_t)s * fp + cp) * 2);
+                    x1[j] += v.x; x2[j] += v.y;
+                }
+            }
+        }
+        slab_tree<JB>(x1, x2);
+        b1[q] = x1[0]; b2[q] = x2[0];
+    }
+    slab_tree<NB>(b1, b2);
+    s1 = b1[0]; s2 = b2[0];
+}
+template <int G>
+__device__ __forceinline__ void slab_tree_groups(const double2* part, int stride, double& s1, double& s2) {
+    double x1[G], x2[G];
+#pragma unroll
+    for (int g = 0; g < G; ++g) { const double2 t = part[(size_t)g * stride]; x1[g] = t.x; x2[g] = t.y; }
+    slab_tree<G>(x1, x2);
+    s1 = x1[0]; s2 = x2[0];
+}
+
+__device__ __forceinline__ void bn_fin_live(const BnFin& a, int& nslab, double& M) {
+    const int32_t* meta = a.meta;
+    M = a.M;
+    nslab = a.nslab;
+    if (meta[EAGCN_META_NLOG] > 0) M = (double)a.batch_B * (double)meta[EAGCN_META_NLOG];
+    if (a.M_dev) M = *a.M_dev;
+    if (a.tiles_per_wg > 0) nslab = min(nslab, (meta[EAGCN_META_NTILES] + a.tiles_per_wg - 1) / a.tiles_per_wg);
+    if (a.tiles_per_wg < 0) nslab = min(nslab, meta[EAGCN_META_NBLK]);
+}
+__device__ __forceinline__ void bn_train_consts(double s1, double s2, double M, float eps, double& mean, double& var, float& mu, float& inv) {
+    mean = s1 / M;
+    var = s2 / M - mean * mean;
+    var = var > 0.0 ? var : 0.0;
+    mu = (float)mean;
+    inv = (float)(1.0 / sqrt(var + (double)eps));
+}
+__device__ __forceinline__ void bn_scale_shift(float gamma, float beta, float mu, float inv, float& sc, float& sh) {
+    sc = gamma * inv;
+    sh = beta - mu * sc;
+}
+template <int L>
+__device__ __forceinline__ void bn_finalize_body(const BnFin& a, int blk) {
+    const int fp = a.fp;
+    int nslab;
+    double M;
+    bn_fin_live(a, nslab, M);
+    const int cpr = blk * (256 / L) + threadIdx.x / L, sl = threadIdx.x % L;
+    const int cp = min(cpr, fp - 1);
+    double s1 = 0.0, s2 = 0.0;
+    if (a.training) slab_sum<L>(a.slab, nslab, fp, cp, sl, s1, s2);
+    if (cpr >= fp || sl != 0) return;
+    const float* __restrict__ colp = a.colp;
+    const int k = col_view(a.vc, cp), f = cp - a.vc.off[k];
+    const float gamma = colp[CP_GAMMA * fp + cp], beta = colp[CP_BETA * fp + cp];
+    const float bias = colp[CP_BIAS * fp + cp];
+    float mu, inv;
+    if (a.training) {
+        double mean, var;
+        bn_train_consts(s1, s2, M, a.eps, mean, var, mu, inv);
+        if (f < a.vc.width[k]) {
+            const double unbiased = var * (M / (M - 1.0));
+            float *rm = a.run_mean[0], *rv = a.run_var[0];
+#pragma unroll
+            for (int v = 1; v < EAGCN_MAX_VIEWS; ++v)
+                if (k == v) { rm = a.run_mean[v]; rv = a.run_var[v]; }
+            rm[f] = (float)((1.0 - a.momentum) * (double)colp[CP_RMEAN * fp + cp] + a.momentum * (mean + (double)bias));
+            rv[f] = (float)((1.0 - a.momentum) * (double)colp[CP_RVAR * fp + cp] + a.momentum * unbiased);
+        }
+    } else {
+        mu = colp[CP_RMEAN * fp + cp] - bias;
+        inv = 1.0f / sqrtf(colp[CP_RVAR * fp + cp] + a.eps);
+    }
+    float sc, sh;
+    bn_scale_shift(gamma, beta, mu, inv, sc, sh);
+    a.bn[BN_SC * fp + cp] = sc;
+    a.bn[BN_SH * fp + cp] = sh;
+    a.bn[BN_MU * fp + cp] = mu;
+    a.bn[BN_INV * fp + cp] = inv;
+}
+inline int bn_fin_rows(const BnFin& a, int gx) { return (a.nfin + gx - 1) / gx; }
+__device__ __forceinline__ void bn_finalize_colaunch(const BnFin& a, int rows) {
+    const int blk = ((int)blockIdx.y - rows) * (int)gridDim.x + (int)blockIdx.x;
+    if (blk >= a.nfin) return;
+    if (a.L == 64) bn_finalize_body<64>(a, blk);
+    else bn_finalize_body<16>(a, blk);
+}
+
+}
diff --git a/eagcn_amd/csrc/head.hip b/eagcn_amd/csrc/head.hip
--- a/eagcn_amd/csrc/head.hip
+++ b/eagcn_amd/csrc/head.hip
@@ -305,6 +305,15 @@
     *xout_offset = s.xout_last_off;
     *pad_row_offset = s.pad_last_off;
     *ld = eagcn_layer_out_ld(&m->layer[m->n_layers - 1]);
+    return EAGCN_OK;
+}
+
+extern "C" int eagcn_model_bn_table(const eagcn_batch* b, const eagcn_model* m, int layer, size_t* bn_offset, int* fp) {
+    EAGCN_CHECK_ARG(b && m && bn_offset && fp && layer >= 0 && layer < m->n_layers, "eagcn_model_bn_table: bad argument");
+    ModelSaved s;
+    carve_saved(nullptr, b, m, &s);
+    *bn_offset = (size_t)reinterpret_cast<uintptr_t>(s.L[layer].bn);
+    *fp = s.L[layer].fp;
     return EAGCN_OK;
 }
 
@@ -429,8 +438,10 @@
         RC(pack_params_all(b, ps, pk, pkb, m->n_layers, stream, &zj, &ho));
     }
     P = plan_model(b, m, sv, sc, ModelAsk{});
+    BnFin top_fin = {};
     for (int l = 0; l < m->n_layers; ++l)
-        RC(layer_forward_impl(b, &m->layer[l], &P.L[l].w, stream, P.L[l].fwd, true, P.L[l].skip_apply, P.L[l].planes_only));
+        RC(layer_forward_impl(b, &m->layer[l], &P.L[l].w, stream, P.L[l].fwd, true, P.L[l].skip_apply, P.L[l].planes_only,
+                              l == m->n_layers - 1 && P.L[l].skip_apply ? &top_fin : nullptr));
     const eagcn_layer_params* last = &m->layer[m->n_layers - 1];
     const LayerSaved& LL = sv.L[m->n_layers - 1];
     const eagcn_layout lay = out_layout(last);
@@ -446,6 +457,7 @@
         rb.cnt0 = st_g + 2 * F; rb.cnt1 = st_1 + 2 * n1; rb.cnt2 = st_2 + 2 * n2;
         rb.st_copies = copies; rb.st_stride = sc.n_hst;
         if (P.top_formed) { rb.A1 = sv.top_a1; rb.A2 = sv.top_a2; }
+        if (top_fin.L) { rb.fold = 1; rb.fin = top_fin; }
         RC(readout_bn_forward(b, &lay, rb, stream));
     } else if (pad_sampled(m))
         RC(readout_forward_sampled(b, LL.xout, &lay, last, LL.bn + (size_t)LL.fp , size,
diff --git a/eagcn_amd/csrc/kernels.h b/eagcn_amd/csrc/kernels.h
--- a/eagcn_amd/csrc/kernels.h
+++ b/eagcn_amd/csrc/kernels.h
@@ -290,8 +290,23 @@
 int launch_attr_dense(const eagcn_batch* b, const eagcn_layout* in, const float* acc, const float* x, const float* base, float* attr,
                       float* score, hipStream_t s);
 int model_input_slot(const eagcn_batch* b, const eagcn_model* m, void* saved, size_t saved_bytes, float** x0, const char* who);
+struct BnFin {
+    const double* slab; int nslab;
+    int fp;
+    double M;
+    int training; float eps, momentum;
+    const float* colp;
+    float* run_mean[EAGCN_MAX_VIEWS];
+    float* run_var[EAGCN_MAX_VIEWS];
+    ViewCols vc;
+    float* bn;
+    const int32_t* meta; int tiles_per_wg, batch_B;
+    const double* M_dev;
+    int L;
+    int nfin;
+};
 int layer_forward_impl(const eagcn_batch* b, const eagcn_layer_params* p, const eagcn_layer_bufs* w, void* stream, const LayerRoute& r,
-                       bool prepacked, bool skip_apply = false, bool planes_only = false);
+                       bool prepacked, bool skip_apply = false, bool planes_only = false, BnFin* fin_out = nullptr);
 inline int check_reserved_null(const void* value, const char* who, const char* field) {
     EAGCN_CHECK_ARG(!value, "%s: %s is reserved and must be null", who, field);
     return EAGCN_OK;
@@ -310,6 +325,8 @@
     bool pair = false;
     double *cnt0, *cnt1, *cnt2;
     float* A1 = nullptr; float* A2 = nullptr;
+    int fold = 0;
+    BnFin fin = {};
 };
 int readout_bn_forward(const eagcn_batch* b, const eagcn_layout* lay, const ReadoutBn& a, void* stream);
 int readout_forward_sampled(const eagcn_batch* b, const float* x, const eagcn_layout* lay, const eagcn_layer_params* p,
diff --git a/eagcn_amd/csrc/layer.hip b/eagcn_amd/csrc/layer.hip
--- a/eagcn_amd/csrc/layer.hip
+++ b/eagcn_amd/csrc/layer.hip
@@ -2,6 +2,7 @@
 
 #include <stdlib.h>
 
+#include "bn_fold.h"
 #include "common.h"
 #include "kernels.h"
 
@@ -38,14 +39,6 @@
     float* dave_w;
 };
 
-enum { CP_GAMMA = 0, CP_BETA, CP_BIAS, CP_RMEAN, CP_RVAR, CP_AVEW, CP_ROWS = 8 };
-
-__device__ __forceinline__ int col_view(const ViewCols& vc, int cp) {
-    int k = 0;
-#pragma unroll
-    for (int v = 1; v < EAGCN_MAX_VIEWS; ++v) k += (v < vc.K && cp >= vc.off[v]) ? 1 : 0;
-    return k;
-}
 __device__ __forceinline__ int packed_to_exact(const ColMapD& m, int cp) {
     int eo = 0, po = 0;
     for (int s = 0; s < m.nseg; ++s) {
@@ -138,27 +131,6 @@
     if (blockIdx.x == 0 && blockIdx.y == 0 && threadIdx.x == 0) handoff_body(ho);
 }
 
-template <int L>
-__device__ __forceinline__ void slab_sum(const double* __restrict__ slab, int nslab, int fp, int cp, int sl,
-                                           double& s1, double& s2) {
-    s1 = 0.0;
-    s2 = 0.0;
-    for (int s0 = sl; s0 < nslab; s0 += L * 8) {
-        double2 v[8];
-#pragma unroll
-        for (int u = 0; u < 8; ++u) {
-            const int s = s0 + L * u;
-            v[u] = s < nslab ? *reinterpret_cast<const double2*>(slab + ((size_t)s * fp + cp) * 2) : make_double2(0.0, 0.0);
-        }
-#pragma unroll
-        for (int u = 0; u < 8; ++u) { s1 += v[u].x; s2 += v[u].y; }
-    }
-#pragma unroll
-    for (int o = L / 2; o > 0; o >>= 1) {
-        s1 += __shfl_xor(s1, o);
-        s2 += __shfl_xor(s2, o);
-    }
-}
 
 constexpr int BWD_ROWS = 7;
 template <int L>
@@ -178,46 +150,7 @@
 }
 
 template <int L>
-__global__ __launch_bounds__(256) void bn_finalize_kernel(const double* __restrict__ slab, int nslab, int fp,
-                                                           double M, int training, float eps, float momentum,
-                                                           const float* __restrict__ colp, ParamPtrs pp,
-                                                           ViewCols vc, float* __restrict__ bn,
-                                                           const int32_t* __restrict__ meta, int tiles_per_wg, int batch_B,
-                                                           const double* __restrict__ M_dev) {
-    if (meta[EAGCN_META_NLOG] > 0) M = (double)batch_B * (double)meta[EAGCN_META_NLOG];
-    if (M_dev) M = *M_dev;
-    if (tiles_per_wg > 0) nslab = min(nslab, (meta[EAGCN_META_NTILES] + tiles_per_wg - 1) / tiles_per_wg);
-    if (tiles_per_wg < 0) nslab = min(nslab, meta[EAGCN_META_NBLK]);
-    const int cpr = blockIdx.x * (256 / L) + threadIdx.x / L, sl = threadIdx.x % L;
-    const int cp = min(cpr, fp - 1);
-    double s1 = 0.0, s2 = 0.0;
-    if (training) slab_sum<L>(slab, nslab, fp, cp, sl, s1, s2);
-    if (cpr >= fp || sl != 0) return;
-    const int k = col_view(vc, cp), f = cp - vc.off[k];
-    const float gamma = colp[CP_GAMMA * fp + cp], beta = colp[CP_BETA * fp + cp];
-    const float bias = colp[CP_BIAS * fp + cp];
-    float mu, inv;
-    if (training) {
-        const double mean = s1 / M;
-        double var = s2 / M - mean * mean;
-        var = var > 0.0 ? var : 0.0;
-        mu = (float)mean;
-        inv = (float)(1.0 / sqrt(var + (double)eps));
-        if (f < vc.width[k]) {
-            const double unbiased = var * (M / (M - 1.0));
-            pp.run_mean[k][f] = (float)((1.0 - momentum) * (double)colp[CP_RMEAN * fp + cp] + momentum * (mean + (double)bias));
-            pp.run_var[k][f] = (float)((1.0 - momentum) * (double)colp[CP_RVAR * fp + cp] + momentum * unbiased);
-        }
-    } else {
-        mu = colp[CP_RMEAN * fp + cp] - bias;
-        inv = 1.0f / sqrtf(colp[CP_RVAR * fp + cp] + eps);
-    }
-    const float sc = gamma * inv;
-    bn[BN_SC * fp + cp] = sc;
-    bn[BN_SH * fp + cp] = beta - mu * sc;
-    bn[BN_MU * fp + cp] = mu;
-    bn[BN_INV * fp + cp] = inv;
-}
+__global__ __launch_bounds__(256) void bn_finalize_kernel(BnFin a) { bn_finalize_body<L>(a, blockIdx.x); }
 
 struct ApplyArgs {
     eagcn_batch bt;
@@ -231,11 +164,82 @@
     int do_drop; uint32_t thr; float inv_keep; uint64_t seed; const uint64_t* seed_dev;
     BxOut planes;
     int tile_map;
+    int fold;
+    BnFin fin;
 };
-
+static_assert(sizeof(ApplyArgs) <= 4096, "kernel argument block");
+
+__device__ __forceinline__ void bn_apply_store4(const ApplyArgs& a, uint64_t seed, int r, int c, float4 y, float4 sc, float4 sh, float m) {
+    float4 o;
+    o.x = fmaxf(y.x * sc.x + sh.x, 0.0f) * m;
+    o.y = fmaxf(y.y * sc.y + sh.y, 0.0f) * m;
+    o.z = fmaxf(y.z * sc.z + sh.z, 0.0f) * m;
+    o.w = fmaxf(y.w * sc.w + sh.w, 0.0f) * m;
+    if (a.do_drop) {
+        float ds[4];
+        drop_scale4(seed, (uint64_t)r * a.fp + c, a.thr, a.inv_keep, ds);
+        o.x *= ds[0]; o.y *= ds[1]; o.z *= ds[2]; o.w *= ds[3];
+    }
+    if (a.out) *reinterpret_cast<float4*>(a.out + (size_t)r * a.ldo + c) = o;
+    if (a.planes.p) bx_store4(a.planes, r, c, o);
+}
+__device__ __forceinline__ void bn_apply_folded(const ApplyArgs& a, uint64_t seed, float (*s_cf)[32], double2 (*s_part)[32]) {
+    const int fp = a.fp;
+    const int panels = (fp + 31) >> 5;
+    if ((int)blockIdx.y >= panels) { bn_finalize_colaunch(a.fin, panels); return; }
+    if (blockIdx.x == 0 && blockIdx.y == 0)
+        for (int c = threadIdx.x; c < a.ldo; c += blockDim.x) a.pad_row[c] = 0.0f;
+    const int T = dev_rows(a.bt);
+    if ((int)blockIdx.x * 32 >= T) return;
+    const int lane = threadIdx.x & 63, wave = threadIdx.x >> 6;
+    const int c = (int)blockIdx.y * 32 + (lane & 7) * 4;
+    int rg = (int)blockIdx.x * 4 + wave;
+    int r = rg * 8 + (lane >> 3);
+    bool ok = r < T && c < fp;
+    float4 y = make_float4(0.0f, 0.0f, 0.0f, 0.0f);
+    float m = 0.0f;
+    if (ok) { y = *reinterpret_cast<const float4*>(a.Y + (size_t)r * a.ldy + c); m = a.bt.row_m[r]; }
+    int nslab;
+    double M;
+    bn_fin_live(a.fin, nslab, M);
+    {
+        const int cl = threadIdx.x & 31, g = threadIdx.x >> 5, cq = min((int)blockIdx.y * 32 + cl, fp - 1);
+        double s1, s2;
+        if (a.fin.L == 64) slab_tree_sum<64, 8, 1>(a.fin.slab, nslab, fp, cq, g, s1, s2);
+        else slab_tree_sum<16, 8, 1>(a.fin.slab, nslab, fp, cq, g, s1, s2);
+        s_part[g][cl] = make_double2(s1, s2);
+        __syncthreads();
+        if (threadIdx.x < 32) {
+            slab_tree_groups<8>(&s_part[0][cl], 32, s1, s2);
+            double mean, var;
+            float mu, inv;
+            bn_train_consts(s1, s2, M, a.fin.eps, mean, var, mu, inv);
+            bn_scale_shift(a.colp[CP_GAMMA * fp + cq], a.colp[CP_BETA * fp + cq], mu, inv, s_cf[0][cl], s_cf[1][cl]);
+        }
+    }
+    __syncthreads();
+    const float4 sc = *reinterpret_cast<const float4*>(&s_cf[0][(lane & 7) * 4]);
+    const float4 sh = *reinterpret_cast<const float4*>(&s_cf[1][(lane & 7) * 4]);
+    for (;;) {
+        if (ok) bn_apply_store4(a, seed, r, c, y, sc, sh, m);
+        rg += (int)gridDim.x * 4;
+        if (rg * 8 >= T) break;
+        r = rg * 8 + (lane >> 3);
+        ok = r < T && c < fp;
+        if (ok) { y = *reinterpret_cast<const float4*>(a.Y + (size_t)r * a.ldy + c); m = a.bt.row_m[r]; }
+    }
+}
+
+template <bool FOLD>
 __global__ __launch_bounds__(256) void bn_apply_kernel(ApplyArgs a) {
     const int fp = a.fp;
     const uint64_t seed = a.seed_dev ? *a.seed_dev : a.seed;
+    if constexpr (FOLD) {
+        __shared__ __attribute__((aligned(16))) float s_cf[2][32];
+        __shared__ double2 s_part[8][32];
+        bn_apply_folded(a, seed, s_cf, s_part);
+        return;
+    }
     if (blockIdx.x == 0) {
         for (int c = threadIdx.x; c < a.ldo; c += blockDim.x) {
             float v = 0.0f;
@@ -975,10 +979,45 @@
     return ok;
 }
 
+constexpr int BN_FOLD_DEFAULT = 3;
+static int g_bn_fold = env_int("EAGCN_BN_FOLD", BN_FOLD_DEFAULT) & 15;
+static long g_bn_fold_taken[4] = {0, 0, 0, 0};
+static int g_bn_fold_max_slabs = 96;
+static long g_bn_fold_max_bytes = 16L << 20;
+extern "C" int eagcn_set_bn_fold(int mask) {
+    const int old = g_bn_fold;
+    g_bn_fold = mask & 15;
+    return old;
+}
+extern "C" void eagcn_bn_fold_taken(int reset, long out[4]) {
+    for (int i = 0; i < 4; ++i) {
+        if (out) out[i] = g_bn_fold_taken[i];
+        if (reset) g_bn_fold_taken[i] = 0;
+    }
+}
+extern "C" void eagcn_set_bn_fold_caps(int max_slabs, long max_bytes) {
+    if (max_slabs > 0) g_bn_fold_max_slabs = max_slabs;
+    if (max_bytes > 0) g_bn_fold_max_bytes = max_bytes;
+}
+static bool bn_fold_fwd(int bit, const eagcn_batch* b, const eagcn_layer_params* p, const eagcn_layer_bufs* w, const LayerDims& d,
+                        const LayerRoute& r, long consumer_wgs) {
+    if (!(g_bn_fold & (1 << bit)) || !p->training || p->structure != EAGCN_STRUCT_CONCATE || w->stats_hook) return false;
+    if (b->T <= 0 || r.fwd_agg != AGG_LAGG) return false;
+    for (int k = 0; k < p->K; ++k)
+        if (p->width[k] & 3) return false;
+    const long slabs = std::min(lagg_slabs(b), lagg_bwd_grid_y(b, d.vc));
+    return slabs <= g_bn_fold_max_slabs && consumer_wgs * slabs * 512 <= g_bn_fold_max_bytes;
+}
+static int apply_fold_gx(const eagcn_batch* b, const LayerDims& d) {
+    return std::max(1, std::min(cdiv(cdiv(std::max(b->T, 1), 8), 4), std::max(1, 1024 / cdiv(d.fp, 32))));
+}
+
 static int apply_launch(const eagcn_batch* b, const eagcn_layer_params* p, const eagcn_layer_bufs* w, const LayerDims& d,
-                        const float* colp, hipStream_t s, bool planes_only = false) {
+                        const float* colp, hipStream_t s, bool planes_only = false, const BnFin* fin = nullptr) {
     ProfScope psbn(PROF_BN, s);
     ApplyArgs aa;
+    aa.fold = 0;
+    memset(&aa.fin, 0, sizeof(aa.fin));
     aa.bt = *b; aa.vc = d.vc; aa.structure = p->structure; aa.fp = d.fp; aa.Y = w->Y; aa.ldy = d.fp;
     aa.bn = w->bn; aa.colp = colp; aa.out = w->xout; aa.ldo = d.ldo; aa.pad_row = w->pad_row;
     const DropArgs dr = drop_args(p->dropout, p->training != 0, p->seed, p->seed_dev);
@@ -987,7 +1026,14 @@
     if (planes_only && aa.planes.p) aa.out = nullptr;
     aa.tile_map = aa.planes.p ? 1 : 0;
     const size_t nthr = aa.tile_map ? (size_t)cdiv(std::max(b->T, 1), 8) * cdiv(d.ldo, 32) * 64 : (size_t)std::max(b->T, 1) * d.ldo / 4;
-    bn_apply_kernel<<<ew_grid(nthr), 256, 0, s>>>(aa);
+    if (fin) {
+        EAGCN_CHECK_ARG(aa.tile_map == 1 && p->structure == EAGCN_STRUCT_CONCATE, "apply_launch: the folded finalize runs on the panel map of a Concate layer");
+        aa.fold = 1;
+        aa.fin = *fin;
+        const int gx = apply_fold_gx(b, d);
+        bn_apply_kernel<true><<<dim3(gx, cdiv(d.fp, 32) + bn_fin_rows(*fin, gx)), 256, 0, s>>>(aa);
+    } else
+        bn_apply_kernel<false><<<ew_grid(nthr), 256, 0, s>>>(aa);
     EAGCN_LAUNCH_CHECK();
     return EAGCN_OK;
 }
@@ -1097,7 +1143,7 @@
                                             else kernel<16><<<cdiv(d.fp, 16), 256, 0, s>>>(__VA_ARGS__); } while (0)
 
 int eagcn::layer_forward_impl(const eagcn_batch* b, const eagcn_layer_params* p, const eagcn_layer_bufs* w,
-                              void* stream, const LayerRoute& r, bool prepacked, bool skip_apply, bool planes_only) {
+                              void* stream, const LayerRoute& r, bool prepacked, bool skip_apply, bool planes_only, BnFin* fin_out) {
     hipStream_t s = (hipStream_t)stream;
     int rc = check_layer(b, p, "eagcn_layer_forward");
     if (rc) return rc;
@@ -1149,6 +1195,8 @@
         if (rc) return rc;
     }
     const double M = (double)b->B * (double)b->N;
+    BnFin fin;
+    bool folded = false;
     {
         ProfScope psbn(PROF_BN, s);
         const bool sync = w->stats_hook && p->training;
@@ -1161,12 +1209,26 @@
             }
             nslab = 1;
         }
-        EAGCN_BY_SLABS(nslab, bn_finalize_kernel, sync ? sc.gsum : sc.stats, nslab, d.fp, M, p->training, p->bn_eps, p->bn_momentum, sc.pk.colp,
-                       pp, d.vc, w->bn, b->meta, sync ? 0 : tiles_per_wg, b->B, sync ? sc.gsum + 2 * d.fp : nullptr);
-        EAGCN_LAUNCH_CHECK();
-    }
+        fin.slab = sync ? sc.gsum : sc.stats; fin.nslab = nslab; fin.fp = d.fp; fin.M = M; fin.training = p->training;
+        fin.eps = p->bn_eps; fin.momentum = p->bn_momentum; fin.colp = sc.pk.colp;
+        for (int k = 0; k < EAGCN_MAX_VIEWS; ++k) { fin.run_mean[k] = pp.run_mean[k]; fin.run_var[k] = pp.run_var[k]; }
+        fin.vc = d.vc; fin.bn = w->bn; fin.meta = b->meta; fin.tiles_per_wg = sync ? 0 : tiles_per_wg; fin.batch_B = b->B;
+        fin.M_dev = sync ? sc.gsum + 2 * d.fp : nullptr;
+        fin.L = nslab > 64 ? 64 : 16;
+        fin.nfin = cdiv(d.fp, 256 / fin.L);
+        if (skip_apply)
+            folded = fin_out && bn_fold_fwd(1, b, p, w, d, r, (long)cdiv(b->B, 4) * cdiv(d.vc.off[p->K], 64));
+        else
+            folded = gemm_planes() && w->xout_planes && bn_fold_fwd(0, b, p, w, d, r, (long)apply_fold_gx(b, d) * cdiv(d.fp, 32));
+        if (folded) ++g_bn_fold_taken[skip_apply ? 1 : 0];
+        else {
+            EAGCN_BY_SLABS(nslab, bn_finalize_kernel, fin);
+            EAGCN_LAUNCH_CHECK();
+        }
+    }
+    if (fin_out) { *fin_out = fin; if (!folded) fin_out->L = 0; }
     if (skip_apply) return EAGCN_OK;
-    return apply_launch(b, p, w, d, sc.pk.colp, s, planes_only);
+    return apply_launch(b, p, w, d, sc.pk.colp, s, planes_only, folded ? &fin : nullptr);
 }
 
 static int g_top_bn_sums = !env_flag("EAGCN_TOP_BN_SUMS", true) ? 0 : env_int("EAGCN_TOP_BN_SUMS", 1) == 2 ? 2 : 1;
diff --git a/eagcn_amd/csrc/readout.hip b/eagcn_amd/csrc/readout.hip
--- a/eagcn_amd/csrc/readout.hip
+++ b/eagcn_amd/csrc/readout.hip
@@ -1,5 +1,6 @@
 #include <algorithm>
 
+#include "bn_fold.h"
 #include "common.h"
 #include "kernels.h"
 
@@ -163,11 +164,13 @@
     }
 }
 
-template <bool SUMS>
+template <bool SUMS, bool FOLD = false>
 __global__ __launch_bounds__(256) void readout_bn_fwd_kernel(eagcn_batch bt, ColMapD m, ReadoutBn a) {
     __shared__ float part[4][4][64];
     __shared__ float part_a[SUMS ? 2 : 1][SUMS ? 4 : 1][SUMS ? 4 : 1][SUMS ? 64 : 1];
+    __shared__ double2 s_sum[FOLD ? 4 : 1][FOLD ? 64 : 1];
     const int lane = threadIdx.x & 63, wave = threadIdx.x >> 6;
+    if (FOLD && (int)blockIdx.y >= (a.F + 63) / 64) { bn_finalize_colaunch(a.fin, (a.F + 63) / 64); return; }
     const int b0 = blockIdx.x * 4;
     const int f = blockIdx.y * 64 + lane;
     if (blockIdx.x == 0 && blockIdx.y == 0 && threadIdx.x == 0) {
@@ -188,17 +191,43 @@
     int bnd[4];
 #pragma unroll
     for (int j = 0; j < 4; ++j) bnd[j] = bt.row0[min(b0 + j + 1, b0 + nb)];
+    float sc = 0.0f, sh = 0.0f, mu = 0.0f, iv = 0.0f;
+    float y[8], mk[8];
+    if constexpr (FOLD) {
+        if (okf && rbeg + wave < rend) {
+#pragma unroll
+            for (int u = 0; u < 8; ++u) {
+                const int r = min(rbeg + wave + 4 * u, rend - 1);
+                y[u] = a.Y[(size_t)r * a.ldy + cp];
+                mk[u] = bt.row_m[r];
+            }
+        }
+        int nslab;
+        double M;
+        bn_fin_live(a.fin, nslab, M);
+        double s1, s2;
+        if (a.fin.L == 64) slab_tree_sum<64, 4, 2>(a.fin.slab, nslab, a.fp, cp, wave, s1, s2);
+        else slab_tree_sum<16, 4, 1>(a.fin.slab, nslab, a.fp, cp, wave, s1, s2);
+        s_sum[wave][lane] = make_double2(s1, s2);
+        __syncthreads();
+        slab_tree_groups<4>(&s_sum[0][lane], 64, s1, s2);
+        double mean, var;
+        bn_train_consts(s1, s2, M, a.fin.eps, mean, var, mu, iv);
+        bn_scale_shift(a.fin.colp[CP_GAMMA * a.fp + cp], a.fin.colp[CP_BETA * a.fp + cp], mu, iv, sc, sh);
+    } else if (okf) {
+        sc = a.bn[BN_SC * a.fp + cp]; sh = a.bn[BN_SH * a.fp + cp];
+        mu = SUMS ? a.bn[BN_MU * a.fp + cp] : 0.0f; iv = SUMS ? a.bn[BN_INV * a.fp + cp] : 0.0f;
+    }
     if (okf) {
         const uint64_t seed = a.do_drop ? (a.seed_dev ? *a.seed_dev : a.seed) : 0ull;
-        const float sc = a.bn[BN_SC * a.fp + cp], sh = a.bn[BN_SH * a.fp + cp];
-        const float mu = SUMS ? a.bn[BN_MU * a.fp + cp] : 0.0f, iv = SUMS ? a.bn[BN_INV * a.fp + cp] : 0.0f;
         for (int r0 = rbeg + wave; r0 < rend; r0 += 32) {
-            float y[8], mk[8];
-#pragma unroll
-            for (int u = 0; u < 8; ++u) {
-                const int r = min(r0 + 4 * u, rend - 1);
-                y[u] = a.Y[(size_t)r * a.ldy + cp];
-                mk[u] = bt.row_m[r];
+            if (!FOLD || r0 != rbeg + wave) {
+#pragma unroll
+                for (int u = 0; u < 8; ++u) {
+                    const int r = min(r0 + 4 * u, rend - 1);
+                    y[u] = a.Y[(size_t)r * a.ldy + cp];
+                    mk[u] = bt.row_m[r];
+                }
             }
             float ds[8];
             if (a.do_drop && a.pair) {
@@ -284,8 +313,12 @@
     aa.pair = (a.fp & 3) == 0 && (a.F & 3) == 0;
     for (int sg = 0; sg < lay->nseg; ++sg) aa.pair = aa.pair && (lay->width[sg] & 3) == 0 && (lay->pad[sg] & 3) == 0;
     EAGCN_CHECK_ARG((a.A1 == nullptr) == (a.A2 == nullptr), "readout_bn_forward: A1 and A2 come together");
-    const dim3 grid(cdiv(b->B, 4), cdiv(a.F, 64));
-    if (a.A1) readout_bn_fwd_kernel<true><<<grid, 256, 0, s>>>(*b, make_colmap(lay), aa);
+    EAGCN_CHECK_ARG(!a.fold || (a.fin.L == 16 || a.fin.L == 64), "readout_bn_forward: folded finalize without its description");
+    const dim3 grid(cdiv(b->B, 4), cdiv(a.F, 64) + (a.fold ? bn_fin_rows(a.fin, cdiv(b->B, 4)) : 0));
+    if (a.fold) {
+        if (a.A1) readout_bn_fwd_kernel<true, true><<<grid, 256, 0, s>>>(*b, make_colmap(lay), aa);
+        else readout_bn_fwd_kernel<false, true><<<grid, 256, 0, s>>>(*b, make_colmap(lay), aa);
+    } else if (a.A1) readout_bn_fwd_kernel<true><<<grid, 256, 0, s>>>(*b, make_colmap(lay), aa);
     else readout_bn_fwd_kernel<false><<<grid, 256, 0, s>>>(*b, make_colmap(lay), aa);
     EAGCN_LAUNCH_CHECK();
     return EAGCN_OK;
diff --git a/include/eagcn_hip.h b/include/eagcn_hip.h
--- a/include/eagcn_hip.h
+++ b/include/eagcn_hip.h
@@ -390,6 +390,10 @@
 int eagcn_set_first_layer_fused(int on);
 long eagcn_first_layer_fused_taken(int reset);
 void eagcn_first_layer_fused_last(int32_t out[3]);
+int eagcn_set_bn_fold(int mask);
+void eagcn_bn_fold_taken(int reset, long out[4]);
+int eagcn_model_bn_table(const eagcn_batch* b, const eagcn_model* m, int layer, size_t* bn_offset, int* fp);
+void eagcn_set_bn_fold_caps(int max_slabs, long max_bytes);
 int eagcn_bx3_pair_used_splits(int splits, int M, int N, int K, int M0, int N0, int K0);
 int eagcn_gemm_bx3(int tn, int M, int N, int K, const uint16_t* A, size_t a_pstride, int lda, int a_rows, const uint16_t* B,
                    size_t b_pstride, int ldb, int b_rows, float* C, int ldc, int splits, size_t slab, int np, void* stream);
```

Result: faster. 800,600, median of 5 (+1.4%).
